# chpio/crdt-enc

Hardware: AMD Instinct MI355X
Metric: op files compacted/sec + AEAD-open GB/s, 1M×4KiB ops/4096 actors, 1–8 GPUs (higher is better)
Workload: dtype u32; 1 GPU; C2: 1,048,576 x 4 KiB encrypted GCounter op files per GPU (4096 actors x 256 versions at N=1), decrypt + max-join + compact; plaintext_bytes=4085, actors=4096, parallelism=single GPU

## Files before the change

### crdt-enc_amd/csrc/ce_core.cpp

```cpp
#include <algorithm>
#include <atomic>
#include <cstdio>
#include <functional>
#include <set>

#include "ce_core.h"
#include "ce_shard.h"

using namespace ce;

namespace ce {


bool skip_any(Rd& r, int depth) {
  if (depth > 1024) return false;
  uint64_t at, cnt = 0;
  if (r.i >= r.n) return false;
  const uint8_t m = r.p[r.i];
  bool cont = false;
  if ((m & 0xf0) == 0x80) { r.i++; cnt = 2ull * (m & 15); cont = true; }
  else if ((m & 0xf0) == 0x90) { r.i++; cnt = m & 15; cont = true; }
  else if (m == 0xdc || m == 0xdd || m == 0xde || m == 0xdf) {
    r.i++;
    if (!rd_be(r, (m == 0xdc || m == 0xde) ? 2 : 4, &cnt)) return false;
// ... 660 lines not shown
  if (is_dotset_kind(c->kind))
    return ds_ingest_ops(c, d_blob, d_offs, n, blob_len, actors, m, d_fa, d_fv, status_out);
  if (c->kind == CE_STATE_GSET)
    return gs_ingest_ops(c, d_blob, d_offs, n, blob_len, actors, m, d_fa, d_fv, status_out);
  if (c->kind == CE_STATE_LWWREG)
    return lw_ingest_ops(c, d_blob, d_offs, n, blob_len, actors, m, d_fa, d_fv, status_out);
  hipError_t e;
  const KeyRef key = key_of(c);
  const bool pnc = c->kind == CE_STATE_PNCOUNTER;
  auto words = [&] { return (uint64_t)state_planes(c->kind) * c->cap; };
  std::vector<uint32_t> wslot;
  if (c->last_writers_gen == c->table_gen && c->last_writers.size() == 16ull * m &&
      std::memcmp(c->last_writers.data(), actors, 16ull * m) == 0) {
    wslot = c->last_wslot;
  } else {
    wslot.resize(m);
    const uint64_t gen0 = c->table_gen;
    for (uint32_t a = 0; a < m; a++) {
      Uuid u;
      std::memcpy(u.data(), actors + 16ull * a, 16);
      int rc = insert_actor(c, u, &wslot[a]);
      if (rc) return rc;
    }
    if (c->table_gen != gen0) refresh_slots(c, actors, m, &wslot);
    c->last_writers.assign(actors, actors + 16ull * m);
    c->last_wslot = wslot;
    c->last_writers_gen = c->table_gen;
  }
  int rc = table_upload(c);
  if (rc) return rc;
  if ((rc = ensure_supported(c))) return rc;
  if ((e = ctx->out.reserve(blob_len + 16ull * n + 128)) || (e = ctx->status.reserve(n * 4ull + 64)) ||
      (e = ctx->apply.reserve(n + 64)) || (e = ctx->refold.reserve(n + 64)) ||
      (e = c->d_refold2.reserve(n + 64)) || (e = ctx->miss.reserve(65536 * 16)) ||
      (e = c->d_gate.reserve(m * 32ull + 8ull * c->cap + 64)) ||
      (e = ctx->h_stage2.reserve(m * 32ull + 8ull * c->cap + 64)) ||
      (e = ctx->redo.reserve(n + 64)))
    return ctx->hip_fail(e, "ingest reserve");

  uint64_t* he0 = ctx->h_stage2.as<uint64_t>();
  for (uint32_t a = 0; a < m; a++) he0[a] = c->nov[wslot[a]];
  std::memcpy(he0 + m, wslot.data(), m * 4ull);
  if (after_commit) std::memcpy(reinterpret_cast<uint8_t*>(he0) + 32ull * m, c->nov.data(), 8ull * c->cap);
  GateArgs ga{};
  ga.fa = d_fa;
  ga.fv = d_fv;
  ga.n = n;
  ga.m = m;
  uint8_t* gbase = c->d_gate.as<uint8_t>();
  ga.e0 = reinterpret_cast<const uint64_t*>(gbase);
  ga.newnov = reinterpret_cast<unsigned long long*>(gbase + 16ull * m);
  ga.run_count = reinterpret_cast<uint32_t*>(gbase + 24ull * m);
  ga.run_first = reinterpret_cast<uint32_t*>(gbase + 28ull * m);
  ga.flags = ctx->counters.as<uint32_t>() + 12;
  ga.apply = ctx->apply.as<uint8_t>();

  static const bool gate_dma = getenv("CE_GATE_DMA") != nullptr;
  const uint8_t* he0_dev = nullptr;
  if (!gate_dma) {
    void* dp = nullptr;
    if (hipHostGetDevicePointer(&dp, he0, 0) == hipSuccess) he0_dev = static_cast<const uint8_t*>(dp);
    else (void)hipGetLastError();
  }
  if (!he0_dev &&
      ((!ctx->side && (e = hipStreamCreateWithFlags(&ctx->side, hipStreamNonBlocking))) ||
       (!ctx->up_ev && (e = hipEventCreateWithFlags(&ctx->up_ev, hipEventDisableTiming))) ||
       (e = hipMemcpyAsync(gbase, he0, 12ull * m, hipMemcpyHostToDevice, ctx->side)) ||
       (after_commit && (e = hipMemcpyAsync(gbase + 32ull * m, reinterpret_cast<uint8_t*>(he0) + 32ull * m,
                                            8ull * c->cap, hipMemcpyHostToDevice, ctx->side))) ||
       (e = hipEventRecord(ctx->up_ev, ctx->side))))
    return ctx->hip_fail(e, "gate upload");

  static const bool gate_after_setup = getenv("CE_GATE_AFTER_SETUP") != nullptr;
  auto launch_gate_now = [&]() -> int {
    if (!he0_dev && (e = hipStreamWaitEvent(ctx->stream, ctx->up_ev, 0))) return ctx->hip_fail(e, "gate upload");
    const int t = ctx->tbegin("gate");
    if ((e = sharded ? launch_gate_window(ctx->stream, ga, shard_hi, ctx->counters.as<uint32_t>())
                     : launch_gate(ctx->stream, ga)))
      return ctx->hip_fail(e, "gate");
    ctx->tend(t);
    return CE_OK;
  };
  uint32_t ec;
  {
    FillArgs fl{};
    fl.r[0] = {reinterpret_cast<uint32_t*>(gbase + 16ull * m), 4ull * m, 0u};
    fl.r[1] = {c->d_batch.as<uint32_t>(), 2ull * words(), 0u};
    fl.r[2] = {ctx->refold.as<uint32_t>(), (n + 3ull) / 4, 0u};
    fl.r[3] = {ctx->redo.as<uint32_t>(), (n + 3ull) / 4, 0u};
    fl.n = 4;
    if (he0_dev) {
      fl.r[fl.n++] = {reinterpret_cast<uint32_t*>(gbase), 3ull * m, 0u, reinterpret_cast<const uint32_t*>(he0_dev)};
      if (after_commit)
        fl.r[fl.n++] = {reinterpret_cast<uint32_t*>(gbase + 32ull * m), 2ull * c->cap, 0u,
                        reinterpret_cast<const uint32_t*>(he0_dev + 32ull * m)};
    }
    if (!gate_after_setup) {
      const std::function<int()> gate = launch_gate_now;
      int rr = device_open_setup(ctx, d_blob, d_offs, n, blob_len, true, key, ctx->status.as<int32_t>(),
                                 &ec, &fl, &gate);
      if (rr) return rr;
    } else {
      int rr = device_open_setup(ctx, d_blob, d_offs, n, blob_len, true, key, ctx->status.as<int32_t>(),
                                 &ec, &fl);
      if (rr) return rr;
    }
  }
  uint32_t* hsetup = ctx->h_counters.as<uint32_t>() + 32;
  static const bool setup_event = getenv("CE_SETUP_EVENT") != nullptr;
  uint32_t* hsetup_dev = nullptr;
  if (!setup_event) {
    void* dp = nullptr;
    if (hipHostGetDevicePointer(&dp, hsetup, 0) == hipSuccess) hsetup_dev = static_cast<uint32_t*>(dp);
    else (void)hipGetLastError();
  }
  const uint32_t gen = ++ctx->publish_gen ? ctx->publish_gen : ++ctx->publish_gen;
  if (hsetup_dev) {
    if ((e = launch_publish_words(ctx->stream, ctx->counters.as<uint32_t>(), 16, hsetup_dev, gen)))
      return ctx->hip_fail(e, "setup counters");
  } else {
    if ((!ctx->setup_ev && (e = hipEventCreateWithFlags(&ctx->setup_ev, hipEventDisableTiming))) ||
        (!ctx->side_ev && (e = hipEventCreateWithFlags(&ctx->side_ev, hipEventDisableTiming))) ||
        (!ctx->side && (e = hipStreamCreateWithFlags(&ctx->side, hipStreamNonBlocking))))
      return ctx->hip_fail(e, "event");
    if ((e = hipEventRecord(ctx->side_ev, ctx->stream)) || (e = hipStreamWaitEvent(ctx->side, ctx->side_ev, 0)) ||
        (e = hipMemcpyAsync(hsetup, ctx->counters.p, 64, hipMemcpyDeviceToHost, ctx->side)) ||
        (e = hipEventRecord(ctx->setup_ev, ctx->side)))
      return ctx->hip_fail(e, "setup counters");
  }
  bool setup_known = false;
  uint32_t n_large = 0;
  if (gate_after_setup) {
    const int rg = launch_gate_now();
    if (rg) return rg;
  }
  DecodeArgs da{};
  da.pt = ctx->out.as<uint8_t>();
  da.blob = d_blob;
  da.params = ctx->params.as<FileParams>();
  da.aux = ctx->poly_aux.as<PolyAux>();
  da.status = ctx->status.as<int32_t>();
  da.n = n;
  da.supported = c->d_supported.as<uint8_t>();
  da.n_supported = (uint32_t)c->supported.size();
  da.apply = ctx->apply.as<uint8_t>();
  da.counters = ctx->counters.as<uint32_t>();
  da.miss_list = ctx->miss.as<uint4>();
  da.miss_cap = 65536;
  da.refold = ctx->refold.as<uint8_t>();
  da.table = c->d_table.as<ActorSlot>();
  da.mask = c->cap - 1;
  da.nil_actor = table_has_nil(c);
  da.batch = c->d_batch.as<unsigned long long>();
  da.large_list = ctx->large.as<uint32_t>();

  ctx->open_log.grid_cap = test_grid_cap();
  ctx->open_log.stamps = test_wave_stamps(ctx);
  ctx->open_log.stamp_waves = 0;
  auto run_fold = [&](const uint8_t* only) -> int {
    da.only = only;
    da.large_only = 1;
    if (only && (e = hipMemsetAsync(ctx->counters.as<uint32_t>() + kTicketWord, 0, 4, ctx->stream)))
      return ctx->hip_fail(e, "ticket");
    if (pnc) {
      hipEvent_t t0, t1;
      (void)ctx->tlaunch("open_fold_small", &t0, &t1);
      if ((e = launch_open_fold_pn(ctx->stream, da, ctx->open_log, t0, t1))) return ctx->hip_fail(e, "fused");
    } else if (c->fused == 2 && c->files_per_wave != 1) {
      hipEvent_t t0, t1;
      (void)ctx->tlaunch("open_fold_small", &t0, &t1);
      if ((e = launch_open_fold_v2(ctx->stream, da, c->files_per_wave, ctx->open_log, t0, t1))) return ctx->hip_fail(e, "fused");
    } else {
      const int t = ctx->tbegin("open_fold_small");
      if ((e = launch_open_fold_small(ctx->stream, da, c->files_per_wave, ctx->open_log))) return ctx->hip_fail(e, "fused");
      ctx->tend(t);
    }
    count_open_launches(c, ctx);
    if (!setup_known) {
      if (hsetup_dev) {
        volatile const uint32_t* hp = hsetup;
        for (uint64_t i = 0; hp[16] != gen; i++) {
          if (i >= 64) sched_yield();
          if (i == (1ull << 22)) {
            if ((e = hipStreamSynchronize(ctx->stream))) return ctx->hip_fail(e, "setup counters");
          } else if (i > (1ull << 22) && hp[16] != gen) {
            return ctx->fail(CE_ERR_DEVICE, "setup counters never published");
          }
        }
        std::atomic_thread_fence(std::memory_order_acquire);
      } else if ((e = hipEventSynchronize(ctx->setup_ev))) {
        return ctx->hip_fail(e, "setup counters");
      }
      n_large = hsetup[9];
      setup_known = true;
    }
    if (n_large == 0) return CE_OK;
    const char* sdv = getenv("CE_SEGDEC");
    const bool segdec = !pnc && !(sdv && sdv[0] == '0') && !getenv("CE_SPLIT");
    if (!only) {
      SegScratch sc = segscratch(ctx, ec);
      if (segdec && (e = ctx->segrec.reserve((size_t)ec * 2 * 32))) return ctx->hip_fail(e, "segment records");
      int t = ctx->tbegin("segments_open");
      if ((e = segdec ? launch_segments_decode(ctx->stream, d_blob, ctx->out.as<uint8_t>(), da, sc,
                                               grid_waves_for(n + ec), ctx->segrec.as<uint4>())
                      : launch_segments(ctx->stream, false, d_blob, ctx->out.as<uint8_t>(), da.params, n,
                                        da.status, sc, grid_waves_for(n + ec), true)))
        return ctx->hip_fail(e, "segments");
      ctx->tend(t);
      t = ctx->tbegin("finalize_open");
      if ((e = launch_finalize_multi(ctx->stream, false, ctx->out.as<uint8_t>(), da.params, da.status, sc, n)))
        return ctx->hip_fail(e, "finalize");
      ctx->tend(t);
      if (segdec) {
        t = ctx->tbegin("decode");
        DecodeArgs rd = da;
        rd.redo = ctx->redo.as<uint8_t>();
        if ((e = launch_segdec_apply(ctx->stream, rd, sc, ctx->segrec.as<uint4>(), n_large)))
          return ctx->hip_fail(e, "decode");
        rd.only = rd.redo;
        if ((e = launch_decode_dots(ctx->stream, rd, grid_waves_for(n)))) return ctx->hip_fail(e, "decode");
        ctx->tend(t);
        return CE_OK;
      }
// ... 1636 lines not shown
```

### crdt-enc_amd/csrc/ce_ctx.cpp

```cpp
#include <sys/random.h>

#include <algorithm>
#include <cstdio>

#include "ce_dotset.h"
#include "ce_dotset_io.h"
#include "ce_internal.h"
#include "ce_lww.h"

namespace ce {

hipError_t DevBuf::reserve(size_t bytes) {
  if (bytes <= cap) return hipSuccess;
  if (p) (void)hipFree(p);
  p = nullptr;
  cap = 0;
  size_t want = std::max<size_t>(bytes, 256);
  want = (want + 4095) & ~size_t(4095);
  hipError_t e = hipMalloc(&p, want);
  if (e == hipSuccess) cap = want;
  return e;
}
DevBuf::~DevBuf() {
  if (p) (void)hipFree(p);
// ... 15 lines not shown

void os_random(uint8_t* out, size_t n) {
  size_t got = 0;
  while (got < n) {
    ssize_t r = getrandom(out + got, n - got, 0);
    if (r > 0) got += (size_t)r;
  }
}

int32_t key_status(const KeyRef& k) {
  if (std::memcmp(k.version, kKeyVersion, 16) != 0) return CE_ERR_KEY_VERSION;
  if (k.len != 32) return CE_ERR_KEY_LEN;
  return CE_OK;
}

DevKey dev_key(const KeyRef& k) {
  DevKey d{};
  if (k.len == 32) std::memcpy(d.k, k.key, 32);
  return d;
}

uint32_t test_grid_cap() {
  const char* e = getenv("CE_TEST_GRID_CAP");
  const long v = e ? atol(e) : 0;
  return v < 1 ? 0u : (uint32_t)std::min<long>(v, 1l << 30);
}

unsigned long long* test_wave_stamps(ce_ctx* ctx) {
  const char* e = getenv("CE_TEST_WAVE_STAMPS");
  if (!e || atoi(e) < 1) return nullptr;
  const size_t bytes = (size_t)kStampWaves * kStampWords * 8;
  if (ctx->stamps.reserve(bytes) != hipSuccess || hipMemsetAsync(ctx->stamps.p, 0, bytes, ctx->stream) != hipSuccess) {
    (void)hipGetLastError();
    return nullptr;
  }
  return ctx->stamps.as<unsigned long long>();
}

uint32_t grid_waves_for(uint32_t work) {
  uint32_t full = 256u * 32u;
  if (const uint32_t cap = test_grid_cap()) full = std::min(full, cap);
  return std::max<uint32_t>(1, std::min<uint32_t>(work, full));
}

static int reserve_batch(ce_ctx* ctx, uint32_t n, uint64_t blob_len, uint32_t* extra_cap,
                         uint32_t seg_blocks = kSegBlocks) {
  const uint64_t ec = blob_len / (seg_blocks * 16) + 16;
  if (ec > 0xffffffffull) return ctx->fail(CE_ERR_INVALID_ARG, "batch too large");
  *extra_cap = (uint32_t)ec;
  hipError_t e;
  if ((e = ctx->params.reserve((size_t)n * sizeof(FileParams))) != hipSuccess ||
      (e = ctx->status.reserve((size_t)n * 4 + 64)) != hipSuccess ||
      (e = ctx->counters.reserve(256)) != hipSuccess ||
      (e = ctx->extra.reserve(ec * 8)) != hipSuccess ||
      (e = ctx->multi.reserve(ec * 4)) != hipSuccess ||
      (e = ctx->partials.reserve(ec * 2 * 5 * 4)) != hipSuccess ||
      (e = ctx->large.reserve((size_t)n * 4 + 64)) != hipSuccess ||
      (e = ctx->h_counters.reserve(256)) != hipSuccess)
    return ctx->hip_fail(e, "reserve batch scratch");
  return CE_OK;
}

SegScratch segscratch(ce_ctx* ctx, uint32_t extra_cap) {
  SegScratch sc;
  sc.counters = ctx->counters.as<uint32_t>();
  sc.extra_list = ctx->extra.as<uint2>();
  sc.extra_cap = extra_cap;
  sc.multi_files = ctx->multi.as<uint32_t>();
  sc.partials = ctx->partials.as<uint32_t>();
  sc.large_list = ctx->large.as<uint32_t>();
  sc.seg_blocks = kSegBlocks;
  return sc;
}

static hipError_t reset_counters(ce_ctx* ctx) {
  FillArgs fl{};
  fl.n = 0;
  fl.counters = ctx->counters.as<uint32_t>();
  return launch_fill(ctx->stream, fl);
}

int device_open_setup(ce_ctx* ctx, const uint8_t* d_blob, const uint64_t* d_offs, uint32_t n,
                      uint64_t blob_len, bool outer, const KeyRef& key, int32_t* d_status,
                      uint32_t* extra_cap, FillArgs* fills, const std::function<int()>* after_fill) {
  int rc = reserve_batch(ctx, n, blob_len, extra_cap);
  if (rc) return rc;
  hipError_t e;
  if (fills) {
    fills->counters = ctx->counters.as<uint32_t>();
    if ((e = launch_fill(ctx->stream, *fills)) != hipSuccess) return ctx->hip_fail(e, "fill");
  } else if ((e = reset_counters(ctx)) != hipSuccess) {
    return ctx->hip_fail(e, "memset counters");
  }
  if (after_fill && (rc = (*after_fill)())) return rc;
  SegScratch sc = segscratch(ctx, *extra_cap);
  if ((e = ctx->poly_aux.reserve((size_t)n * sizeof(PolyAux))) != hipSuccess)
    return ctx->hip_fail(e, "reserve poly aux");
  const int t = ctx->tbegin("open_setup");
  if ((e = launch_open_setup(ctx->stream, d_blob, d_offs, n, outer, dev_key(key), key_status(key),
                             ctx->params.as<FileParams>(), d_status, sc,
                             ctx->poly_aux.as<PolyAux>())) != hipSuccess)
    return ctx->hip_fail(e, "open setup");
  ctx->tend(t);
  return CE_OK;
}

int device_open(ce_ctx* ctx, const uint8_t* d_blob, const uint64_t* d_offs, uint32_t n,
                uint64_t blob_len, bool outer, const KeyRef& key, uint8_t* d_out,
                int32_t* d_status, bool sync_counters, bool small_lanes, const DecodeArgs* ds) {
  uint32_t ec;
  int rc = reserve_batch(ctx, n, blob_len, &ec);
  if (rc) return rc;
  hipError_t e;
  if ((e = reset_counters(ctx)) != hipSuccess) return ctx->hip_fail(e, "memset counters");
  SegScratch sc = segscratch(ctx, ec);
  FileParams* P = ctx->params.as<FileParams>();
  static const bool ds8_on = !(getenv("CE_DS8") && atoi(getenv("CE_DS8")) == 0);
  const bool want_aux = small_lanes && ds && ds->ds.on && ds->ds.big && ds8_on;
  if (want_aux && (e = ctx->poly_aux.reserve((size_t)n * sizeof(PolyAux))) != hipSuccess)
    return ctx->hip_fail(e, "reserve poly aux");
  int t = ctx->tbegin("open_setup");
  if ((e = launch_open_setup(ctx->stream, d_blob, d_offs, n, outer, dev_key(key), key_status(key),
                             P, d_status, sc, want_aux ? ctx->poly_aux.as<PolyAux>() : nullptr)) != hipSuccess)
    return ctx->hip_fail(e, "open setup");
  ctx->tend(t);
  if (small_lanes) {
    ctx->open_log.grid_cap = test_grid_cap();
    ctx->open_log.stamps = nullptr;
    ctx->open_log.stamp_waves = 0;
    DecodeArgs da{};
    da.pt = d_out;
    da.blob = d_blob;
    da.params = P;
    da.status = d_status;
    da.n = n;
    da.counters = ctx->counters.as<uint32_t>();
    if (ds) {
      da.ds = ds->ds;
      da.aux = want_aux ? ctx->poly_aux.as<PolyAux>() : nullptr;
      da.supported = ds->supported;
      da.n_supported = ds->n_supported;
      da.table = ds->table;
      da.mask = ds->mask;
    }
    t = ctx->tbegin("open_small");
    if ((e = launch_open_small_v2(ctx->stream, da, ctx->open_log)) != hipSuccess) return ctx->hip_fail(e, "open small");
    ctx->tend(t);
  }
  t = ctx->tbegin("segments_open");
  if ((e = launch_segments(ctx->stream, false, d_blob, d_out, P, n, d_status, sc,
                           grid_waves_for(n + ec), small_lanes)) != hipSuccess)
    return ctx->hip_fail(e, "open segments");
  ctx->tend(t);
  t = ctx->tbegin("finalize_open");
  if ((e = launch_finalize_multi(ctx->stream, false, d_out, P, d_status, sc, n)) != hipSuccess)
    return ctx->hip_fail(e, "open finalize");
  ctx->tend(t);
  if (sync_counters) {
    if ((e = hipMemcpyAsync(ctx->h_counters.p, ctx->counters.p, 64, hipMemcpyDeviceToHost,
                            ctx->stream)) != hipSuccess ||
        (e = stream_wait(ctx->stream)) != hipSuccess)
      return ctx->hip_fail(e, "open sync");
  }
  return CE_OK;
}

uint32_t* ctx_counters(ce_ctx* ctx) {
  return ctx->counters.reserve(256) == hipSuccess ? ctx->counters.as<uint32_t>() : nullptr;
}

int device_seal(ce_ctx* ctx, const uint8_t* d_clear, const uint64_t* d_offs, uint32_t n,
                uint64_t clear_len_total, const uint8_t* d_outer_version, const uint8_t* d_nonces,
                uint8_t* d_out, const uint64_t* d_out_offs, const KeyRef& key, bool counters_ready) {
  if (int32_t ks = key_status(key)) return ctx->fail(ks, "key rejected");
  const uint32_t seg_blocks = n <= 4 && clear_len_total <= (1u << 20) ? kPageBytes / 16 : kSegBlocks;
  uint32_t ec;
  int rc = reserve_batch(ctx, n, clear_len_total + 16ull * n, &ec, seg_blocks);
  if (rc) return rc;
  hipError_t e;
  if (!counters_ready && (e = reset_counters(ctx)) != hipSuccess) return ctx->hip_fail(e, "memset counters");
  SegScratch sc = segscratch(ctx, ec);
  sc.seg_blocks = seg_blocks;
  FileParams* P = ctx->params.as<FileParams>();
  int t = ctx->tbegin("seal_setup");
  if ((e = launch_seal_setup(ctx->stream, d_clear, d_offs, n, d_outer_version, d_nonces, d_out,
                             d_out_offs, dev_key(key), P, sc)) != hipSuccess)
    return ctx->hip_fail(e, "seal setup");
  ctx->tend(t);
  t = ctx->tbegin("segments_seal");
  if ((e = launch_segments(ctx->stream, true, d_clear, d_out, P, n, ctx->status.as<int32_t>(), sc,
                           grid_waves_for(n + ec))) != hipSuccess)
    return ctx->hip_fail(e, "seal segments");
  ctx->tend(t);
  t = ctx->tbegin("finalize_seal");
  if ((e = launch_finalize_multi(ctx->stream, true, d_out, P, ctx->status.as<int32_t>(), sc, n)) !=
      hipSuccess)
    return ctx->hip_fail(e, "seal finalize");
  ctx->tend(t);
  return CE_OK;
}

int seal_one(ce_ctx* ctx, const KeyRef& key, const uint8_t* outer_version, const uint8_t* nonce,
             const uint8_t* clear_in, size_t clear_in_len, std::vector<uint8_t>* file,
             const uint8_t* prefix16) {
  if (int32_t ks = key_status(key)) return ctx->fail(ks, "key rejected");
  const size_t pl = prefix16 ? 16 : 0;
  const size_t clear_len = pl + clear_in_len;
  const uint64_t pre = outer_version ? 16 : 0;
  const uint64_t total = pre + sealed_len(clear_len);
  uint8_t nb[24];
  if (nonce) std::memcpy(nb, nonce, 24);
  else os_random(nb, 24);
  hipError_t e;
  const uint64_t A = (clear_len + 255) & ~255ull;
  if ((e = ctx->blob.reserve(A + 128)) != hipSuccess ||
      (e = ctx->out.reserve(total + 64)) != hipSuccess ||
      (e = ctx->h_stage.reserve(std::max<uint64_t>(A + 128, total) + 256)) != hipSuccess)
    return ctx->hip_fail(e, "seal_one reserve");
  uint8_t* hs = ctx->h_stage.as<uint8_t>();
  const uint64_t args[3] = {0, clear_len, 0};
  if (pl) std::memcpy(hs, prefix16, 16);
  std::memcpy(hs + pl, clear_in, clear_in_len);
  std::memcpy(hs + A, args, 24);
  std::memcpy(hs + A + 24, nb, 24);
  if (outer_version) std::memcpy(hs + A + 48, outer_version, 16);
  if ((e = hipMemcpyAsync(ctx->blob.p, hs, A + 64, hipMemcpyHostToDevice, ctx->stream)))
    return ctx->hip_fail(e, "seal_one upload");
  uint8_t* db = ctx->blob.as<uint8_t>();
  int rc = device_seal(ctx, db, reinterpret_cast<const uint64_t*>(db + A), 1, clear_len,
                       outer_version ? db + A + 48 : nullptr, db + A + 24, ctx->out.as<uint8_t>(),
                       reinterpret_cast<const uint64_t*>(db + A + 16), key);
  if (rc) return rc;
  if ((e = hipMemcpyAsync(hs, ctx->out.p, total, hipMemcpyDeviceToHost, ctx->stream)) ||
      (e = stream_wait(ctx->stream)))
    return ctx->hip_fail(e, "seal_one download");
  file->resize(total);
  std::memcpy(file->data(), hs, total);
  return CE_OK;
}

}

using namespace ce;

template <typename F>
static int prim_run(ce_ctx* c, const char* what, bool null_arg, F&& call) {
  if (!c) return CE_ERR_INVALID_ARG;
  std::lock_guard<std::recursive_mutex> g(c->mu);
  (void)hipSetDevice(c->device);
  size_t tb = 0;
  hipError_t e = call(nullptr, tb);
  if (e == hipErrorInvalidValue) return c->fail(CE_ERR_INVALID_ARG, std::string(what) + ": more items than the primitive takes");
  if (e != hipSuccess) return c->hip_fail(e, what);
  if (null_arg) return c->fail(CE_ERR_INVALID_ARG, std::string(what) + ": null pointer");
  void* tmp = nullptr;
  if ((e = hipMalloc(&tmp, tb)) != hipSuccess) return c->hip_fail(e, what);
  if ((e = hipMemsetAsync(tmp, 0xFF, tb, c->stream)) == hipSuccess) e = call(tmp, tb);
  const hipError_t w = hipStreamSynchronize(c->stream);
  if (e == hipSuccess) e = w;
// ... 401 lines not shown
```

### crdt-enc_amd/csrc/ce_device.h

```cpp
#pragma once
#include "ce_kernels.h"

#ifndef CE_ROT16_SDWA
#define CE_ROT16_SDWA 1
#endif

namespace ce {

__device__ __forceinline__ uint32_t rotl32(uint32_t x, int c) {
  return __builtin_amdgcn_alignbit(x, x, 32 - c);
}

template <bool SD>
__device__ __forceinline__ uint32_t xor_rotl16_t(uint32_t d, uint32_t a) {
  if (!SD) return rotl32(d ^ a, 16);
  uint32_t r;
  asm("v_xor_b32_sdwa %0, %1, %2 dst_sel:WORD_0 dst_unused:UNUSED_PRESERVE src0_sel:WORD_1 src1_sel:WORD_1\n\t"
      "v_xor_b32_sdwa %0, %1, %2 dst_sel:WORD_1 dst_unused:UNUSED_PRESERVE src0_sel:WORD_0 src1_sel:WORD_0"
      : "=&v"(r) : "v"(d), "v"(a));
  return r;
}
__device__ __forceinline__ uint32_t xor_rotl16(uint32_t d, uint32_t a) {
  return xor_rotl16_t<CE_ROT16_SDWA != 0>(d, a);
}
// ... 221 lines not shown
  c = h.v[0] >> 26; h.v[0] &= M26; h.v[1] += c;
  return h;
}

__device__ __forceinline__ L5 block_limbs(uint32_t w0, uint32_t w1, uint32_t w2, uint32_t w3) {
  L5 m;
  m.v[0] = w0 & M26;
  m.v[1] = __builtin_amdgcn_alignbit(w1, w0, 26) & M26;
  m.v[2] = __builtin_amdgcn_alignbit(w2, w1, 20) & M26;
  m.v[3] = __builtin_amdgcn_alignbit(w3, w2, 14) & M26;
  m.v[4] = __builtin_amdgcn_alignbit(1u, w3, 8);
  return m;
}

__device__ __forceinline__ void poly_tag(L5 h, const uint32_t (&s)[4], uint32_t (&tag)[4]) {
  h = carry5(h);
  uint32_t c;
  c = h.v[1] >> 26; h.v[1] &= M26; h.v[2] += c;
  c = h.v[2] >> 26; h.v[2] &= M26; h.v[3] += c;
  c = h.v[3] >> 26; h.v[3] &= M26; h.v[4] += c;
  uint32_t g[5];
  g[0] = h.v[0] + 5; c = g[0] >> 26; g[0] &= M26;
  g[1] = h.v[1] + c; c = g[1] >> 26; g[1] &= M26;
  g[2] = h.v[2] + c; c = g[2] >> 26; g[2] &= M26;
  g[3] = h.v[3] + c; c = g[3] >> 26; g[3] &= M26;
  g[4] = h.v[4] + c - (1u << 26);
  const uint32_t mask = (g[4] >> 31) - 1;
#pragma unroll
  for (int i = 0; i < 5; i++) h.v[i] = (h.v[i] & ~mask) | (g[i] & mask);
  const uint32_t w0 = h.v[0] | (h.v[1] << 26);
  const uint32_t w1 = (h.v[1] >> 6) | (h.v[2] << 20);
  const uint32_t w2 = (h.v[2] >> 12) | (h.v[3] << 14);
  const uint32_t w3 = (h.v[3] >> 18) | (h.v[4] << 8);
  uint64_t f = (uint64_t)w0 + s[0]; tag[0] = (uint32_t)f;
  f = (uint64_t)w1 + s[1] + (f >> 32); tag[1] = (uint32_t)f;
  f = (uint64_t)w2 + s[2] + (f >> 32); tag[2] = (uint32_t)f;
  f = (uint64_t)w3 + s[3] + (f >> 32); tag[3] = (uint32_t)f;
}

__device__ __forceinline__ L5 load_l5(const uint32_t* p) {
  L5 o;
#pragma unroll
  for (int i = 0; i < 5; i++) o.v[i] = p[i];
  return o;
}

__device__ __forceinline__ uint32_t ld_le32(const uint8_t* p) {
  return (uint32_t)p[0] | ((uint32_t)p[1] << 8) | ((uint32_t)p[2] << 16) | ((uint32_t)p[3] << 24);
}

__device__ __forceinline__ void key_schedule_w(const DevKey& key, const uint32_t (&nw)[6], FileParams& P) {
  uint32_t k[8], n16[4], sub[8];
#pragma unroll
  for (int i = 0; i < 8; i++) k[i] = key.k[i];
#pragma unroll
  for (int i = 0; i < 4; i++) n16[i] = nw[i];
  hchacha20(k, n16, sub);
  const uint32_t n2a = nw[4], n2b = nw[5];
  uint32_t b0[16];
  chacha_block(sub, 0, 0, n2a, n2b, b0);
#pragma unroll
  for (int i = 0; i < 8; i++) P.subkey[i] = sub[i];
  P.n2[0] = n2a; P.n2[1] = n2b;
  const uint32_t r0 = b0[0] & 0x0fffffffu, r1 = b0[1] & 0x0ffffffcu, r2 = b0[2] & 0x0ffffffcu,
                 r3 = b0[3] & 0x0ffffffcu;
  L5 r;
  r.v[0] = r0 & M26;
  r.v[1] = __builtin_amdgcn_alignbit(r1, r0, 26) & M26;
  r.v[2] = __builtin_amdgcn_alignbit(r2, r1, 20) & M26;
  r.v[3] = __builtin_amdgcn_alignbit(r3, r2, 14) & M26;
  r.v[4] = r3 >> 8;
  P.s[0] = b0[4]; P.s[1] = b0[5]; P.s[2] = b0[6]; P.s[3] = b0[7];
#pragma unroll
  for (int i = 0; i < 5; i++) P.rpow[0][i] = r.v[i];
  L5 p = r;
#pragma unroll
  for (int kk = 1; kk < 7; kk++) {
    p = mulmod(p, p);
#pragma unroll
    for (int i = 0; i < 5; i++) P.rpow[kk][i] = p.v[i];
  }
}

__device__ __forceinline__ void poly_aux(const FileParams& P, PolyAux& X) {
  const L5 r = load_l5(P.rpow[0]), r2 = load_l5(P.rpow[1]), r4 = load_l5(P.rpow[2]);
  const L5 r3 = mulmod(r2, r);
  const L5 r12 = mulmod(load_l5(P.rpow[3]), r4);
  const L5 r48 = mulmod(load_l5(P.rpow[5]), load_l5(P.rpow[4]));
  const uint32_t npc = (P.len + 15) >> 4, nblk = (P.len + 63) >> 6;
  const uint32_t delta = 4 * nblk - npc;
  const L5 r5 = mulmod(r4, r), r6 = mulmod(r4, r2);
  const L5 e6 = delta == 0 ? r6 : delta == 1 ? r5 : delta == 2 ? r4 : r3;
  const L5 lr = mulmod(block_limbs(0u, 0u, P.len, 0u), r);
#pragma unroll
  for (int i = 0; i < 5; i++) {
    X.r3[i] = r3.v[i]; X.r12[i] = r12.v[i]; X.r48[i] = r48.v[i];
    X.e6[i] = e6.v[i]; X.lr[i] = lr.v[i];
  }
  uint64_t b = 0;
#pragma unroll
  for (int i = 0; i < 4; i++) {
    const uint64_t d = (uint64_t)P.tag[i] - P.s[i] - b;
    X.ts[i] = (uint32_t)d;
    b = (d >> 32) & 1;
  }
  X.pad[0] = X.pad[1] = X.pad[2] = 0;
}

__device__ __forceinline__ bool poly_check(L5 h, const uint32_t (&ts)[4]) {
  uint32_t c;
  c = h.v[0] >> 26; h.v[0] &= M26; h.v[1] += c;
  c = h.v[1] >> 26; h.v[1] &= M26; h.v[2] += c;
  c = h.v[2] >> 26; h.v[2] &= M26; h.v[3] += c;
  c = h.v[3] >> 26; h.v[3] &= M26; h.v[4] += c;
  c = h.v[4] >> 26; h.v[4] &= M26; h.v[0] += c * 5;
  c = h.v[0] >> 26; h.v[0] &= M26; h.v[1] += c;
  c = h.v[1] >> 26; h.v[1] &= M26; h.v[2] += c;
  c = h.v[2] >> 26; h.v[2] &= M26; h.v[3] += c;
  c = h.v[3] >> 26; h.v[3] &= M26; h.v[4] += c;
  uint32_t g[5];
  g[0] = h.v[0] + 5; c = g[0] >> 26; g[0] &= M26;
  g[1] = h.v[1] + c; c = g[1] >> 26; g[1] &= M26;
  g[2] = h.v[2] + c; c = g[2] >> 26; g[2] &= M26;
  g[3] = h.v[3] + c; c = g[3] >> 26; g[3] &= M26;
  g[4] = h.v[4] + c - (1u << 26);
  const uint32_t mask = (g[4] >> 31) - 1;
#pragma unroll
  for (int i = 0; i < 5; i++) h.v[i] = (h.v[i] & ~mask) | (g[i] & mask);
  const uint32_t w0 = h.v[0] | (h.v[1] << 26);
  const uint32_t w1 = (h.v[1] >> 6) | (h.v[2] << 20);
  const uint32_t w2 = (h.v[2] >> 12) | (h.v[3] << 14);
  const uint32_t w3 = (h.v[3] >> 18) | (h.v[4] << 8);
  return ((w0 ^ ts[0]) | (w1 ^ ts[1]) | (w2 ^ ts[2]) | (w3 ^ ts[3])) == 0;
}

__device__ __forceinline__ void key_schedule(const DevKey& key, const uint8_t* nonce, FileParams& P) {
  uint32_t nw[6];
#pragma unroll
  for (int i = 0; i < 6; i++) nw[i] = ld_le32(nonce + 4 * i);
  key_schedule_w(key, nw, P);
}

__device__ __forceinline__ void reserve_segments(FileParams& P, uint32_t f, SegScratch sc, bool mine = true) {
  const uint64_t nblk = ((uint64_t)P.len + 15) / 16 + 1;
  const uint32_t nseg = mine ? (uint32_t)((nblk + sc.seg_blocks - 1) / sc.seg_blocks) : 0u;
  if (mine) {
    P.nseg = nseg;
    P.extra_base = 0;
  }
  uint32_t e = 0;
  if (nseg > 1) {
    e = atomicAdd(&sc.counters[0], nseg - 1);
    const uint32_t pb = atomicAdd(&sc.counters[6], nseg);
    const uint32_t mf = atomicAdd(&sc.counters[1], 1u);
    P.extra_base = pb;
    sc.multi_files[mf] = f;
    if (nseg <= 33)
      for (uint32_t j = 1; j < nseg; j++) sc.extra_list[e + j - 1] = make_uint2(f, j);
  }
  const unsigned long long act = __ballot(true);
  const uint32_t lane = threadIdx.x & 63;
  const uint32_t rank = (uint32_t)__builtin_popcountll(act & ((1ull << lane) - 1ull));
  const uint32_t nact = (uint32_t)__builtin_popcountll(act);
  for (unsigned long long big = __ballot(nseg > 33); big; big &= big - 1) {
    const int src = (int)__builtin_ctzll(big);
    const uint32_t fe = (uint32_t)__shfl((int)e, src), ff = (uint32_t)__shfl((int)f, src);
    const uint32_t fn = (uint32_t)__shfl((int)nseg, src);
    for (uint32_t j = 1 + rank; j < fn; j += nact) sc.extra_list[fe + j - 1] = make_uint2(ff, j);
  }
}


static constexpr int kKsStride = 80;

__device__ __forceinline__ uint32_t bcast(uint32_t v) { return __builtin_amdgcn_readfirstlane(v); }

__device__ __forceinline__ void batch_max(unsigned long long* p, unsigned long long v) {
  if (v > *p) atomicMax(p, v);
}

__device__ __forceinline__ uint32_t lookup_slot(const ActorSlot* __restrict__ tab, uint32_t mask,
// ... 87 lines not shown
```

### crdt-enc_amd/csrc/ce_fused.hip

```cpp
#include <algorithm>

#include <hip/hip_ext.h>

#include "ce_device.h"
#include "ce_gset_device.h"
#include "ce_lww.h"

namespace ce {

static constexpr uint32_t kRegion = 64 * kKsStride - 16;

#ifndef CE_NCH
#define CE_NCH 2
#endif
template <int LPF>
struct FusedCfg {
  static constexpr int F = 64 / LPF;
  static constexpr int WPB = LPF == 16 ? 2 : 4;
  static constexpr int LOG = LPF == 16 ? 4 : LPF == 32 ? 5 : 6;
  static constexpr int WAVES_PER_SIMD = LPF == 16 ? 2 : LPF == 32 ? 3 : 4;
  static constexpr int NCH = LPF * CE_NCH <= 64 ? CE_NCH : 64 / LPF;
  static constexpr int LOGCH = NCH == 4 ? 2 : NCH == 2 ? 1 : 0;
};

// ... 586 lines not shown
        uint4 x = ct[j];
        const uint32_t boff = q * 16;
        if (boff + 16 > len) {
          const uint32_t rem = len - boff;
          uint32_t xw[4] = {x.x, x.y, x.z, x.w};
#pragma unroll
          for (int i = 0; i < 4; i++) {
            const uint32_t lo = 4 * i;
            const uint32_t keep = rem >= lo + 4 ? 0xffffffffu
                                  : (rem <= lo ? 0u : ((1u << (8 * (rem - lo))) - 1));
            xw[i] &= keep;
            kw_mask[i] = keep;
          }
          x = make_uint4(xw[0], xw[1], xw[2], xw[3]);
        }
        uint4 y = make_uint4(x.x ^ (k4.x & kw_mask[0]), x.y ^ (k4.y & kw_mask[1]),
                             x.z ^ (k4.z & kw_mask[2]), x.w ^ (k4.w & kw_mask[3]));
        *reinterpret_cast<uint4*>(fl + boff) = y;
        acc[c] = add5(mulmod(acc[c], RS), block_limbs(x.x, x.y, x.z, x.w));
      }
    }
    L5 lv = acc[0];
    {
      L5 p1, p2;
#pragma unroll
      for (int i = 0; i < 5; i++) {
        p1.v[i] = rp[5 * C::LOG + i];
        p2.v[i] = C::NCH > 2 ? rp[5 * (C::LOG + 1) + i] : 0u;
      }
      if (C::NCH > 1) lv = add5(lv, mulmod(acc[C::NCH > 1 ? 1 : 0], p1));
      if (C::NCH > 2) lv = add5(lv, mulmod(acc[C::NCH > 2 ? 2 : 0], p2));
      if (C::NCH > 3) lv = add5(lv, mulmod(acc[C::NCH > 3 ? 3 : 0], mulmod(p1, p2)));
      lv = carry5(lv);
    }
    __builtin_amdgcn_wave_barrier();

    L5 v = lv;
#pragma unroll
    for (int k = 0; k < C::LOG; k++) {
      L5 rk;
#pragma unroll
      for (int i = 0; i < 5; i++) rk.v[i] = rp[5 * k + i];
      L5 o;
#pragma unroll
      for (int i = 0; i < 5; i++)
        o.v[i] = k < 4 ? row_down(v.v[i], 1 << k) : (uint32_t)__shfl_down((int)v.v[i], 1u << k);
      v = carry5(add5(v, mulmod(o, rk)));
    }
    L5 r1;
#pragma unroll
    for (int i = 0; i < 5; i++) r1.v[i] = rp[i];
    const L5 tot = mulmod(v, r1);
    bool tag_ok = false;
    if (act && sub == 0) {
      const uint32_t sv[4] = {sv4.x, sv4.y, sv4.z, sv4.w};
      uint32_t tag[4];
      poly_tag(tot, sv, tag);
      tag_ok = ((tag[0] ^ tg4.x) | (tag[1] ^ tg4.y) | (tag[2] ^ tg4.z) | (tag[3] ^ tg4.w)) == 0;
      if (!tag_ok) a.status[f] = CE_ERR_AUTH;
    }
    fails.add(act && sub == 0 && !tag_ok, f);
    const bool ok = grp_bits<LPF>(tag_ok, grp) != 0;

    decode_fold<LPF>(a, sup, fl, len, act && ok, cur.apply != 0, f, grp, sub, S,
                     [&] { nx = load_pre<C::LOG + C::LOGCH>(a, (g + stride) * F + grp); });
    __builtin_amdgcn_wave_barrier();
  }
  fails.flush(a);
}

template <typename K>
static uint32_t resident_blocks(K kernel, int threads) {
  int dev = 0, per_cu = 0, cus = 0;
  if (hipGetDevice(&dev) != hipSuccess) return 256;
  if (hipDeviceGetAttribute(&cus, hipDeviceAttributeMultiprocessorCount, dev) != hipSuccess) cus = 256;
  if (hipOccupancyMaxActiveBlocksPerMultiprocessor(&per_cu, kernel, threads, 0) != hipSuccess ||
      per_cu < 1)
    per_cu = 1;
  return (uint32_t)(per_cu * cus);
}

hipError_t launch_open_fold_small(hipStream_t s, const DecodeArgs& a, int files_per_wave, OpenLaunchLog& log) {
  if (a.n == 0) return hipSuccess;
  static const uint32_t res16 = resident_blocks(k_open_fold_small<16>, 128);
  static const uint32_t res32 = resident_blocks(k_open_fold_small<32>, 256);
  static const uint32_t res64 = resident_blocks(k_open_fold_small<64>, 256);
  const uint32_t groups = (a.n + files_per_wave - 1) / files_per_wave;
  if (files_per_wave == 4) {
    const uint32_t blocks = log.grid(std::min<uint32_t>((groups + 1) / 2, res16), "open_small_lpf16");
    hipLaunchKernelGGL(k_open_fold_small<16>, dim3(blocks), dim3(128), 0, s, a);
  } else if (files_per_wave == 2) {
    const uint32_t blocks = log.grid(std::min<uint32_t>((groups + 3) / 4, res32), "open_small_lpf32");
    hipLaunchKernelGGL(k_open_fold_small<32>, dim3(blocks), dim3(256), 0, s, a);
  } else {
    const uint32_t blocks = log.grid(std::min<uint32_t>((groups + 3) / 4, res64), "open_small_lpf64");
    hipLaunchKernelGGL(k_open_fold_small<64>, dim3(blocks), dim3(256), 0, s, a);
  }
  return hipGetLastError();
}

static constexpr uint32_t kRegion2 = 4096;
static constexpr uint32_t kRegionStride2 = 4128;

template <int LPF>
struct V2Cfg {
  static constexpr int F = 64 / LPF;
  static constexpr int BPL = 64 / LPF;
  static constexpr int LOG = LPF == 16 ? 4 : 5;
  static constexpr int NRP = LPF == 16 ? 8 : 9;
};

struct FilePre2 {
  uint32_t ok, apply, len, in_off, in_hi;
  uint32_t key[8];
  uint32_t n2a, n2b;
  uint32_t R1[5];
  uint32_t R64[5];
  uint32_t R2[5];
};

__device__ __forceinline__ FilePre2 load_pre2(const DecodeArgs& a, uint32_t f) {
  FilePre2 p;
  const bool in = f < a.n;
  const uint32_t fi = in ? f : 0u;
  const FileParams* Pp = a.params + fi;
  const int32_t stv = a.status[fi];
  const uint32_t ov = a.only ? (uint32_t)a.only[fi] : 1u;
  const uint32_t av = a.apply ? (uint32_t)a.apply[fi] : 1u;
  p.ok = (uint32_t)in & (uint32_t)(stv == CE_OK) & (uint32_t)(ov != 0);
  p.apply = av != 0;
  p.len = Pp->len;
  p.in_off = (uint32_t)Pp->in_off;
  p.in_hi = (uint32_t)(Pp->in_off >> 32);
#pragma unroll
  for (int i = 0; i < 8; i++) p.key[i] = Pp->subkey[i];
  p.n2a = Pp->n2[0];
  p.n2b = Pp->n2[1];
#pragma unroll
  for (int i = 0; i < 5; i++) {
    p.R1[i] = Pp->rpow[0][i];
    p.R64[i] = Pp->rpow[6][i];
    p.R2[i] = Pp->rpow[1][i];
  }
  return p;
}

static constexpr uint32_t kDsStride = kDsFuseRegion + 96;
static constexpr uint32_t kDsCandCap = 96;
static constexpr uint32_t kDsVCap = 64;
static constexpr uint32_t kDsAuxHalves = kDsCandCap + 2 * kDsVCap;
static constexpr uint32_t kAddMagic = 0x6441a381u;
static constexpr uint32_t kRmMagic = 0x6d52a281u;

template <int N>
struct LdsWin {
  uint32_t w[N];
  __device__ __forceinline__ LdsWin(const uint32_t* L, uint32_t x) {
    const uint32_t* b = L + (x >> 2);
    const uint32_t sh = x & 3u;
    uint32_t d[N + 1];
#pragma unroll
    for (int k = 0; k <= N; k++) d[k] = b[k];
#pragma unroll
    for (int k = 0; k < N; k++) w[k] = __builtin_amdgcn_alignbyte(d[k + 1], d[k], sh);
  }
  __device__ __forceinline__ uint32_t word(int b) const {
    return (b & 3) ? __builtin_amdgcn_alignbyte(w[(b >> 2) + 1], w[b >> 2], b & 3) : w[b >> 2];
  }
  __device__ __forceinline__ uint32_t byte(int b) const { return (w[b >> 2] >> (8 * (b & 3))) & 0xffu; }
  __device__ __forceinline__ unsigned long long uint_at(int b, uint32_t* len) const {
    const uint32_t m = byte(b);
    const uint32_t x0 = __builtin_bswap32(word(b + 1)), x1 = __builtin_bswap32(word(b + 5));
    *len = m < 0x80u ? 1u : m == 0xccu ? 2u : m == 0xcdu ? 3u : m == 0xceu ? 5u : m == 0xcfu ? 9u : 0u;
    return m < 0x80u ? m : m == 0xccu ? x0 >> 24 : m == 0xcdu ? x0 >> 16 : m == 0xceu ? x0
                                                       : ((unsigned long long)x0 << 32) | x1;
  }
};

struct DsOp {
  uint32_t kind;
  uint32_t len, u0, u1, u2, u3;
  unsigned long long ctr, mem;
};

__device__ __forceinline__ DsOp ds_parse_fast(const uint32_t* L, uint32_t x, uint32_t len) {
  DsOp o{};
  const LdsWin<13> v(L, x);
  uint32_t l = 0, y = 0;
  if (v.w[0] == kAddMagic && v.w[1] == 0x64a38264u && v.w[2] == 0xa582746fu && v.w[3] == 0x6f746361u &&
      (v.w[4] & 0xffffffu) == 0x10c472u && v.word(35) == 0x756f63a7u && v.word(39) == 0x7265746eu) {
    o.ctr = v.uint_at(43, &l);
    o.u0 = v.word(19); o.u1 = v.word(23); o.u2 = v.word(27); o.u3 = v.word(31);
    y = 43 + l;
    o.kind = l ? 1u : 0u;
  } else if (v.w[0] == kRmMagic && v.w[1] == 0x6c63a582u && v.w[2] == 0x816b636fu && v.w[3] == 0x746f64a4u &&
             v.w[4] == 0x10c48173u) {
    o.ctr = v.uint_at(36, &l);
    o.u0 = v.w[5]; o.u1 = v.w[6]; o.u2 = v.w[7]; o.u3 = v.w[8];
    y = 36 + l;
    o.kind = l ? 2u : 0u;
  }
  if (o.kind) {
    const LdsWin<5> m(L, x + y);
    uint32_t lm = 0;
    if (m.word(0) == 0x6d656da7u && m.word(4) == 0x73726562u && m.byte(8) == 0x91u) o.mem = m.uint_at(9, &lm);
    o.len = y + 9 + lm;
    if (!lm || x + o.len > len) o.kind = 0;
  }
  return o;
}

struct DsActorCache {
  uint32_t k0 = 0, k1 = 0, k2 = 0, k3 = 0, id = 0xffffffffu;
  uint4 pk = make_uint4(0, 0, 0, 0);
  uint32_t pused = 0, pid = 0xffffffffu;
  __device__ __forceinline__ void prime(const DecodeArgs& a, const uint32_t* L, uint32_t p0, uint32_t len) {
    if (p0 + 40 > len) return;
    const LdsWin<6> w(L, p0);
    const uint32_t u = w.byte(1) == 0xa3u ? 19u : 20u;
    const LdsWin<4> v(L, p0 + u);
    k0 = v.w[0]; k1 = v.w[1]; k2 = v.w[2]; k3 = v.w[3];
    const ActorSlot& sl = a.table[actor_hash(k0, k1, k2, k3) & a.mask];
    pk = *reinterpret_cast<const uint4*>(sl.k);
    pused = sl.used;
    pid = sl.pad[0];
// ... 577 lines not shown
  uint32_t wv = 0, wm = 0, stride = 0;
  if (dec && cnt > 0 && blen - h >= 14) {
    wv = lww_uint_width((uint8_t)body[h + 5]);
    if (wv && h + 12 + wv < blen) wm = lww_uint_width((uint8_t)body[h + 12 + wv]);
    if (wv && wm) stride = 12 + wv + wm;
    if (stride && (unsigned long long)cnt * stride > blen - h) stride = 0;
  }
  bool bad = dec && cnt > 0 && stride == 0;
  unsigned long long bm = 0, bv = 0;
  uint32_t bi = 0xffffffffu;
  if (stride)
    for (uint32_t e = sub; e < cnt && !bad; e += LPF) {
      const uint32_t x = h + e * stride;
      const LdsWin<4> V(L, x);
      uint32_t lv = 0, lm = 0;
      const unsigned long long v = V.uint_at(5, &lv);
      const LdsWin<4> M(L, x + 5 + wv);
      const unsigned long long m = M.uint_at(7, &lm);
      bad = V.w[0] != 0x6176a382u || V.byte(4) != 0x6cu || lv != wv || M.w[0] != 0x72616da6u ||
            (M.w[1] & 0xffffffu) != 0x72656bu || lm != wm;
      if (!bad && m > bm) { bm = m; bv = v; bi = e; }
    }
  const bool general = dec && grp_bits<LPF>(bad, grp) != 0;
  if (dec && sub == 0) {
    C.uni += general ? 0u : 1u;
    C.gen += general ? 1u : 0u;
  }
#pragma unroll
  for (int d = LPF / 2; d >= 1; d >>= 1) {
    const unsigned long long om = lw_shfl_xor64(bm, d), ov = lw_shfl_xor64(bv, d);
    const uint32_t oi = (uint32_t)__shfl_xor((int)bi, d);
    const bool take = om > bm || (om == bm && oi < bi);
    bm = take ? om : bm;
    bv = take ? ov : bv;
    bi = take ? oi : bi;
  }
  if (general && sub == 0) {
    bm = 0;
    bv = 0;
    Rd q{body, blen, h};
    for (uint32_t e = 0; e < cnt; e++) {
      uint64_t v = 0, m = 0;
      if (parse_lww_op(q, &v, &m) != 1) { st = CE_ERR_DECODE; break; }
      if (m > bm) { bm = m; bv = v; }
    }
  }
  if (dec && st == CE_OK && apply && sub == 0 && bm != 0) a.lw->rec[f] = LwwRec{bm, bv};
  if (live && st != CE_OK && sub == 0) {
    a.status[f] = st;
    atomicAdd(&a.counters[3], 1u);
    atomicMin(&a.counters[5], f);
  }
}

__device__ const uint32_t kPolyOne[8] = {1u, 0u, 0u, 0u, 0u, 0u, 0u, 0u};

template <bool PAIR, bool EARLY, bool PN = false, bool GS = false, bool LW = false>
__global__ __launch_bounds__(64, 2)
void k_open_fold_v3(DecodeArgs a) {
  constexpr int LPF = 16, F = 4, BPL = 4;
  __shared__ __attribute__((aligned(16))) uint8_t lds[(F - 1) * kRegionStride2 + kRegion2 + 64];
  const uint32_t lane = threadIdx.x & 63;
  const uint32_t grp = lane / LPF, sub = lane % LPF;
  uint8_t* fl = lds + grp * kRegionStride2;
  const uint32_t ngroups = (a.n + F - 1) / F;
  const uint32_t fixed = (uint32_t)((uint64_t)(ngroups / gridDim.x) * CE_DYN_STATIC_PCT / 100u);
  const uint32_t dyn0 = fixed * gridDim.x;
  uint32_t tk = 0;
  auto draw = [&] {
    uint32_t tw = kTicketWord;
    asm volatile("" : "+v"(tw));
    if (lane == 0) tk = atomicAdd(a.counters + tw, 1u);
  };
  auto chunk = [&](uint32_t& lo, uint32_t& hi) {
    const uint64_t s = dyn0 + (uint64_t)bcast(tk) * CE_DYN_CHUNK;
    lo = s < ngroups ? (uint32_t)s : ngroups;
    hi = ngroups - lo < CE_DYN_CHUNK ? ngroups : lo + CE_DYN_CHUNK;
    draw();
  };
  draw();
  uint32_t gn = bcast(blockIdx.x * fixed), c_end = gn + fixed;
  if (fixed == 0) chunk(gn, c_end);
  if (a.stamps && lane == 0) a.stamps[(uint64_t)kStampWords * blockIdx.x] = __builtin_amdgcn_s_memrealtime();
  FilePre2 nx = load_pre2(a, gn * F + grp);
  const SupVers sup(a);
  DecState S{PN ? 51u : 38u, 0, 0, 0, 0, 0xffffffffu};
  GsCounts gsc;
  LwCounts lwc;
  AuthFails fails;
  const uint32_t qpos = (sub + 15u) & 15u;
  const uint32_t qx = qpos & 3u, qy = qpos >> 2;
  static_assert(offsetof(FileParams, rpow) == 80, "rpow offset");
  auto wsrc = [&](uint32_t q, uint32_t aux_off, uint32_t rp_idx, const uint8_t*& base, uint32_t& stride) {
    base = q == 0 ? reinterpret_cast<const uint8_t*>(kPolyOne)
         : q == 3 ? reinterpret_cast<const uint8_t*>(a.aux) + aux_off
                  : reinterpret_cast<const uint8_t*>(a.params) + 80u + 20u * rp_idx;
    stride = q == 0 ? 0u : q == 3 ? (uint32_t)sizeof(PolyAux) : (uint32_t)sizeof(FileParams);
  };
  const uint8_t* x_base;
  const uint8_t* y_base;
  uint32_t x_stride, y_stride;
  wsrc(qx, (uint32_t)offsetof(PolyAux, r12), qx + 1u, x_base, x_stride);
  wsrc(qy, (uint32_t)offsetof(PolyAux, r48), qy + 3u, y_base, y_stride);

  uint4 ct[BPL][4];
  while (gn < ngroups) {
    const uint32_t f = gn * F + grp;
    const FilePre2 cur = nx;
    if (++gn == c_end) chunk(gn, c_end);
    if (EARLY) nx = load_pre2(a, gn * F + grp);
    const bool act = cur.ok && cur.len <= kSmallMax;
    const uint32_t len = act ? cur.len : 0u;
    const uint32_t npc = (len + 15) >> 4;
    const int32_t nblk = (int32_t)((len + 63) >> 6);
    const FileParams* Pp = a.params + (act ? f : 0);
    const PolyAux* Xp = a.aux + (act ? f : 0);
    const uint8_t* src = act ? a.blob + (((uint64_t)cur.in_hi << 32) | cur.in_off)
                             : reinterpret_cast<const uint8_t*>(a.params);
#pragma unroll
    for (int k = BPL - 1; k >= 0; k--) {
      const int32_t b = nblk - 1 - (int32_t)sub - LPF * k;
      if (k > 0) {
        const uint8_t* bp = b >= 0 ? src + 64u * (uint32_t)b : reinterpret_cast<const uint8_t*>(a.params);
#pragma unroll
        for (int j = 0; j < 4; j++) ct[k][j] = *reinterpret_cast<const uint4*>(bp + 16 * j);
      } else {
#pragma unroll
        for (int j = 0; j < 4; j++) {
          const uint32_t q = (uint32_t)(4 * b + j);
          const uint32_t off = b >= 0 ? 16u * (q < npc ? q : npc - 1u) : 0u;
          ct[0][j] = *reinterpret_cast<const uint4*>(src + off);
        }
      }
    }
    L5 R1, RC, R2, R3;
#pragma unroll
    for (int i = 0; i < 5; i++) {
      R1.v[i] = cur.R1[i];
      RC.v[i] = cur.R64[i];
      R2.v[i] = Pp->rpow[1][i];
      R3.v[i] = Xp->r3[i];
    }
    const ChachaPre cpre = chacha_pre(cur.key, 0u, cur.n2a, cur.n2b);
    L5 acc{{0, 0, 0, 0, 0}}, glast{{0, 0, 0, 0, 0}};
    L5 X, Y, E6, LR;
    uint32_t ts[4];
    uint4 pc[4];
    const uint32_t dl = sub == 0 ? (uint32_t)(4 * nblk) - npc : 0u;
    const uint32_t rb = sub == 0 && npc ? len - 16u * (npc - 1u) : 16u;
    uint32_t kbn[16];

#pragma unroll
    for (int k = BPL - 1; k >= 0; k--) {
      const int32_t b = nblk - 1 - (int32_t)sub - LPF * k;
      const bool has = b >= 0;
      if (k == (PAIR ? 1 : 0)) {
        const int32_t b0 = nblk - 1 - (int32_t)sub;
        const uint8_t* pb = b0 >= 0 ? src + 16 * (int64_t)(4 * b0 - (int32_t)dl) : src;
#pragma unroll
        for (int j = 0; j < 4; j++) pc[j] = *reinterpret_cast<const uint4*>(pb + 16 * j);
        const uint32_t fi = act ? f : 0u;
        const uint32_t* xs = reinterpret_cast<const uint32_t*>(x_base + (uint64_t)fi * x_stride);
        const uint32_t* ys = reinterpret_cast<const uint32_t*>(y_base + (uint64_t)fi * y_stride);
#pragma unroll
        for (int i = 0; i < 5; i++) {
          X.v[i] = xs[i];
          Y.v[i] = ys[i];
          E6.v[i] = Xp->e6[i];
          LR.v[i] = Xp->lr[i];
        }
#pragma unroll
        for (int i = 0; i < 4; i++) ts[i] = Xp->ts[i];
      }
      uint32_t kb[16];
      if (!PAIR) {
        chacha_block_pre<true, CE_V3_UNR>(cpre, cur.key, 1u + (uint32_t)b, 0u, cur.n2a, cur.n2b, kb);
      } else {
        if (k & 1) chacha_block_pre2<CE_V3_UNR>(cpre, cur.key, 1u + (uint32_t)b, 1u + (uint32_t)(b + LPF), 0u,
                                     cur.n2a, cur.n2b, kb, kbn);
        else {
#pragma unroll
          for (int i = 0; i < 16; i++) kb[i] = kbn[i];
        }
      }
      L5 m[4];
#pragma unroll
      for (int j = 0; j < 4; j++) {
        const uint32_t q = (uint32_t)(4 * b + j);
        const uint4 c = ct[k][j];
        const uint4 pv = make_uint4(c.x ^ kb[4 * j], c.y ^ kb[4 * j + 1], c.z ^ kb[4 * j + 2], c.w ^ kb[4 * j + 3]);
        *reinterpret_cast<uint4*>(fl + (has ? q * 16u : kRegion2 - 16u)) = pv;
        if (k > 0) {
          m[j] = block_limbs(c.x, c.y, c.z, c.w);
        } else {
          uint32_t w[4] = {pc[j].x, pc[j].y, pc[j].z, pc[j].w};
          const bool pres = (uint32_t)j >= dl;
#pragma unroll
          for (int i = 0; i < 4; i++) {
            if (j == 3) {
              const int32_t cb = (int32_t)rb - 4 * i;
              const uint32_t keep = cb >= 4 ? ~0u : cb <= 0 ? 0u : ((1u << (8 * cb)) - 1u);
              w[i] &= keep;
            } else {
              w[i] = pres ? w[i] : 0u;
            }
          }
          m[j] = block_limbs(w[0], w[1], w[2], w[3]);
          if (j < 3) m[j].v[4] = pres ? m[j].v[4] : 0u;
        }
      }
      uint64_t d[5] = {m[3].v[0], m[3].v[1], m[3].v[2], m[3].v[3], m[3].v[4]};
      if (k < BPL - 1) {
        L5 ain = acc;
        if (k == 0) {
#pragma unroll
          for (int i = 0; i < 5; i++) ain.v[i] = sub == 0 ? 0u : acc.v[i];
        }
        mac5(d, ain, mul_r(RC));
      }
      mac5(d, m[0], mul_r(R3));
      mac5(d, m[1], mul_r(R2));
      mac5(d, m[2], mul_r(R1));
      const L5 an = reduce5(d);
      const bool to_acc = has && !(k == 0 && sub == 0);
#pragma unroll
      for (int i = 0; i < 5; i++) acc.v[i] = to_acc ? an.v[i] : acc.v[i];
      if (k == 0) {
#pragma unroll
        for (int i = 0; i < 5; i++) glast.v[i] = has && sub == 0 ? an.v[i] : 0u;
      }
    }

    L5 v = mulmod(mulmod(acc, X), Y);
#pragma unroll
    for (int k = 0; k < 4; k++) {
#pragma unroll
      for (int i = 0; i < 5; i++) v.v[i] += row_down(v.v[i], 1 << k);
    }
    uint64_t d[5] = {LR.v[0], LR.v[1], LR.v[2], LR.v[3], LR.v[4]};
    mac5(d, v, mul_r(E6));
    mac5(d, glast, mul_r(R2));
    const L5 tot = reduce5(d);
    bool tag_ok = false;
    if (act && sub == 0) {
      tag_ok = poly_check(tot, ts);
      if (!tag_ok) a.status[f] = CE_ERR_AUTH;
    }
    fails.add(act && sub == 0 && !tag_ok, f);
    const bool ok = grp_bits<LPF>(tag_ok, grp) != 0;

    if (CE_V3_PRIO) __builtin_amdgcn_s_setprio(CE_V3_PRIO);
    if constexpr (LW) {
      decode_lww_lds<LPF>(a, sup, fl, len, act && ok, cur.apply != 0, f, grp, sub, lwc, [&] {
        if (!EARLY) nx = load_pre2(a, gn * F + grp);
      });
    } else if constexpr (GS) {
      decode_gset_lds<LPF>(a, sup, fl, len, act && ok, cur.apply != 0, f, grp, sub, gsc, [&] {
        if (!EARLY) nx = load_pre2(a, gn * F + grp);
      });
    } else {
      decode_fold<LPF, true, PN>(a, sup, fl, len, act && ok, cur.apply != 0, f, grp, sub, S, [&] {
        if (!EARLY) nx = load_pre2(a, gn * F + grp);
      });
    }
    if (CE_V3_PRIO) __builtin_amdgcn_s_setprio(0);
    __builtin_amdgcn_wave_barrier();
  }
  if constexpr (LW) lwc.flush(a);
  else if constexpr (GS) gsc.flush(a);
  else flush_pending<LPF>(a, sub, S.pslot, S.pbest);
  fails.flush(a);
  if (a.stamps) {
    const unsigned long long t_out = __builtin_amdgcn_s_memrealtime();
    const unsigned long long hw = (uint32_t)__builtin_amdgcn_s_getreg((31 << 11) | 4) |
                                  ((unsigned long long)(uint32_t)__builtin_amdgcn_s_getreg((3 << 11) | 20) << 32);
    if (lane == 0) {
      unsigned long long* o = a.stamps + (uint64_t)kStampWords * blockIdx.x;
      o[1] = t_out;
      o[2] = hw;
    }
  }
}

template <bool PF>
__global__ __launch_bounds__(64, 2)
void k_open_ds8(DecodeArgs a) {
  constexpr int LPF = 8, F = 8, BPL = 4;
  constexpr uint32_t kStride = kDsFuseRegion + 64;
  __shared__ __attribute__((aligned(16))) uint8_t lds[F * kStride + F * kDsAuxHalves * 2];
  const uint32_t lane = threadIdx.x & 63;
  const uint32_t grp = lane / LPF, sub = lane % LPF;
  uint8_t* fl = lds + grp * kStride;
  uint16_t* aux = reinterpret_cast<uint16_t*>(lds + F * kStride) + grp * kDsAuxHalves;
  const uint32_t ngroups = (a.n + F - 1) / F;
  const uint32_t g_end = (uint32_t)(((uint64_t)(blockIdx.x + 1) * ngroups) / gridDim.x);
  uint32_t g = bcast((uint32_t)(((uint64_t)blockIdx.x * ngroups) / gridDim.x));
  FilePre2 nx = load_pre2(a, g * F + grp);
  const SupVers sup(a);
  AuthFails fails;
  const uint32_t qpos = (sub + 7u) & 7u;
  const uint32_t qx = qpos & 3u;
  const bool x_one = qx == 0, y_one = (qpos >> 2) == 0, x_aux = qx == 3;
  const uint32_t x_off = x_aux ? (uint32_t)offsetof(PolyAux, r12) : 80u + 20u * (qx + 1u);
  uint4 ct[BPL][4];
  auto load_ct = [&](const FilePre2& p) {
    const bool ac = p.ok && p.len <= kDsFuseRegion;
    const uint32_t ln = ac ? p.len : 0u;
    const uint32_t np = (ln + 15) >> 4;
    const int32_t nb = (int32_t)((ln + 63) >> 6);
    const uint8_t* sr = ac ? a.blob + (((uint64_t)p.in_hi << 32) | p.in_off) : reinterpret_cast<const uint8_t*>(a.params);
#pragma unroll
    for (int k = BPL - 1; k >= 0; k--) {
      const int32_t b = nb - 1 - (int32_t)sub - LPF * k;
      if (k > 0) {
        const uint8_t* bp = b >= 0 ? sr + 64u * (uint32_t)b : reinterpret_cast<const uint8_t*>(a.params);
#pragma unroll
        for (int j = 0; j < 4; j++) ct[k][j] = *reinterpret_cast<const uint4*>(bp + 16 * j);
      } else {
#pragma unroll
        for (int j = 0; j < 4; j++) {
          const uint32_t q = (uint32_t)(4 * b + j);
          const uint32_t off = b >= 0 ? 16u * (q < np ? q : np - 1u) : 0u;
          ct[0][j] = *reinterpret_cast<const uint4*>(sr + off);
        }
      }
    }
  };
  if (PF) load_ct(nx);
  for (; g < g_end; g++) {
    const uint32_t f = g * F + grp;
    const FilePre2 cur = nx;
    nx = load_pre2(a, (g + 1) * F + grp);
    const bool act0 = cur.ok && cur.len <= kSmallMax;
    const bool big = act0 && cur.len > kDsFuseRegion;
    const bool act = act0 && !big;
    const uint32_t len = act ? cur.len : 0u;
    const uint32_t npc = (len + 15) >> 4;
    const int32_t nblk = (int32_t)((len + 63) >> 6);
    const FileParams* Pp = a.params + (act ? f : 0);
    const PolyAux* Xp = a.aux + (act ? f : 0);
    const uint8_t* src = act ? a.blob + (((uint64_t)cur.in_hi << 32) | cur.in_off)
                             : reinterpret_cast<const uint8_t*>(a.params);
    uint8_t* gout = const_cast<uint8_t*>(a.pt) + Pp->out_off;
    if (!PF) load_ct(cur);
    L5 R1, RC, R2, R3;
// ... 84 lines not shown
      X.v[i] = x_one ? (i == 0 ? 1u : 0u) : X.v[i];
      Y.v[i] = y_one ? (i == 0 ? 1u : 0u) : Y.v[i];
    }
    L5 v = mulmod(mulmod(acc, X), Y);
#pragma unroll
    for (int k = 0; k < 3; k++) {
#pragma unroll
      for (int i = 0; i < 5; i++) v.v[i] += row_down(v.v[i], 1 << k);
    }
    uint64_t d[5] = {LR.v[0], LR.v[1], LR.v[2], LR.v[3], LR.v[4]};
    mac5(d, v, mul_r(E6));
    mac5(d, glast, mul_r(R2));
    const L5 tot = reduce5(d);
    bool tag_ok = false;
    if (act && sub == 0) {
      tag_ok = poly_check(tot, ts);
      if (!tag_ok) a.status[f] = CE_ERR_AUTH;
    }
    fails.add(act && sub == 0 && !tag_ok, f);
    const bool ok = grp_bits<LPF>(tag_ok, grp) != 0;
    if (PF) load_ct(nx);
    bool done = false;
    if (__any(act && ok)) {
      if (CE_DS_PRIO) __builtin_amdgcn_s_setprio(CE_DS_PRIO);
      done = ds_fused_decode<LPF>(a, sup, fl, aux, len, act && ok, f, grp, sub);
      if (CE_DS_PRIO) __builtin_amdgcn_s_setprio(0);
    }
    if (act && ok && !done) {
      for (uint32_t q = sub; q * 16u < len; q += LPF)
        *reinterpret_cast<uint4*>(gout + q * 16u) = *reinterpret_cast<const uint4*>(fl + q * 16u);
    }
    if (sub == 0 && f < a.n) {
      a.ds.done[f] = done ? 1 : 0;
      a.ds.big[f] = big ? 1 : 0;
    }
    const unsigned long long bb = __ballot(big && sub == 0);
    if (bb && lane == (uint32_t)__builtin_ctzll(bb)) atomicAdd(&a.counters[10], (uint32_t)__builtin_popcountll(bb));
    __syncthreads();
  }
  fails.flush(a);
}

template <int LPF, int W, bool PF, bool DEC = true, bool DS = false>
static void launch_v2(hipStream_t s, const DecodeArgs& a, OpenLaunchLog& log, const char* key,
                      hipEvent_t t0 = nullptr, hipEvent_t t1 = nullptr) {
  static const uint32_t res = resident_blocks(k_open_fold_v2<LPF, W, PF, DEC, DS>, 64);
  const uint32_t groups = (a.n + 64 / LPF - 1) / (64 / LPF);
  const dim3 grid(log.grid(std::min<uint32_t>(groups, res), key));
  if (t0) {
    hipExtLaunchKernelGGL((k_open_fold_v2<LPF, W, PF, DEC, DS>), grid, dim3(64), 0, s, t0, t1, 0u, a);
  } else {
    hipLaunchKernelGGL((k_open_fold_v2<LPF, W, PF, DEC, DS>), grid, dim3(64), 0, s, a);
  }
}

hipError_t launch_open_small_v2(hipStream_t s, const DecodeArgs& a, OpenLaunchLog& log) {
  if (a.n == 0) return hipSuccess;
  static const bool ds8_on = !(getenv("CE_DS8") && atoi(getenv("CE_DS8")) == 0);
  if (a.ds.on && a.aux && a.ds.big && ds8_on) {
    static const bool pf = !(getenv("CE_DS8_PF") && atoi(getenv("CE_DS8_PF")) == 0);
    if (pf) {
      static const uint32_t res = resident_blocks(k_open_ds8<true>, 64);
      const dim3 grid(log.grid(std::min<uint32_t>((a.n + 7) / 8, res), "open_ds8_pf"));
      hipLaunchKernelGGL(k_open_ds8<true>, grid, dim3(64), 0, s, a);
    } else {
      static const uint32_t res = resident_blocks(k_open_ds8<false>, 64);
      const dim3 grid(log.grid(std::min<uint32_t>((a.n + 7) / 8, res), "open_ds8_nopf"));
      hipLaunchKernelGGL(k_open_ds8<false>, grid, dim3(64), 0, s, a);
    }
    DecodeArgs b = a;
    b.only = a.ds.big;
    launch_v2<16, 3, false, false, true>(s, b, log, "open_ds16");
  } else if (a.ds.on) {
    launch_v2<16, 3, false, false, true>(s, a, log, "open_ds16");
  } else {
    launch_v2<16, 3, false, false>(s, a, log, "open_only_lpf16");
  }
  return hipGetLastError();
}

hipError_t launch_open_fold_pn(hipStream_t s, const DecodeArgs& a, OpenLaunchLog& log, hipEvent_t t0,
                               hipEvent_t t1) {
  if (a.n == 0) return hipSuccess;
  if (!a.aux) return hipErrorInvalidValue;
  static const uint32_t res = resident_blocks(k_open_fold_v3<false, true, true>, 64);
  const dim3 grid(log.grid(std::min<uint32_t>((a.n + 3) / 4, res), "open_v3_pn"));
  const DecodeArgs b = log.stamped(a, grid.x);
  if (t0) hipExtLaunchKernelGGL((k_open_fold_v3<false, true, true>), grid, dim3(64), 0, s, t0, t1, 0u, b);
  else hipLaunchKernelGGL((k_open_fold_v3<false, true, true>), grid, dim3(64), 0, s, b);
  return hipGetLastError();
}

hipError_t launch_open_fold_gset(hipStream_t s, const DecodeArgs& a, OpenLaunchLog& log, hipEvent_t t0,
                                 hipEvent_t t1) {
  if (a.n == 0) return hipSuccess;
  if (!a.aux || !a.gs) return hipErrorInvalidValue;
  static const uint32_t res = resident_blocks(k_open_fold_v3<false, true, false, true>, 64);
  const dim3 grid(log.grid(std::min<uint32_t>((a.n + 3) / 4, res), "open_v3_gset"));
  const DecodeArgs b = log.stamped(a, grid.x);
  if (t0) hipExtLaunchKernelGGL((k_open_fold_v3<false, true, false, true>), grid, dim3(64), 0, s, t0, t1, 0u, b);
  else hipLaunchKernelGGL((k_open_fold_v3<false, true, false, true>), grid, dim3(64), 0, s, b);
  return hipGetLastError();
}

hipError_t launch_open_fold_lww(hipStream_t s, const DecodeArgs& a, OpenLaunchLog& log, hipEvent_t t0,
                                hipEvent_t t1) {
  if (a.n == 0) return hipSuccess;
  if (!a.aux || !a.lw) return hipErrorInvalidValue;
  static const uint32_t res = resident_blocks(k_open_fold_v3<false, true, false, false, true>, 64);
  const dim3 grid(log.grid(std::min<uint32_t>((a.n + 3) / 4, res), "open_v3_lww"));
  const DecodeArgs b = log.stamped(a, grid.x);
  if (t0) hipExtLaunchKernelGGL((k_open_fold_v3<false, true, false, false, true>), grid, dim3(64), 0, s, t0, t1, 0u, b);
  else hipLaunchKernelGGL((k_open_fold_v3<false, true, false, false, true>), grid, dim3(64), 0, s, b);
  return hipGetLastError();
}

hipError_t launch_open_fold_v2(hipStream_t s, const DecodeArgs& a, int files_per_wave, OpenLaunchLog& log,
                               hipEvent_t t0, hipEvent_t t1) {
  if (a.n == 0) return hipSuccess;
  static const bool force_v2 = getenv("CE_FUSED_V2") != nullptr;
  if (files_per_wave == 4 && a.aux && !force_v2) {
    static const int v3 = [] {
      const char* e = getenv("CE_V3");
      return e ? atoi(e) : 2;
    }();
    auto go = [&](auto kern, const char* key) {
      const uint32_t res = resident_blocks(kern, 64);
      const dim3 grid(log.grid(std::min<uint32_t>((a.n + 3) / 4, res), key));
      const DecodeArgs b = log.stamped(a, grid.x);
      if (t0) hipExtLaunchKernelGGL(kern, grid, dim3(64), 0, s, t0, t1, 0u, b);
      else hipLaunchKernelGGL(kern, grid, dim3(64), 0, s, b);
    };
    switch (v3 & 3) {
      case 1: go(k_open_fold_v3<true, false>, "open_v3_p1e0"); break;
      case 2: go(k_open_fold_v3<false, true>, "open_v3_p0e1"); break;
      case 3: go(k_open_fold_v3<true, true>, "open_v3_p1e1"); break;
      default: go(k_open_fold_v3<false, false>, "open_v3_p0e0"); break;
    }
    return hipGetLastError();
  }
  if (files_per_wave == 2) launch_v2<32, 3, true>(s, a, log, "open_v2_lpf32", t0, t1);
  else launch_v2<16, 2, false>(s, a, log, "open_v2_lpf16", t0, t1);
  return hipGetLastError();
}

__global__ void k_gate_runs(GateArgs g) {
  const uint32_t i = blockIdx.x * blockDim.x + threadIdx.x;
  if (i >= g.n) return;
  const uint32_t a = g.fa[i];
  if (a >= g.m) { atomicOr(&g.flags[0], 1u); return; }
  if (i == 0 || g.fa[i - 1] != a) {
    if (atomicAdd(&g.run_count[a], 1u) != 0) atomicOr(&g.flags[0], 1u);
    g.run_first[a] = i;
    if (g.fv[i] > g.e0[a]) atomicMin(&g.flags[1], i);
  } else if (g.fv[i] != g.fv[i - 1] + 1) {
    atomicOr(&g.flags[0], 1u);
  }
}

__global__ void k_gate_apply(GateArgs g) {
  const uint32_t i = blockIdx.x * blockDim.x + threadIdx.x;
  if (i >= g.n) return;
  const uint32_t a = g.fa[i];
  bool ap = false;
  if (a < g.m) {
    const uint64_t e0 = g.e0[a];
    const uint64_t vf = g.fv[g.run_first[a]];
    const uint32_t gap = g.flags[1];
    ap = g.fv[i] >= e0 && vf <= e0 && i < gap;
    const bool last = i + 1 == g.n || g.fa[i + 1] != a || i + 1 >= gap;
    if (ap && last) {
      atomicMax(&g.newnov[a], (unsigned long long)(g.fv[i] + 1));
      if (g.newnov_host) g.newnov_host[a] = g.fv[i] + 1;
    }
  }
  g.apply[i] = ap ? 1 : 0;
}

hipError_t launch_gate(hipStream_t s, const GateArgs& g) {
  if (g.n == 0) return hipSuccess;
  const uint32_t blocks = (g.n + 255) / 256;
  hipLaunchKernelGGL(k_gate_runs, dim3(blocks), dim3(256), 0, s, g);
  hipLaunchKernelGGL(k_gate_apply, dim3(blocks), dim3(256), 0, s, g);
  return hipGetLastError();
}

}
```

### crdt-enc_amd/csrc/ce_gset.h

```cpp
#pragma once
#include <hip/hip_runtime.h>
#include <stdint.h>

#include "ce_kernels.h"

namespace ce {

static constexpr int kGsCount = 0;
static constexpr int kGsZero = 1;
static constexpr int kGsOverflow = 2;
static constexpr int kGsMetaWords = 4;

struct GsTable {
  unsigned long long* slots;
  uint32_t mask;
  uint32_t limit;
  uint32_t* meta;
};

struct GsDecodeArgs {
  const uint8_t* pt;
  const FileParams* params;
  int32_t* status;
  uint32_t n;
  const uint8_t* supported;
  uint32_t n_supported;
  const uint8_t* apply;
  const uint8_t* only;
  int large_only;
  GsTable committed;
  GsTable batch;
  uint32_t* paths;
};

struct GsFused {
  GsTable committed, batch;
  uint32_t* paths;
};

hipError_t launch_decode_gset(hipStream_t s, const GsDecodeArgs& a, uint32_t grid_waves);
hipError_t launch_gs_insert(hipStream_t s, GsTable t, const unsigned long long* keys, uint32_t n);
static constexpr uint32_t kGsMaxParts = 64;
struct GsParts {
  const unsigned long long* part[kGsMaxParts];
  uint32_t pre[kGsMaxParts + 1];
  uint32_t k;
};
hipError_t launch_gs_insert_parts(hipStream_t s, GsTable t, const GsParts& ps);
struct GsStateFile {
  unsigned long long body;
  uint32_t blen;
  uint32_t count;
  uint32_t pre;
  uint32_t pad;
};
static constexpr uint32_t kGsStateRunWords = 8;
static constexpr uint32_t kGsStateMaxFiles = 128;
hipError_t launch_gs_state_runs(hipStream_t s, const uint8_t* base, const GsStateFile* files, uint32_t n,
                                uint32_t max_count, uint32_t* runs);
hipError_t launch_gs_state_insert(hipStream_t s, GsTable t, const uint8_t* base, const GsStateFile* files, uint32_t k,
                                  uint32_t total, const uint32_t* runs);
hipError_t launch_gs_move(hipStream_t s, GsTable src, GsTable dst);
hipError_t launch_gs_contains(hipStream_t s, GsTable t, const unsigned long long* q, uint64_t n, uint8_t* out,
                              uint32_t grid_cap);
hipError_t launch_gs_collect(hipStream_t s, GsTable t, unsigned long long* out, uint32_t* n_out);
hipError_t launch_gs_widths(hipStream_t s, const unsigned long long* v, uint32_t n, uint32_t* w);
hipError_t launch_gs_write(hipStream_t s, const unsigned long long* v, const uint32_t* off, uint32_t n, uint8_t* out,
                           unsigned long long* clear_len_at, uint64_t head_len);

static constexpr uint32_t kGsFileMembers = 453;
struct GsFilesArgs {
  const unsigned long long* members;
  unsigned long long n;
  uint32_t per_file;
  uint32_t n_files;
  uint32_t* clen;
  uint32_t* xlen;
  const uint32_t* coff;
  const uint32_t* xoff;
  uint8_t dv[16];
  uint8_t* clear;
  unsigned long long* offs;
  unsigned long long* file_offs;
};
static constexpr uint64_t kGsSealBase = 16 + sealed_len(0);
hipError_t launch_gs_file_sizes(hipStream_t s, const GsFilesArgs& a);
hipError_t launch_gs_files_encode(hipStream_t s, const GsFilesArgs& a, uint32_t grid_cap);
hipError_t launch_gs_new_mark(hipStream_t s, GsTable t, const unsigned long long* sorted, uint32_t n, uint32_t* keep);
hipError_t launch_gs_new_compact(hipStream_t s, const unsigned long long* sorted, const uint32_t* keep,
                                 const uint32_t* pos, uint32_t n, unsigned long long* out);

}
```

### crdt-enc_amd/csrc/ce_gset.hip

```cpp
#include <hip/hip_runtime.h>
#include <stdint.h>

#include "ce_gset.h"
#include "ce_gset_device.h"

namespace ce {
namespace {

constexpr int kWaves = 4;

__device__ uint32_t gs_elem(const uint8_t* body, uint32_t blen, uint32_t p, unsigned long long* out) {
  if (p >= blen) return 0;
  const uint32_t m = body[p];
  if (m <= 0x7f) {
    *out = m;
    return 1;
  }
  if (m < 0xcc || m > 0xd3) return 0;
  const bool sgn = m >= 0xd0;
  const uint32_t w = 1u << ((m - 0xcc) & 3);
  if (blen - p - 1 < w) return 0;
  unsigned long long x = 0;
  for (uint32_t k = 0; k < w; k++) x = (x << 8) | body[p + 1 + k];
  if (sgn && ((x >> (8 * w - 1)) & 1)) return 0;
// ... 10 lines not shown
  else {
    const uint4 dv = *reinterpret_cast<const uint4*>(pt);
    bool found = false;
    for (uint32_t s = 0; s < a.n_supported; s++) {
      const uint4 sv = *reinterpret_cast<const uint4*>(a.supported + 16 * s);
      found |= dv.x == sv.x && dv.y == sv.y && dv.z == sv.z && dv.w == sv.w;
    }
    if (!found) st = CE_ERR_PT_VERSION;
  }
  const bool ins = st == CE_OK && a.apply[f];
  auto put = [&](unsigned long long v) { gs_put(a.committed, a.batch, v); };
  if (st == CE_OK) {
    const uint8_t* body = pt + 16;
    const uint32_t blen = len - 16;
    uint32_t cnt = 0, h = 0;
    if (blen == 0) st = CE_ERR_DECODE;
    else {
      const uint32_t m = body[0];
      if ((m & 0xf0) == 0x90) { cnt = m & 15; h = 1; }
      else if (m == 0xdc && blen >= 3) { cnt = (uint32_t)body[1] << 8 | body[2]; h = 3; }
      else if (m == 0xdd && blen >= 5) {
        cnt = (uint32_t)body[1] << 24 | (uint32_t)body[2] << 16 | (uint32_t)body[3] << 8 | body[4];
        h = 5;
      } else st = CE_ERR_DECODE;
      if (st == CE_OK && cnt > blen - h) st = CE_ERR_DECODE;
    }
    if (st == CE_OK) {
      uint32_t w0 = 0, mk = 0;
      if (cnt > 0) {
        mk = body[h];
        w0 = mk <= 0x7f ? 1u : (mk >= 0xcc && mk <= 0xcf) ? 1u + (1u << (mk - 0xcc)) : 0u;
        if (w0 && (unsigned long long)cnt * w0 > blen - h) w0 = 0;
      }
      bool ok = w0 != 0;
      if (w0)
        for (uint32_t e = lane; e < cnt && ok; e += 64) {
          const uint32_t m = body[h + e * w0];
          ok = w0 == 1 ? m <= 0x7f : m == mk;
        }
      const bool uniform = cnt == 0 || __ballot(ok) == ~0ull;
      if (uniform) {
        if (lane == 0) atomicAdd(&a.paths[0], 1u);
        if (ins) {
          for (uint32_t e = lane; e < cnt; e += 64) {
            unsigned long long v = 0;
            (void)gs_elem(body, blen, h + e * w0, &v);
            put(v);
          }
        }
      } else {
        if (lane == 0) atomicAdd(&a.paths[1], 1u);
        uint32_t pos = h, remaining = cnt;
        while (remaining > 0 && st == CE_OK) {
          const uint32_t todo = remaining < 64 ? remaining : 64;
          uint32_t mine = 0xffffffffu;
          for (uint32_t k = 0; k < todo; k++) {
            uint32_t w = 0;
            unsigned long long v;
            if (lane == 0) w = gs_elem(body, blen, pos, &v);
            w = (uint32_t)__shfl((int)w, 0);
            if (w == 0) { st = CE_ERR_DECODE; break; }
            if (lane == k) mine = pos;
            pos += w;
          }
          if (st != CE_OK) break;
          if (ins && mine != 0xffffffffu) {
            unsigned long long v = 0;
            (void)gs_elem(body, blen, mine, &v);
            put(v);
          }
          remaining -= todo;
        }
      }
    }
  }
  if (st != CE_OK && lane == 0) a.status[f] = st;
}

__global__ __launch_bounds__(256) void k_decode_gset(GsDecodeArgs a) {
  const uint32_t lane = threadIdx.x & 63;
  const uint32_t stride = gridDim.x * kWaves;
  for (uint32_t f = __builtin_amdgcn_readfirstlane(blockIdx.x * kWaves + (threadIdx.x >> 6)); f < a.n; f += stride) {
    if (a.only && !a.only[f]) continue;
    if (a.large_only && a.params[f].len <= kSmallMax) continue;
    if (a.status[f] != CE_OK) continue;
    decode_gset_file(a, f, lane);
  }
}

__global__ __launch_bounds__(256) void k_gs_insert(GsTable t, const unsigned long long* keys, uint32_t n) {
  for (uint32_t i = blockIdx.x * 256 + threadIdx.x; i < n; i += gridDim.x * 256) gs_insert(t, keys[i]);
}

__global__ __launch_bounds__(256) void k_gs_insert_parts(GsTable t, GsParts ps) {
  __shared__ uint32_t s_pre[kGsMaxParts + 1];
  __shared__ const unsigned long long* s_ptr[kGsMaxParts];
  if (threadIdx.x <= ps.k) s_pre[threadIdx.x] = ps.pre[threadIdx.x];
  if (threadIdx.x < ps.k) s_ptr[threadIdx.x] = ps.part[threadIdx.x];
  __syncthreads();
  const uint32_t total = ps.pre[ps.k];
  const uint32_t stride = gridDim.x * 256;
  for (uint32_t base = blockIdx.x * 256 + threadIdx.x; base < total; base += 4 * stride) {
    unsigned long long v[4], s[4];
#pragma unroll
    for (int j = 0; j < 4; j++) {
      const uint32_t i = base + (uint32_t)j * stride;
      v[j] = 0;
      if (i < total) {
        uint32_t lo = 0, hi = ps.k;
        while (hi - lo > 1) {
          const uint32_t mid = (lo + hi) >> 1;
          if (s_pre[mid] <= i) lo = mid;
          else hi = mid;
        }
        v[j] = s_ptr[lo][i - s_pre[lo]];
      }
    }
#pragma unroll
    for (int j = 0; j < 4; j++) s[j] = ld_slot(&t.slots[gs_hash(v[j]) & t.mask]);
#pragma unroll
    for (int j = 0; j < 4; j++) {
      if (base + (uint32_t)j * stride >= total) continue;
      if (v[j] != 0 && s[j] == v[j]) continue;
      gs_insert(t, v[j]);
    }
  }
}

__device__ __forceinline__ uint32_t gs_run_width(uint32_t r) { return r == 0 ? 1u : r == 1 ? 2u : r == 2 ? 3u : r == 3 ? 5u : 9u; }

__global__ __launch_bounds__(256) void k_gs_state_runs(const uint8_t* base, const GsStateFile* files, uint32_t n,
                                                       uint32_t* runs, uint32_t phase) {
  const uint32_t w = gs_run_width(phase);
  const uint32_t stride = gridDim.x * 256;
  for (uint32_t f = blockIdx.y; f < n; f += gridDim.y) {
    const GsStateFile F = files[f];
    uint32_t* R = runs + kGsStateRunWords * f;
    uint32_t s = 0;
    unsigned long long o = 0;
    for (uint32_t k = 0; k < phase; k++) {
      const uint32_t L = R[k];
      s += L;
      o += (unsigned long long)L * gs_run_width(k);
    }
    const uint32_t rem = F.count - s;
    const uint8_t* body = base + F.body;
    for (uint32_t t = blockIdx.x * 256 + threadIdx.x; t <= rem; t += stride) {
      if (t >= ld_word(&R[phase])) break;
      bool bad = t == rem;
      if (!bad) {
        const unsigned long long pos = o + (unsigned long long)w * t;
        if (pos + w > F.blen) bad = true;
        else {
          const uint32_t m = body[pos];
          bad = phase == 0 ? m > 0x7f : m != 0xcbu + phase;
        }
      }
      if (bad) {
        if (t < ld_word(&R[phase])) atomicMin(&R[phase], t);
        break;
      }
    }
  }
}

__global__ __launch_bounds__(256) void k_gs_state_insert(GsTable t, const uint8_t* base, const GsStateFile* files,
                                                         uint32_t k, const uint32_t* runs) {
// ... 215 lines not shown
```

### crdt-enc_amd/csrc/ce_gset_host.cpp

```cpp
#include <algorithm>
#include <cstring>

#include "ce_core.h"
#include "ce_dotset.h"
#include "ce_dotset_io.h"
#include "ce_gset.h"

namespace ce {

struct GsState {
  DevBuf slots, bslots;
  DevBuf meta;
  uint32_t cap = 0, bcap = 0;
  bool batch_dirty = false;
  DevBuf col, sorted, vals, sort_tmp, scan_tmp, only;
  DevBuf gate;
  DevBuf fused;
  GsFused h_fused;
  DevBuf rd;
  HostBuf h_rd;
  uint64_t head_hint = 1u << 14;
  DevBuf wr, filt, up_col, up_files, up_offs;
};

// ... 2 lines not shown
namespace {

constexpr uint32_t kMetaWords = 16;
constexpr uint32_t kMinCap = 16;

uint32_t pow2_at_least(uint64_t v) {
  uint32_t p = kMinCap;
  while (p < v && p < (1u << 31)) p <<= 1;
  return p;
}

GsTable committed(const GsState* g) {
  return GsTable{g->slots.as<unsigned long long>(), g->cap - 1, g->cap / 2, g->meta.as<uint32_t>()};
}
GsTable batch(const GsState* g) {
  return GsTable{g->bslots.as<unsigned long long>(), g->bcap - 1, g->bcap / 2, g->meta.as<uint32_t>() + 4};
}

int read_meta(ce_core* c, uint32_t* hm) {
  hipError_t e;
  if ((e = hipMemcpyAsync(hm, c->gs->meta.p, kMetaWords * 4, hipMemcpyDeviceToHost, c->ctx->stream)) ||
      (e = stream_wait(c->ctx->stream)))
    return c->ctx->hip_fail(e, "gset meta");
  return CE_OK;
}

int rehash(ce_core* c, bool is_batch, uint32_t new_cap) {
  GsState* g = c->gs;
  hipStream_t s = c->ctx->stream;
  DevBuf nb;
  hipError_t e;
  uint32_t* meta = g->meta.as<uint32_t>();
  if ((e = nb.reserve((size_t)new_cap * 8)) || (e = hipMemsetAsync(nb.p, 0, (size_t)new_cap * 8, s)) ||
      (e = hipMemsetAsync(meta + 8, 0, 16, s)))
    return c->ctx->hip_fail(e, "gset grow");
  const GsTable src = is_batch ? batch(g) : committed(g);
  const GsTable dst{nb.as<unsigned long long>(), new_cap - 1, new_cap / 2, meta + 8};
  if ((e = launch_gs_move(s, src, dst)) ||
      (e = hipMemcpyAsync(src.meta, meta + 8, 16, hipMemcpyDeviceToDevice, s)) || (e = stream_wait(s)))
    return c->ctx->hip_fail(e, "gset grow");
  if (is_batch) {
    g->bslots = std::move(nb);
    g->bcap = new_cap;
  } else {
    g->slots = std::move(nb);
    g->cap = new_cap;
  }
  c->path_counts[is_batch ? "gset_batch_grows" : "gset_grows"]++;
  return CE_OK;
}

int ensure_committed(ce_core* c, uint64_t count, uint64_t extra) {
  GsState* g = c->gs;
  if (count + extra <= g->cap / 2) return CE_OK;
  if (count + extra > (1ull << 30)) return c->ctx->fail(CE_ERR_INVALID_ARG, "set too large for the table");
  return rehash(c, false, pow2_at_least(2 * (count + extra)));
}

int clear_batch(ce_core* c) {
  GsState* g = c->gs;
  hipError_t e;
  if ((e = hipMemsetAsync(g->bslots.p, 0, (size_t)g->bcap * 8, c->ctx->stream)) ||
      (e = hipMemsetAsync(g->meta.as<uint32_t>() + 4, 0, 16, c->ctx->stream)))
    return c->ctx->hip_fail(e, "gset batch clear");
  g->batch_dirty = false;
  return CE_OK;
}

int decode_pass(ce_core* c, uint32_t n, const uint8_t* only, bool large_only = false) {
  ce_ctx* ctx = c->ctx;
  GsState* g = c->gs;
  hipError_t e;
  for (int round = 0;; round++) {
    GsDecodeArgs a{};
    a.pt = ctx->out.as<uint8_t>();
    a.params = ctx->params.as<FileParams>();
    a.status = ctx->status.as<int32_t>();
    a.n = n;
    a.supported = c->d_supported.as<uint8_t>();
    a.n_supported = (uint32_t)c->supported.size();
    a.apply = ctx->apply.as<uint8_t>();
    a.only = only;
    a.large_only = large_only ? 1 : 0;
    a.committed = committed(g);
    a.batch = batch(g);
    a.paths = g->meta.as<uint32_t>() + 12;
    if ((e = hipMemsetAsync(a.paths, 0, 12, ctx->stream))) return ctx->hip_fail(e, "gset decode");
    const int t = ctx->tbegin("decode_gset");
    if ((e = launch_decode_gset(ctx->stream, a, grid_waves_for(n)))) return ctx->hip_fail(e, "gset decode");
    ctx->tend(t);
    g->batch_dirty = true;
    uint32_t hm[kMetaWords];
    int rc = read_meta(c, hm);
    if (rc) return rc;
    if (!hm[4 + kGsOverflow]) {
      c->path_counts["gset_uniform_files"] += hm[12];
      c->path_counts["gset_general_files"] += hm[13];
      return CE_OK;
    }
    if (round > 32 || g->bcap >= (1u << 31)) return ctx->fail(CE_ERR_DEVICE, "batch table did not converge");
    if ((e = hipMemsetAsync(g->meta.as<uint32_t>() + 4 + kGsOverflow, 0, 4, ctx->stream)))
      return ctx->hip_fail(e, "gset decode");
    if ((rc = rehash(c, true, g->bcap * 2))) return rc;
  }
}

int download_status(ce_core* c, uint32_t n, std::vector<int32_t>* st) {
  st->resize(n);
  hipError_t e;
  if ((e = hipMemcpyAsync(st->data(), c->ctx->status.p, n * 4ull, hipMemcpyDeviceToHost, c->ctx->stream)) ||
      (e = stream_wait(c->ctx->stream)))
    return c->ctx->hip_fail(e, "status");
  return CE_OK;
}

int commit_batch(ce_core* c) {
  GsState* g = c->gs;
  uint32_t hm[kMetaWords];
  int rc = read_meta(c, hm);
  if (rc) return rc;
  if (hm[4 + kGsCount] == 0 && hm[4 + kGsZero] == 0) return clear_batch(c);
  if ((rc = ensure_committed(c, hm[kGsCount], hm[4 + kGsCount]))) return rc;
  hipError_t e;
  const int t = c->ctx->tbegin("gset_commit");
  if ((e = launch_gs_move(c->ctx->stream, batch(g), committed(g)))) return c->ctx->hip_fail(e, "gset commit");
  c->ctx->tend(t);
  return clear_batch(c);
}

bool read_members(Rd& r, std::vector<uint64_t>* out) {
  uint64_t cnt;
  if (!rd_array_hdr(r, &cnt) || cnt > r.n - r.i) return false;
  out->reserve(out->size() + cnt);
  for (uint64_t k = 0; k < cnt; k++) {
    uint64_t v;
    if (!rd_u64(r, &v)) return false;
    out->push_back(v);
  }
  return true;
}

}

bool parse_gset_ops(const uint8_t* p, size_t n, std::vector<uint64_t>* out) {
  Rd r{p, n, 0};
  return read_members(r, out);
}

bool read_gset_state(Rd& r, std::vector<uint64_t>* out) {
  return read_struct(r, {"value"}, [&](int, Rd& q) { return read_members(q, out); });
}

void write_gset_state(Wr* w, const std::vector<uint64_t>& sorted_members) {
  w->map(1);
  w->str("value");
  w->arr(sorted_members.size());
  for (uint64_t v : sorted_members) w->uint(v);
}

int gs_init(ce_core* c) {
  GsState* g = c->gs = new GsState();
  uint32_t cap = 1u << 16;
  if (const char* e = getenv("CE_GSET_CAP")) cap = pow2_at_least((uint64_t)std::max(1l, atol(e)));
  g->cap = g->bcap = cap;
  hipError_t e;
  hipStream_t s = c->ctx->stream;
// ... 555 lines not shown
  const uint64_t v0 = c->nov[slot];
  if (c->storage) {
    std::vector<uint8_t> out(total);
    std::vector<uint64_t> fo(F + 1);
    if ((e = hipMemcpyAsync(out.data(), d_files, total, hipMemcpyDeviceToHost, s)) ||
        (e = hipMemcpyAsync(fo.data(), d_file_offs, 8ull * (F + 1), hipMemcpyDeviceToHost, s)) || (e = stream_wait(s)))
      return ctx->hip_fail(e, "gset apply download");
    for (uint32_t i = 0; i < F; i++)
      if ((rc = storage_store_op(c->storage, c->local_actor, v0 + i, out.data() + fo[i], fo[i + 1] - fo[i])))
        return ctx->fail(rc, "failed writing ops file");
  }
  t = ctx->tbegin("gset_apply_insert");
  if ((e = launch_gs_insert(s, committed(g), col, n))) return ctx->hip_fail(e, "gset apply insert");
  ctx->tend(t);
  if ((e = stream_wait(s))) return ctx->hip_fail(e, "gset apply insert");
  slot = c->slot_of.at(c->local_actor);
  c->nov[slot] = v0 + F;
  c->path_counts["gset_apply_device_files"] += F;
  c->path_counts["gset_apply_device_members"] += n;
  *n_files = F;
  *bytes = total;
  return table_upload(c);
}

namespace {

struct GsGate {
  std::vector<uint32_t> wslot;
  uint64_t gen0 = 0;
  std::vector<uint64_t> expect;
  uint32_t first_gap = 0xffffffffu;
  bool gap = false;
};

int prepare_ingest(ce_core* c, uint32_t n, uint64_t blob_len, const uint8_t* actors, uint32_t m, GsGate* gt) {
  ce_ctx* ctx = c->ctx;
  GsState* g = c->gs;
  hipError_t e;
  int rc;
  gt->wslot.resize(m);
  gt->gen0 = c->table_gen;
  for (uint32_t a = 0; a < m; a++) {
    Uuid u;
    std::memcpy(u.data(), actors + 16ull * a, 16);
    if ((rc = insert_actor(c, u, &gt->wslot[a]))) return rc;
  }
  if (c->table_gen != gt->gen0) refresh_slots(c, actors, m, &gt->wslot);
  if ((rc = table_upload(c)) || (rc = ensure_supported(c))) return rc;
  if ((e = ctx->out.reserve(blob_len + 16ull * n + 128)) || (e = ctx->status.reserve(n * 4ull + 64)) ||
      (e = ctx->apply.reserve(n + 64)) || (e = g->only.reserve(n + 64)))
    return ctx->hip_fail(e, "ingest reserve");
  if (g->batch_dirty && (rc = clear_batch(c))) return rc;
  gt->expect.resize(m);
  for (uint32_t a = 0; a < m; a++) gt->expect[a] = c->nov[gt->wslot[a]];
  return CE_OK;
}

int gate_host(ce_core* c, uint32_t n, uint32_t m, const uint32_t* d_fa, const uint64_t* d_fv, GsGate* gt) {
  ce_ctx* ctx = c->ctx;
  hipError_t e;
  std::vector<uint32_t> fa(n);
  std::vector<uint64_t> fv(n);
  std::vector<uint8_t> ap(n);
  if ((e = hipMemcpyAsync(fa.data(), d_fa, n * 4ull, hipMemcpyDeviceToHost, ctx->stream)) ||
      (e = hipMemcpyAsync(fv.data(), d_fv, n * 8ull, hipMemcpyDeviceToHost, ctx->stream)) ||
      (e = stream_wait(ctx->stream)))
    return ctx->hip_fail(e, "gate");
  for (uint32_t i = 0; i < n; i++)
    if (fa[i] >= m) return ctx->fail(CE_ERR_INVALID_ARG, "file_actor out of range");
  gt->first_gap = host_gate(fa.data(), fv.data(), n, &gt->expect, ap.data());
  if ((e = hipMemcpyAsync(ctx->apply.p, ap.data(), n, hipMemcpyHostToDevice, ctx->stream)) ||
      (e = stream_wait(ctx->stream)))
    return ctx->hip_fail(e, "gate");
  return CE_OK;
}

int fold_batch(ce_core* c, const uint8_t* d_blob, const uint64_t* d_offs, uint32_t n, uint64_t blob_len,
               int32_t* status_out) {
  ce_ctx* ctx = c->ctx;
  GsState* g = c->gs;
  hipError_t e;
  int rc;
  uint32_t ec = 0;
  if ((rc = device_open_setup(ctx, d_blob, d_offs, n, blob_len, true, key_of(c), ctx->status.as<int32_t>(), &ec)))
    return rc;
  uint32_t* paths = g->meta.as<uint32_t>() + 12;
  g->h_fused = GsFused{committed(g), batch(g), paths};
  if ((e = g->fused.reserve(sizeof(GsFused))) || (e = hipMemsetAsync(paths, 0, 12, ctx->stream)) ||
      (e = hipMemcpyAsync(g->fused.p, &g->h_fused, sizeof(GsFused), hipMemcpyHostToDevice, ctx->stream)))
    return ctx->hip_fail(e, "gset fused args");
  DecodeArgs da{};
  da.pt = ctx->out.as<uint8_t>();
  da.blob = d_blob;
  da.params = ctx->params.as<FileParams>();
  da.status = ctx->status.as<int32_t>();
  da.n = n;
  da.supported = c->d_supported.as<uint8_t>();
  da.n_supported = (uint32_t)c->supported.size();
  da.apply = ctx->apply.as<uint8_t>();
  da.counters = ctx->counters.as<uint32_t>();
  da.aux = ctx->poly_aux.as<PolyAux>();
  da.gs = g->fused.as<GsFused>();
  ctx->open_log.grid_cap = test_grid_cap();
  ctx->open_log.stamps = test_wave_stamps(ctx);
  ctx->open_log.stamp_waves = 0;
  {
    hipEvent_t t0, t1;
    (void)ctx->tlaunch("open_fold_small", &t0, &t1);
    if ((e = launch_open_fold_gset(ctx->stream, da, ctx->open_log, t0, t1))) return ctx->hip_fail(e, "fused");
  }
  g->batch_dirty = true;
  const SegScratch sc = segscratch(ctx, ec);
  int t = ctx->tbegin("segments_open");
  if ((e = launch_segments(ctx->stream, false, d_blob, ctx->out.as<uint8_t>(), ctx->params.as<FileParams>(), n,
                           ctx->status.as<int32_t>(), sc, grid_waves_for(n + ec), true)))
    return ctx->hip_fail(e, "open segments");
  ctx->tend(t);
  t = ctx->tbegin("finalize_open");
  if ((e = launch_finalize_multi(ctx->stream, false, ctx->out.as<uint8_t>(), ctx->params.as<FileParams>(),
                                 ctx->status.as<int32_t>(), sc, n)))
    return ctx->hip_fail(e, "open finalize");
  ctx->tend(t);
  count_open_launches(c, ctx);
  uint32_t hm[kMetaWords], hc[16];
  if ((e = hipMemcpyAsync(hc, ctx->counters.p, 64, hipMemcpyDeviceToHost, ctx->stream))) return ctx->hip_fail(e, "counters");
  if ((rc = read_meta(c, hm))) return rc;
  std::vector<int32_t> st;
  if (hm[4 + kGsOverflow]) {
    if ((e = hipMemsetAsync(g->meta.as<uint32_t>() + 4 + kGsOverflow, 0, 4, ctx->stream))) return ctx->hip_fail(e, "gset grow");
    if ((rc = rehash(c, true, g->bcap * 2)) ||
        (rc = device_open(ctx, d_blob, d_offs, n, blob_len, true, key_of(c), ctx->out.as<uint8_t>(),
                          ctx->status.as<int32_t>(), false, true)))
      return rc;
    count_open_launches(c, ctx);
    c->path_counts["gset_refolds"]++;
    if ((rc = download_status(c, n, &st))) return rc;
    if (std::find(st.begin(), st.end(), kStatusHostParse) != st.end()) {
      if ((rc = resolve_host_parse(c, d_blob, d_offs, n, true))) return rc;
    }
    if ((rc = decode_pass(c, n, nullptr)) || (rc = download_status(c, n, &st))) return rc;
  } else {
    c->path_counts["gset_fused_files"] += hm[14];
    c->path_counts["gset_uniform_files"] += hm[12];
    c->path_counts["gset_general_files"] += hm[13];
    if (hc[9] && (rc = decode_pass(c, n, nullptr, true))) return rc;
    if ((rc = download_status(c, n, &st))) return rc;
    if (std::find(st.begin(), st.end(), kStatusHostParse) != st.end()) {
      std::vector<uint8_t> sel(n);
      for (uint32_t i = 0; i < n; i++) sel[i] = st[i] == kStatusHostParse;
      if ((rc = resolve_host_parse(c, d_blob, d_offs, n, true))) return rc;
      if ((e = hipMemcpyAsync(g->only.p, sel.data(), n, hipMemcpyHostToDevice, ctx->stream)) ||
          (e = stream_wait(ctx->stream)))
        return ctx->hip_fail(e, "host parse mask");
      if ((rc = decode_pass(c, n, g->only.as<uint8_t>())) || (rc = download_status(c, n, &st))) return rc;
    }
  }
  if ((c->flags & CE_OPEN_MULTI_KEY) && !c->alt_keys.empty()) {
    bool any_auth = false, only_auth = true;
    for (int32_t s : st) {
      any_auth |= s == CE_ERR_AUTH;
      only_auth &= s == CE_OK || s == CE_ERR_AUTH;
    }
    if (any_auth && only_auth) {
      std::vector<int32_t> sk;
      std::vector<uint8_t> sel(n);
      for (const AltKey& ak : c->alt_keys) {
        if (std::find(st.begin(), st.end(), (int32_t)CE_ERR_AUTH) == st.end()) break;
        const KeyRef kr{ak.version, ak.key.data(), ak.key.size()};
        if ((rc = device_open(ctx, d_blob, d_offs, n, blob_len, true, kr, ctx->out.as<uint8_t>(),
                              ctx->status.as<int32_t>(), false)) ||
            (rc = download_status(c, n, &sk)))
          return rc;
        bool opened = false;
        for (uint32_t i = 0; i < n; i++) opened |= (sel[i] = st[i] == CE_ERR_AUTH && sk[i] == CE_OK) != 0;
        if (!opened) continue;
        if ((e = hipMemcpyAsync(g->only.p, sel.data(), n, hipMemcpyHostToDevice, ctx->stream)) ||
            (e = stream_wait(ctx->stream)))
          return ctx->hip_fail(e, "multi-key mask");
        if ((rc = decode_pass(c, n, g->only.as<uint8_t>())) || (rc = download_status(c, n, &sk))) return rc;
        for (uint32_t i = 0; i < n; i++)
          if (sel[i]) st[i] = sk[i];
      }
    }
  }
// ... 217 lines not shown
```

### crdt-enc_amd/csrc/ce_internal.h

```cpp
#pragma once
#include <utility>
#include <hip/hip_runtime.h>
#include <hsa/hsa.h>
#include <sched.h>

#include <array>
#include <cstring>
#include <mutex>
#include <string>
#include <unordered_map>
#include <functional>
#include <vector>

#include "ce_common.h"
#include "ce_kernels.h"
#include "crdtenc.h"

namespace ce {

using Uuid = std::array<uint8_t, 16>;

struct UuidHash {
  size_t operator()(const Uuid& u) const {
    uint32_t w[4];
// ... 32 lines not shown
  size_t cap = 0;
  HostBuf() = default;
  HostBuf(const HostBuf&) = delete;
  HostBuf& operator=(const HostBuf&) = delete;
  HostBuf(HostBuf&& o) noexcept : p(o.p), cap(o.cap) { o.p = nullptr; o.cap = 0; }
  HostBuf& operator=(HostBuf&& o) noexcept {
    std::swap(p, o.p);
    std::swap(cap, o.cap);
    return *this;
  }
  hipError_t reserve(size_t bytes);
  ~HostBuf();
  template <typename T>
  T* as() const { return reinterpret_cast<T*>(p); }
};

inline hipError_t stream_wait(hipStream_t s) {
  static const bool yield = getenv("CE_SYNC_YIELD") != nullptr;
  if (yield) return hipStreamSynchronize(s);
  thread_local hipEvent_t evs[64] = {};
  int dev = 0;
  hipError_t e;
  if ((e = hipGetDevice(&dev))) return e;
  if (dev < 0 || dev >= 64) return hipStreamSynchronize(s);
  hipEvent_t& ev = evs[dev];
  if (!ev && (e = hipEventCreateWithFlags(&ev, hipEventDisableTiming))) return e;
  if ((e = hipEventRecord(ev, s))) return e;
  for (unsigned i = 0; (e = hipEventQuery(ev)) == hipErrorNotReady; i++)
    if (i >= 32) sched_yield();
  return e;
}

inline hipError_t stream_mark(hipStream_t s, hipEvent_t* out) {
  thread_local hipEvent_t evs[64] = {};
  int dev = 0;
  hipError_t e;
  if ((e = hipGetDevice(&dev))) return e;
  if (dev < 0 || dev >= 64) return hipErrorInvalidDevice;
  hipEvent_t& ev = evs[dev];
  if (!ev && (e = hipEventCreateWithFlags(&ev, hipEventDisableTiming))) return e;
  *out = ev;
  return hipEventRecord(ev, s);
}

inline hipError_t mark_wait(hipEvent_t ev) {
  hipError_t e;
  for (unsigned i = 0; (e = hipEventQuery(ev)) == hipErrorNotReady; i++)
    if (i >= 32) sched_yield();
  return e;
}

struct KeyRef {
  const uint8_t* version;
  const uint8_t* key;
  size_t len;
};

struct OpenResult {
  uint32_t auth_failed = 0;
  uint32_t first_fail = 0xffffffffu;
};

}

namespace ce {
struct Uploader;
struct HostPool;
}

struct ce_storage {
  std::string local, remote;
};

struct ce_ctx {
  int device = 0;
  hipStream_t stream = nullptr;
  bool own_stream = false;
  std::recursive_mutex mu;
  std::string last_error;
  ce::DevBuf params, status, counters, extra, multi, partials, large, out, apply, refold, miss,
      supported, blob, offs, nonces, out_offs, outer_ver, batch_counters, split, segrec, redo, heads,
      poly_aux,
      stamps;
  ce::OpenLaunchLog open_log;
  ce::HostBuf h_counters, h_apply, h_stage, h_stage2, h_heads;
  uint32_t publish_gen = 0;
  hipEvent_t setup_ev = nullptr;
  hipStream_t side = nullptr;
  hipEvent_t side_ev = nullptr;
  hipEvent_t up_ev = nullptr;
  ce::Uploader* up = nullptr;
  ce::HostPool* pool = nullptr;
  bool timing = false;
  struct TimedLaunch {
    const char* name;
    hipEvent_t a, b;
  };
  std::vector<TimedLaunch> timed;
  std::vector<hipEvent_t> event_pool;
  hipEvent_t take_event() {
    if (!event_pool.empty()) {
      hipEvent_t e = event_pool.back();
      event_pool.pop_back();
      return e;
    }
    hipEvent_t e = nullptr;
    (void)hipEventCreate(&e);
    return e;
  }
  std::string timing_only;
  int tbegin(const char* name) {
    if (!timing || (!timing_only.empty() && timing_only != name)) return -1;
    TimedLaunch t{name, take_event(), take_event()};
    (void)hipEventRecord(t.a, stream);
    timed.push_back(t);
    return (int)timed.size() - 1;
  }
  void tend(int idx) {
    if (idx >= 0) (void)hipEventRecord(timed[idx].b, stream);
  }
  int tlaunch(const char* name, hipEvent_t* a, hipEvent_t* b) {
    *a = *b = nullptr;
    if (!timing || (!timing_only.empty() && timing_only != name)) return -1;
    TimedLaunch t{name, take_event(), take_event()};
    *a = t.a;
    *b = t.b;
    timed.push_back(t);
    return (int)timed.size() - 1;
  }

  hipEvent_t spin_ev = nullptr;
  hipError_t sync_spin() {
    static const bool yield = getenv("CE_SYNC_YIELD") != nullptr;
    if (yield) return hipStreamSynchronize(stream);
    hipError_t e;
    if (!spin_ev && (e = hipEventCreateWithFlags(&spin_ev, hipEventDisableTiming))) return e;
    if ((e = hipEventRecord(spin_ev, stream))) return e;
    for (unsigned i = 0; (e = hipEventQuery(spin_ev)) == hipErrorNotReady; i++)
      if (i >= 32) sched_yield();
    return e;
  }

  int fail(int code, const std::string& msg) {
    last_error = msg;
    return code;
  }
  int hip_fail(hipError_t e, const char* where) {
    last_error = std::string(where) + ": " + hipGetErrorString(e);
    return CE_ERR_DEVICE;
  }
};

namespace ce {

int32_t key_status(const KeyRef& k);
DevKey dev_key(const KeyRef& k);

int device_open_setup(ce_ctx* ctx, const uint8_t* d_blob, const uint64_t* d_offs, uint32_t n,
                      uint64_t blob_len, bool outer, const KeyRef& key, int32_t* d_status,
                      uint32_t* extra_cap, FillArgs* fills = nullptr,
                      const std::function<int()>* after_fill = nullptr);
SegScratch segscratch(ce_ctx* ctx, uint32_t extra_cap);
int device_open(ce_ctx* ctx, const uint8_t* d_blob, const uint64_t* d_offs, uint32_t n,
                uint64_t blob_len, bool outer, const KeyRef& key, uint8_t* d_out,
                int32_t* d_status, bool sync_counters, bool small_lanes = false,
                const DecodeArgs* ds = nullptr);

int device_seal(ce_ctx* ctx, const uint8_t* d_clear, const uint64_t* d_offs, uint32_t n,
                uint64_t clear_len_total, const uint8_t* d_outer_version, const uint8_t* d_nonces,
                uint8_t* d_out, const uint64_t* d_out_offs, const KeyRef& key, bool counters_ready = false);
uint32_t* ctx_counters(ce_ctx* ctx);

int seal_one(ce_ctx* ctx, const KeyRef& key, const uint8_t* outer_version, const uint8_t* nonce,
             const uint8_t* clear, size_t clear_len, std::vector<uint8_t>* file,
             const uint8_t* prefix16 = nullptr);

uint32_t grid_waves_for(uint32_t work);
uint32_t test_grid_cap();
unsigned long long* test_wave_stamps(ce_ctx* ctx);

struct DmaD2H {
  bool ok = false;
  hsa_agent_t gpu{0}, cpu{0};
  uint32_t engine = 0;
};
bool dma_init(int device, DmaD2H* out);
bool dma_d2h(const DmaD2H& d, void* dst, const void* src, size_t n, hsa_signal_t sig);
void dma_wait(hsa_signal_t sig);
bool dma_signal(hsa_signal_t* sig);
void dma_signal_destroy(hsa_signal_t sig);

int stage_host_batch(ce_ctx* ctx, const uint8_t* const* files, const uint64_t* offs, uint32_t n);
void destroy_uploader(ce_ctx* ctx);
void host_parallel_for(ce_ctx* ctx, uint32_t n, const std::function<void(uint32_t)>& fn);

}
```

### crdt-enc_amd/csrc/ce_kernels.h

```cpp
#pragma once
#include <hip/hip_runtime.h>
#include <stdint.h>

#include "ce_common.h"

namespace ce {

static constexpr uint32_t kPageBytes = 4096;
static constexpr uint32_t kSegPages = 4;
static constexpr uint32_t kSegBlocks = kSegPages * kPageBytes / 16;
static constexpr uint32_t kSmallMax = kPageBytes;

struct alignas(16) FileParams {
  uint32_t subkey[8];
  uint32_t n2[2];
  uint32_t pad0[2];
  uint32_t s[4];
  uint32_t tag[4];
  uint32_t rpow[7][5];
  uint32_t pad1;
  uint64_t in_off;
  uint64_t out_off;
  uint32_t len;
  int32_t status;
  uint32_t nseg;
  uint32_t extra_base;
};
static_assert(sizeof(FileParams) == 256, "FileParams layout");

struct alignas(16) PolyAux {
  uint32_t r3[5];
  uint32_t r12[5];
  uint32_t r48[5];
  uint32_t e6[5];
  uint32_t lr[5];
  uint32_t ts[4];
  uint32_t pad[3];
};
static_assert(sizeof(PolyAux) == 128, "PolyAux layout");

struct DevKey {
  uint32_t k[8];
};

struct SegScratch {
  uint32_t* counters;
  uint2* extra_list;
  uint32_t extra_cap;
  uint32_t* multi_files;
  uint32_t* partials;
  uint32_t* large_list;
  uint32_t seg_blocks;
};

static constexpr int kMaxFill = 10;
struct FillRange {
  uint32_t* p;
  uint64_t words;
  uint32_t value;
  const uint32_t* src = nullptr;
};
struct FillArgs {
  FillRange r[kMaxFill];
  int n;
  uint32_t* counters;
};
hipError_t launch_fill(hipStream_t s, const FillArgs& a);
hipError_t launch_publish_words(hipStream_t s, const uint32_t* src, uint32_t n, uint32_t* dst, uint32_t gen);
hipError_t launch_publish_sealed_len(hipStream_t s, const uint64_t* clear_len_at, uint64_t bound, uint64_t cap,
                                     uint64_t* len_out);

hipError_t launch_open_setup(hipStream_t s, const uint8_t* blob, const uint64_t* offs,
                             uint32_t n, bool outer, DevKey key, int32_t key_status,
                             FileParams* params, int32_t* status, SegScratch sc,
                             PolyAux* aux = nullptr);
hipError_t launch_seal_setup(hipStream_t s, const uint8_t* clear, const uint64_t* offs,
                             uint32_t n, const uint8_t* outer_version ,
                             const uint8_t* nonces, uint8_t* out, const uint64_t* out_offs,
                             DevKey key, FileParams* params, SegScratch sc);
hipError_t launch_segments(hipStream_t s, bool seal, const uint8_t* in, uint8_t* out,
                           const FileParams* params, uint32_t n, int32_t* status, SegScratch sc,
                           uint32_t grid_waves, bool skip_small = false);
hipError_t launch_finalize_multi(hipStream_t s, bool seal, uint8_t* out, const FileParams* params,
                                 int32_t* status, SegScratch sc, uint32_t n);

static constexpr uint32_t kDsFuseRegion = 2048;
struct DsFuse {
  int on;
  uint32_t rows;
  uint32_t* rawcnt;
  uint8_t* done;
  uint32_t* add_actor;
  unsigned long long* add_ctr;
  unsigned long long* add_mem;
  uint32_t* rm_actor;
  unsigned long long* rm_ctr;
  unsigned long long* rm_mem;
  uint32_t* why;
  uint8_t* big;
};

struct DecodeArgs {
  const uint8_t* pt;
  const FileParams* params;
  int32_t* status;
  uint32_t n;
  const uint8_t* supported;
  uint32_t n_supported;
  const uint8_t* apply;
  const ActorSlot* table;
  uint32_t mask;
  unsigned long long* batch;
  uint32_t* counters;
  union {
    uint4* miss_list;
    const struct GsFused* gs;
    const struct LwwFused* lw;
  };
  uint32_t miss_cap;
  uint8_t* refold;
  const uint8_t* only;
  int large_only;
  const uint32_t* large_list;
  const uint8_t* blob;
  uint8_t* redo;
  int nil_actor;
  DsFuse ds;
  const PolyAux* aux;
  unsigned long long* stamps;
};
static constexpr uint32_t kTicketWord = 32;
#ifndef CE_DYN_CHUNK
#define CE_DYN_CHUNK 4u
#endif
#ifndef CE_DYN_STATIC_PCT
#define CE_DYN_STATIC_PCT 50u
#endif
static_assert(CE_DYN_CHUNK >= 1 && CE_DYN_CHUNK <= 64 && CE_DYN_STATIC_PCT <= 100, "k_open_fold_v3 schedule");
static constexpr uint32_t kStampWords = 4;
static constexpr uint32_t kStampWaves = 16384;
hipError_t launch_decode_dots(hipStream_t s, const DecodeArgs& a, uint32_t grid_waves);
hipError_t launch_decode_pn_ops(hipStream_t s, const DecodeArgs& a, uint32_t grid_waves);
hipError_t launch_clock_probe(hipStream_t s, unsigned long long* out, uint32_t blocks,
                              uint32_t samples, uint32_t ticks);

static constexpr uint32_t kSplitParts = 16;
static constexpr uint32_t kSplitMinDots = 2048;
static constexpr uint32_t kSplitDone = 0xfffffffeu;
struct SplitScratch {
  uint4* part;
};
hipError_t launch_decode_split(hipStream_t s, const DecodeArgs& a, SplitScratch sp, uint32_t n_large);
hipError_t launch_segments_decode(hipStream_t s, const uint8_t* in, uint8_t* out, const DecodeArgs& da,
                                  SegScratch sc, uint32_t grid_waves, uint4* rec);
hipError_t launch_segdec_apply(hipStream_t s, const DecodeArgs& a, SegScratch sc, const uint4* rec,
                               uint32_t n_large);

struct OpenLaunchLog {
  uint32_t grid_cap = 0;
  uint32_t n = 0;
  const char* took[8];
  void note(const char* key) {
    if (n < 8) took[n++] = key;
  }
  uint32_t grid(uint32_t blocks, const char* key) {
    note(key);
    if (grid_cap == 0 || blocks <= grid_cap) return blocks;
    note("open_grid_capped");
    return grid_cap;
  }
  unsigned long long* stamps = nullptr;
  uint32_t stamp_waves = 0;
  DecodeArgs stamped(const DecodeArgs& a, uint32_t blocks) {
    DecodeArgs b = a;
    b.stamps = blocks <= kStampWaves ? stamps : nullptr;
    stamp_waves = b.stamps ? blocks : 0;
    return b;
  }
};

hipError_t launch_open_fold_small(hipStream_t s, const DecodeArgs& a, int files_per_wave, OpenLaunchLog& log);
hipError_t launch_open_fold_v2(hipStream_t s, const DecodeArgs& a, int files_per_wave, OpenLaunchLog& log,
                               hipEvent_t t0 = nullptr, hipEvent_t t1 = nullptr);
hipError_t launch_open_fold_pn(hipStream_t s, const DecodeArgs& a, OpenLaunchLog& log,
                               hipEvent_t t0 = nullptr, hipEvent_t t1 = nullptr);
hipError_t launch_open_fold_gset(hipStream_t s, const DecodeArgs& a, OpenLaunchLog& log,
                                 hipEvent_t t0 = nullptr, hipEvent_t t1 = nullptr);
hipError_t launch_open_fold_lww(hipStream_t s, const DecodeArgs& a, OpenLaunchLog& log,
                                hipEvent_t t0 = nullptr, hipEvent_t t1 = nullptr);
hipError_t launch_open_small_v2(hipStream_t s, const DecodeArgs& a, OpenLaunchLog& log);

struct GateArgs {
  const uint32_t* fa;
  const uint64_t* fv;
  uint32_t n, m;
  const uint64_t* e0;
  uint32_t* run_count;
  uint32_t* run_first;
  uint32_t* flags;
  unsigned long long* newnov;
  uint8_t* apply;
  unsigned long long* newnov_host;
};
hipError_t launch_gate(hipStream_t s, const GateArgs& g);

hipError_t launch_merge_max(hipStream_t s, unsigned long long* dst,
                            const unsigned long long* src, uint32_t n);
hipError_t launch_sum_u64_128(hipStream_t s, const unsigned long long* planes, uint32_t cap, uint32_t n_planes,
                              unsigned long long* out);
hipError_t launch_gather_u64(hipStream_t s, const unsigned long long* src, const uint32_t* idx, uint32_t m,
                             unsigned long long* dst);
hipError_t launch_merge_max_if(hipStream_t s, unsigned long long* dst, const unsigned long long* src,
                               uint32_t n, const uint32_t* counters);
hipError_t launch_nov_apply(hipStream_t s, unsigned long long* nov, const uint32_t* wslot,
                            const unsigned long long* newnov, uint32_t m, const uint32_t* counters);
hipError_t launch_serialize_vclock(hipStream_t s, const unsigned long long* nov,
                                  const unsigned long long* st, const uint32_t* sorted, uint32_t k,
                                  const ActorSlot* table, bool gcounter, const uint8_t* prefix16,
                                  uint8_t* out, unsigned long long* offs, uint32_t pn_cap = 0);
inline uint64_t vclock_ser_bound(uint64_t k, bool pn = false) {
  const uint64_t two = 16 + 24 + 5 + 27 * k + 19 + 5 + 27 * k;
  return pn ? two + 3 + 15 + 5 + 27 * k : two;
}

struct CompactArgs {
  uint8_t nonce[24];
  uint8_t outer[16];
  uint8_t prefix[16];
};
hipError_t launch_compact_prologue(hipStream_t s, uint8_t* args, const CompactArgs& ca, uint32_t* seal_counters,
                                   unsigned long long* nov, const uint32_t* wslot,
                                   const unsigned long long* newnov, uint32_t m, const uint32_t* counters,
                                   unsigned long long* merge_dst = nullptr,
                                   const unsigned long long* merge_src = nullptr, uint32_t merge_n = 0);
hipError_t launch_tail_pack(hipStream_t s, uint8_t* dst, const unsigned long long* src_len,
                            const uint32_t* counters, const unsigned long long* newnov, uint32_t m);

struct GatherRange {
  const uint8_t* src;
  uint64_t dst_off, len;
};
hipError_t launch_gather_ranges(hipStream_t s, uint8_t* dst, const GatherRange* r, uint32_t n);

hipError_t launch_state_heads(hipStream_t s, const FileParams* params, const int32_t* status,
                              const uint8_t* out, uint32_t n, uint8_t* dst);

}
```

### crdt-enc_amd/csrc/ce_kernels.hip

```cpp
#include "ce_device.h"

namespace ce {

__global__ __launch_bounds__(256) void k_open_setup(const uint8_t* __restrict__ blob,
                                                    const uint64_t* __restrict__ offs, uint32_t n,
                                                    int outer, DevKey key, int32_t key_status,
                                                    FileParams* __restrict__ params,
                                                    int32_t* __restrict__ status, SegScratch sc,
                                                    PolyAux* __restrict__ aux) {
  __shared__ uint4 stage[256 * 8];
  const uint32_t f = blockIdx.x * blockDim.x + threadIdx.x;
  const bool active = f < n;
  const uint64_t off = active ? offs[f] : 0;
  const uint64_t flen = active ? offs[f + 1] - off : 0;
  const uint8_t* enc = blob + off;
  uint64_t enc_len = flen;
  int32_t st = active ? CE_OK : CE_ERR_OUTER_LEN;
  if (active && outer) {
    if (flen < 16) st = CE_ERR_OUTER_LEN;
    else {
      const uint4 v = *reinterpret_cast<const uint4*>(enc);
      auto le = [](int i) {
        return (uint32_t)kCoreVersion[4 * i] | ((uint32_t)kCoreVersion[4 * i + 1] << 8) |
               ((uint32_t)kCoreVersion[4 * i + 2] << 16) | ((uint32_t)kCoreVersion[4 * i + 3] << 24);
      };
      if (v.x != le(0) || v.y != le(1) || v.z != le(2) || v.w != le(3)) st = CE_ERR_OUTER_VERSION;
      enc += 16;
      enc_len -= 16;
    }
  }
  if (st == CE_OK) st = key_status;
  Envelope e{};
  bool fast = false;
  uint32_t nw[6];
  if (st == CE_OK && enc_len >= 67 + 16) {
    uint32_t w[17];
#pragma unroll
    for (int i = 0; i < 4; i++) {
      const uint4 v = *reinterpret_cast<const uint4*>(enc + 16 * i);
      w[4 * i] = v.x; w[4 * i + 1] = v.y; w[4 * i + 2] = v.z; w[4 * i + 3] = v.w;
    }
    w[16] = ld_le32(enc + 64);
    auto byte = [&](int i) -> uint32_t { return (w[i >> 2] >> (8 * (i & 3))) & 0xffu; };
    bool ok = byte(0) == 0x92 && byte(1) == 0xc4 && byte(2) == 0x10 && byte(19) == 0xc5 &&
              byte(22) == 0x82 && byte(23) == 0xa5 && byte(24) == 'n' && byte(25) == 'o' &&
              byte(26) == 'n' && byte(27) == 'c' && byte(28) == 'e' && byte(29) == 0xc4 &&
              byte(30) == 0x18 && byte(55) == 0xa8 && byte(56) == 'e' && byte(57) == 'n' &&
              byte(58) == 'c' && byte(59) == '_' && byte(60) == 'd' && byte(61) == 'a' &&
              byte(62) == 't' && byte(63) == 'a' && byte(64) == 0xc5;
#pragma unroll
    for (int i = 0; i < 16; i++) ok = ok && byte(3 + i) == kBoxVersion[i];
    const uint32_t eb = (byte(20) << 8) | byte(21);
    const uint32_t l2 = (byte(65) << 8) | byte(66);
    if (ok && eb == 45 + l2 && 22ull + eb <= enc_len && l2 >= 16) {
      e.nonce_off = 31; e.nonce_len = 24; e.enc_off = 67; e.enc_len = l2;
      fast = true;
#pragma unroll
      for (int k = 0; k < 6; k++) nw[k] = __builtin_amdgcn_alignbyte(w[8 + k], w[7 + k], 3);
    }
  }
  if (st == CE_OK && !fast) st = parse_envelope(enc, enc_len, &e);
  FileParams P;
  P.status = st;
  P.len = 0;
  P.in_off = 0;
  P.out_off = (off + 15) & ~15ull;
  P.nseg = 0;
  P.extra_base = 0;
  if (st == CE_OK) {
    const uint64_t ct_off = (uint64_t)(enc - blob) + e.enc_off;
    P.in_off = ct_off;
    P.len = (uint32_t)(e.enc_len - 16);
    const uint4 t = *reinterpret_cast<const uint4*>(blob + ct_off + P.len);
    P.tag[0] = t.x; P.tag[1] = t.y; P.tag[2] = t.z; P.tag[3] = t.w;
    if (!fast) {
#pragma unroll
      for (int k = 0; k < 6; k++) nw[k] = ld_le32(enc + e.nonce_off + 4 * k);
    }
    key_schedule_w(key, nw, P);
    if (P.len > kSmallMax) sc.large_list[atomicAdd(&sc.counters[9], 1u)] = f;
  }
  reserve_segments(P, f, sc, st == CE_OK);
  PolyAux X;
  if (aux) {
    if (st == CE_OK) poly_aux(P, X);
    else X = PolyAux{};
  }
  {
    const uint4* pv = reinterpret_cast<const uint4*>(&P);
    const uint4* xv = reinterpret_cast<const uint4*>(&X);
    const uint32_t f0 = blockIdx.x * blockDim.x;
    const uint32_t nrow = min(n - f0, (uint32_t)blockDim.x);
    uint4* dstp = reinterpret_cast<uint4*>(params + f0);
    uint4* dsta = aux ? reinterpret_cast<uint4*>(aux + f0) : nullptr;
#pragma unroll
    for (int h = 0; h < 3; h++) {
      if (h == 2 && !aux) break;
      if (h) __syncthreads();
#pragma unroll
      for (int i = 0; i < 8; i++) stage[threadIdx.x * 8 + (i ^ (threadIdx.x & 7))] = h < 2 ? pv[8 * h + i] : xv[i];
      __syncthreads();
#pragma unroll
      for (int k = 0; k < 8; k++) {
        const uint32_t j = threadIdx.x + 256u * k;
        const uint32_t row = j >> 3, col = j & 7;
        if (row < nrow) {
          const uint4 v = stage[row * 8 + (col ^ (row & 7))];
          if (h < 2) dstp[row * 16 + 8 * h + col] = v;
          else dsta[row * 8 + col] = v;
        }
      }
    }
  }
  if (!active) return;
  status[f] = st;
  const uint32_t lane = threadIdx.x & 63;
  const unsigned long long hp = __ballot(active && st == kStatusHostParse);
  const unsigned long long bad = __ballot(active && st != CE_OK && st != kStatusHostParse);
  if (hp && lane == (uint32_t)__builtin_ctzll(hp)) atomicAdd(&sc.counters[7], (uint32_t)__builtin_popcountll(hp));
  if (bad && lane == (uint32_t)__builtin_ctzll(bad)) {
    atomicAdd(&sc.counters[8], (uint32_t)__builtin_popcountll(bad));
    atomicMin(&sc.counters[5], f);
  }
}

__global__ __launch_bounds__(256) void k_seal_setup(const uint8_t* __restrict__ clear,
                                                    const uint64_t* __restrict__ offs, uint32_t n,
                                                    const uint8_t* __restrict__ outer_version,
                                                    const uint8_t* __restrict__ nonces,
                                                    uint8_t* __restrict__ out,
                                                    const uint64_t* __restrict__ out_offs,
                                                    DevKey key, FileParams* __restrict__ params,
                                                    SegScratch sc) {
  const uint32_t f = blockIdx.x * blockDim.x + threadIdx.x;
  const bool mine = f < n;
  FileParams P;
  P.len = 0;
  if (mine) {
    const uint64_t off = offs[f];
    const uint64_t len = offs[f + 1] - off;
    uint8_t* o = out + out_offs[f];
    uint64_t k = 0;
    if (outer_version) {
#pragma unroll
      for (int i = 0; i < 16; i++) o[i] = outer_version[i];
      k = 16;
    }
    const uint8_t* nonce = nonces + 24ull * f;
    uint8_t nb[24];
#pragma unroll
    for (int i = 0; i < 24; i++) nb[i] = nonce[i];
    const uint64_t h = put_envelope_header(o + k, len, nb);
    P.status = CE_OK;
    P.in_off = off;
    P.out_off = out_offs[f] + k + h;
    P.len = (uint32_t)len;
    key_schedule(key, nb, P);
  }
  reserve_segments(P, f, sc, mine);
  if (mine) params[f] = P;
}

static constexpr int kWavesPerBlock = 4;
static constexpr uint32_t kSegBytes = kSegBlocks * 16;

template <bool PN = false>
__device__ void decode_file(const DecodeArgs& a, uint32_t f, uint32_t lane);

__device__ __forceinline__ void dot_window(const uint8_t* pt, uint32_t p, uint32_t (&w)[12]) {
  const uint4 A = *reinterpret_cast<const uint4*>(pt + p);
  const uint4 B = *reinterpret_cast<const uint4*>(pt + p + 16);
  const uint4 C = *reinterpret_cast<const uint4*>(pt + p + 32);
  w[0] = A.x; w[1] = A.y; w[2] = A.z; w[3] = A.w;
  w[4] = B.x; w[5] = B.y; w[6] = B.z; w[7] = B.w;
  w[8] = C.x; w[9] = C.y; w[10] = C.z; w[11] = C.w;
}

struct SlotCache {
  uint32_t c0 = 0, c1 = 0, c2 = 0, c3 = 0, slot = 0xffffffffu;
  __device__ __forceinline__ uint32_t get(const DecodeArgs& a, uint32_t k0, uint32_t k1, uint32_t k2, uint32_t k3) {
    if (slot != 0xffffffffu && k0 == c0 && k1 == c1 && k2 == c2 && k3 == c3) return slot;
    const uint32_t s = lookup_slot1(a.table, a.mask, a.nil_actor, k0, k1, k2, k3);
    if (s != 0xffffffffu) { c0 = k0; c1 = k1; c2 = k2; c3 = k3; slot = s; }
    return s;
  }
};

__device__ void seg_record(const DecodeArgs& a, const uint8_t* pt, uint32_t len, uint32_t S,
                           uint32_t E, uint32_t lane, uint4* rec) {
  uint32_t m = 0xffffffffu, L = 0, hcount = 0, hok = 0;
  if (S == 0) {
    uint32_t hm = 0xffffffffu, hl = 0;
    if (lane == 0 && len >= 16) {
      const uint4 dv = *reinterpret_cast<const uint4*>(pt);
      bool found = false;
// ... 461 lines not shown
          continue;
        }
        const uint32_t L2 = PN ? (pos + 39 <= blen ? pn_len_of_marker(body[pos + 38]) : 0)
                               : (pos + 34 <= blen ? dot_len_of_marker(body[pos + 33]) : 0);
        if (L2 != 0 && L2 != L) {
          L = L2;
          in = load(pos, remaining);
          continue;
        }
        int ok = 0;
        uint32_t g0 = 0, g1 = 0, g2 = 0, g3 = 0;
        unsigned long long gc = 0;
        uint32_t npos = pos;
        if (lane == 0) {
          Rd q{body, blen, pos};
          uint64_t aoff = 0, c = 0;
          if constexpr (PN) ok = parse_pn_op(q, &aoff, &c, &dir);
          else ok = parse_dot(q, &aoff, &c);
          if (ok == 1) {
            g0 = ld_le32(body + aoff); g1 = ld_le32(body + aoff + 4);
            g2 = ld_le32(body + aoff + 8); g3 = ld_le32(body + aoff + 12);
            gc = c;
            npos = (uint32_t)q.i;
          }
        }
        ok = __shfl(ok, 0);
        if (ok != 1) { st = CE_ERR_DECODE; break; }
        npos = bcast(npos);
        if (do_fold && lane == 0) fold_dot(g0, g1, g2, g3, gc, dir);
        pos = npos;
        remaining -= 1;
        L = PN ? (remaining > 0 && pos + 39 <= blen ? pn_len_of_marker(body[pos + 38]) : 0)
               : (remaining > 0 && pos + 34 <= blen ? dot_len_of_marker(body[pos + 33]) : 0);
        in = load(pos, remaining);
      }
      if (do_fold) {
        const uint32_t hi = pslot == 0xffffffffu ? 0u : pslot + 1;
        const uint32_t lo = pslot == 0xffffffffu ? 0xffffffffu : pslot + 1;
        uint32_t mx = hi, mn = lo;
        unsigned long long b = pslot == 0xffffffffu ? 0ull : pbest;
#pragma unroll
        for (int d = 32; d >= 1; d >>= 1) {
          const uint32_t omx = (uint32_t)__shfl_xor((int)mx, d), omn = (uint32_t)__shfl_xor((int)mn, d);
          const unsigned long long ob = __shfl_xor(b, d);
          mx = omx > mx ? omx : mx;
          mn = omn < mn ? omn : mn;
          b = ob > b ? ob : b;
        }
        if (mx != 0 && mn == mx) {
          if (lane == 0) batch_max(&a.batch[mx - 1], b);
        } else if (pslot != 0xffffffffu) {
          batch_max(&a.batch[pslot], pbest);
        }
      }
    }
    if (st != CE_OK && lane == 0) {
      a.status[f] = st;
      atomicAdd(&a.counters[3], 1u);
      atomicMin(&a.counters[5], f);
    }
  }
}


__global__ __launch_bounds__(256) void k_decode_pn_ops(DecodeArgs a) {
  const uint32_t lane = threadIdx.x & 63;
  const uint32_t stride = gridDim.x * kWavesPerBlock;
  const uint32_t nwork = (a.large_only && !a.only) ? *((volatile uint32_t*)&a.counters[9]) : a.n;
  if (a.large_only && !a.only) {
    for (;;) {
      uint32_t w = 0;
      if (lane == 0) w = atomicAdd(&a.counters[15], 1u);
      w = __shfl(w, 0);
      if (w >= nwork) break;
      const uint32_t f = bcast(a.large_list[w]);
      const FileParams* Pp = a.params + f;
      if (Pp->len <= kSmallMax || a.status[f] != CE_OK) continue;
      decode_file<true>(a, f, lane);
    }
    return;
  }
  for (uint32_t w = bcast(blockIdx.x * kWavesPerBlock + (threadIdx.x >> 6)); w < nwork; w += stride) {
    const uint32_t f = w;
    const FileParams* Pp = a.params + f;
    if ((a.only && !a.only[f]) || (a.large_only && Pp->len <= kSmallMax)) continue;
    if (a.status[f] != CE_OK) continue;
    decode_file<true>(a, f, lane);
  }
}

__global__ __launch_bounds__(256) void k_decode_dots(DecodeArgs a) {
  const uint32_t lane = threadIdx.x & 63;
  const uint32_t stride = gridDim.x * kWavesPerBlock;
  const uint32_t nwork = (a.large_only && !a.only) ? *((volatile uint32_t*)&a.counters[9]) : a.n;
  if (a.large_only && !a.only) {
    for (;;) {
      uint32_t w = 0;
      if (lane == 0) w = atomicAdd(&a.counters[15], 1u);
      w = __shfl(w, 0);
      if (w >= nwork) break;
      const uint32_t f = bcast(a.large_list[w]);
      const FileParams* Pp = a.params + f;
      if (Pp->len <= kSmallMax || a.status[f] != CE_OK) continue;
      decode_file(a, f, lane);
    }
    return;
  }
  for (uint32_t w = bcast(blockIdx.x * kWavesPerBlock + (threadIdx.x >> 6)); w < nwork; w += stride) {
    const uint32_t f = w;
    const FileParams* Pp = a.params + f;
    if ((a.only && !a.only[f]) || (a.large_only && Pp->len <= kSmallMax)) continue;
    if (a.status[f] != CE_OK) continue;
    decode_file(a, f, lane);
  }
}

__global__ __launch_bounds__(256) void k_decode_split(DecodeArgs a, SplitScratch sp) {
  const uint32_t lane = threadIdx.x & 63;
  const uint32_t stride = gridDim.x * kWavesPerBlock;
  const uint32_t nl = *((volatile uint32_t*)&a.counters[9]);
  for (uint32_t item = bcast(blockIdx.x * kWavesPerBlock + (threadIdx.x >> 6)); item < nl * kSplitParts;
       item += stride) {
    const uint32_t w = item / kSplitParts, part = item % kSplitParts;
    const uint32_t f = bcast(a.large_list[w]);
    const FileParams* Pp = a.params + f;
    if (Pp->len <= kSmallMax || a.status[f] != CE_OK) continue;
    const uint8_t* pt = a.pt + Pp->out_off;
    const uint32_t len = Pp->len;
    bool split = len >= 16 && (a.apply == nullptr || a.apply[f]);
    uint32_t count = 0, pos0 = 0, L = 0;
    const uint8_t* body = pt + 16;
    const uint32_t blen = split ? len - 16 : 0;
    if (split) {
      const uint4 dv = *reinterpret_cast<const uint4*>(pt);
      bool found = false;
      for (uint32_t s = 0; s < a.n_supported; s++) {
        const uint4 sv = *reinterpret_cast<const uint4*>(a.supported + 16 * s);
        found |= dv.x == sv.x && dv.y == sv.y && dv.z == sv.z && dv.w == sv.w;
      }
      Rd r{body, blen, 0};
      uint64_t c64 = 0;
      split = found && rd_array_hdr(r, &c64) && c64 <= blen && c64 >= kSplitMinDots;
      if (split) {
        count = (uint32_t)c64;
        pos0 = (uint32_t)r.i;
        L = pos0 + 34 <= blen ? dot_len_of_marker(body[pos0 + 33]) : 0;
        split = L != 0;
      }
    }
    if (!split) {
      if (part == 0) {
        decode_file(a, f, lane);
        if (lane == 0) sp.part[item] = make_uint4(kSplitDone, 0u, 0u, 0u);
      }
      continue;
    }
    const uint32_t D = ((count + kSplitParts - 1) / kSplitParts + 63) & ~63u;
    const uint32_t d0 = min(part * D, count), d1 = min(d0 + D, count);
    bool fail = false;
    uint32_t myslot = 0xffffffffu, cslot = 0xffffffffu, c0 = 0, c1 = 0, c2 = 0, c3 = 0;
    unsigned long long best = 0;
    for (uint32_t i = d0; i < d1; i += 64) {
      const uint32_t k = i + lane;
      const uint64_t cand = pos0 + (uint64_t)k * L;
      const bool in = k < d1 && cand + L <= blen;
      const uint8_t* q = body + (in ? cand : 0u);
      const uint4 A = *reinterpret_cast<const uint4*>(q);
      const uint4 B = *reinterpret_cast<const uint4*>(q + 16);
      const uint4 C = *reinterpret_cast<const uint4*>(q + 32);
      uint32_t k0 = 0, k1 = 0, k2 = 0, k3 = 0;
      unsigned long long ctr = 0;
      bool valid = false;
      if (in) {
        const uint32_t wv[12] = {A.x, A.y, A.z, A.w, B.x, B.y, B.z, B.w, C.x, C.y, C.z, C.w};
        valid = canon_dot(wv, L, k0, k1, k2, k3, ctr);
      }
      if (k < d1 && !valid) fail = true;
      if (valid) {
        uint32_t slot;
        if (cslot != 0xffffffffu && k0 == c0 && k1 == c1 && k2 == c2 && k3 == c3) slot = cslot;
        else {
          slot = lookup_slot1(a.table, a.mask, a.nil_actor, k0, k1, k2, k3);
          c0 = k0; c1 = k1; c2 = k2; c3 = k3; cslot = slot;
        }
        if (slot == 0xffffffffu || (myslot != 0xffffffffu && slot != myslot)) fail = true;
        else {
          best = (myslot == 0xffffffffu || ctr > best) ? ctr : best;
          myslot = slot;
        }
      }
    }
    uint32_t mx = myslot == 0xffffffffu ? 0u : myslot + 1;
    uint32_t mn = myslot == 0xffffffffu ? 0xffffffffu : myslot + 1;
    unsigned long long bm = best;
// ... 289 lines not shown
      o = out + q_hdr;
      o += mp_put_str(o, "n", 1);
      *o++ = 0x81;
      o += mp_put_str(o, "inner", 5);
      *o++ = 0x81;
      o += mp_put_str(o, "dots", 4);
      o += mp_put_map_hdr(o, cq);
      offs[0] = 0;
      offs[1] = q_at + tbq;
    }
  } else
  if (me == 0 && t == 0) {
    uint8_t* o = out;
    for (uint32_t i = 0; i < pl; i++) *o++ = prefix16[i];
    *o++ = 0x82;
    o += mp_put_str(o, "next_op_versions", 16);
    *o++ = 0x81;
    o += mp_put_str(o, "dots", 4);
    o += mp_put_map_hdr(o, cn);
    o = out + st_hdr;
    o += mp_put_str(o, "state", 5);
    if (gcounter) {
      *o++ = 0x81;
      o += mp_put_str(o, "inner", 5);
    }
    *o++ = 0x81;
    o += mp_put_str(o, "dots", 4);
    o += mp_put_map_hdr(o, cs);
    offs[0] = 0;
    offs[1] = st_at + tbs;
  }
  auto put = [&](uint32_t at, const ActorSlot& a, unsigned long long v) {
    const uint32_t ul = mp_uint_len(v);
    const uint32_t nb = ul - 1;
    const unsigned long long be = nb ? __builtin_bswap64(v) >> (8 * (8 - nb)) : 0ull;
    const uint32_t mk = ul == 2 ? 0xccu : ul == 3 ? 0xcdu : ul == 5 ? 0xceu : 0xcfu;
    const unsigned long long lo = ul == 1 ? v : (mk | (be << 8));
    const uint32_t hi = ul == 9 ? (uint32_t)(be >> 56) : 0u;
    const uint32_t t0 = (uint32_t)lo, t1 = (uint32_t)(lo >> 32);
    uint32_t w[7];
    w[0] = 0x10c4u | (a.k[0] << 16);
    w[1] = (a.k[0] >> 16) | (a.k[1] << 16);
    w[2] = (a.k[1] >> 16) | (a.k[2] << 16);
    w[3] = (a.k[2] >> 16) | (a.k[3] << 16);
    w[4] = (a.k[3] >> 16) | (t0 << 16);
    w[5] = (t0 >> 16) | (t1 << 16);
    w[6] = (t1 >> 16) | (hi << 16);
    const uint32_t len = 18 + ul, nd = len >> 2;
    uint8_t* o = out + at;
#pragma unroll
    for (uint32_t q = 0; q < 7; q++)
      if (q < nd) *reinterpret_cast<uint32_t*>(o + 4 * q) = w[q];
    const uint32_t tail = w[nd < 7 ? nd : 6];
    for (uint32_t b = 4 * nd; b < len; b++) o[b] = (uint8_t)(tail >> (8 * (b & 3)));
  };
  {
    const uint32_t i = me * 1024 + t;
    const uint32_t slot = i < k ? sorted[i] : 0xffffffffu;
    const unsigned long long vn = slot != 0xffffffffu ? nov[slot] : 0ull;
    const unsigned long long vs = slot != 0xffffffffu ? st[slot] : 0ull;
    const uint32_t ln = vn != 0 ? 18u + mp_uint_len(vn) : 0u;
    const uint32_t ls = vs != 0 ? 18u + mp_uint_len(vs) : 0u;
    unsigned long long vq = 0;
    uint32_t lq = 0;
    if constexpr (PN) {
      vq = slot != 0xffffffffu ? st[slot + pn_cap] : 0ull;
      lq = vq != 0 ? 18u + mp_uint_len(vq) : 0u;
    }
    ActorSlot a;
    if (ln | ls | lq) a = table[slot];
    uint32_t tot;
    const uint32_t at = block_scan_1024(ln | (ls << 16), ws, &tot);
    if (ln) put(nov_at + tpn + (at & 0xffff), a, vn);
    if (ls) put(st_at + tps + (at >> 16), a, vs);
    if constexpr (PN) {
      const uint32_t atq = block_scan_1024(lq, ws, &tot);
      if (lq) put(q_at + tpq + atq, a, vq);
    }
  }
}

hipError_t launch_open_setup(hipStream_t s, const uint8_t* blob, const uint64_t* offs, uint32_t n,
                             bool outer, DevKey key, int32_t key_status, FileParams* params,
                             int32_t* status, SegScratch sc, PolyAux* aux) {
  if (n == 0) return hipSuccess;
  hipLaunchKernelGGL(k_open_setup, dim3((n + 255) / 256), dim3(256), 0, s, blob, offs, n,
                     outer ? 1 : 0, key, key_status, params, status, sc, aux);
  return hipGetLastError();
}

__global__ void k_fill(FillArgs a) {
  const uint32_t r = blockIdx.y;
  if ((int)r == a.n) {
    if (blockIdx.x == 0 && threadIdx.x < 16)
      a.counters[threadIdx.x] = (threadIdx.x == 5 || threadIdx.x == 13) ? 0xffffffffu : 0u;
    if (blockIdx.x == 0 && threadIdx.x == kTicketWord) a.counters[kTicketWord] = 0u;
    return;
  }
  const FillRange f = a.r[r];
  const uint64_t t0 = blockIdx.x * (uint64_t)blockDim.x + threadIdx.x, ts = (uint64_t)gridDim.x * blockDim.x;
  const uint64_t head = ((16 - (reinterpret_cast<uintptr_t>(f.p) & 15)) & 15) / 4;
  const bool vec = (reinterpret_cast<uintptr_t>(f.p) & 3) == 0 &&
                   (!f.src || ((reinterpret_cast<uintptr_t>(f.src) ^ reinterpret_cast<uintptr_t>(f.p)) & 15) == 0) &&
                   f.words > head + 4;
  if (!vec) {
    for (uint64_t i = t0; i < f.words; i += ts) f.p[i] = f.src ? f.src[i] : f.value;
    return;
  }
  const uint64_t body = (f.words - head) / 4, tail0 = head + 4 * body;
  uint4* p4 = reinterpret_cast<uint4*>(f.p + head);
  if (f.src) {
    const uint4* s4 = reinterpret_cast<const uint4*>(f.src + head);
    for (uint64_t i = t0; i < body; i += ts) p4[i] = s4[i];
  } else {
    const uint4 v = make_uint4(f.value, f.value, f.value, f.value);
    for (uint64_t i = t0; i < body; i += ts) p4[i] = v;
  }
  if (t0 < head) f.p[t0] = f.src ? f.src[t0] : f.value;
  if (t0 < f.words - tail0) f.p[tail0 + t0] = f.src ? f.src[tail0 + t0] : f.value;
}

__global__ void k_publish_sealed_len(const uint64_t* clear_len_at, uint64_t bound, uint64_t cap, uint64_t* len_out) {
  const uint64_t cl = *clear_len_at;
  const uint64_t total = 16 + sealed_len(cl);
  *reinterpret_cast<volatile uint64_t*>(len_out) = cl > bound ? ~1ull : total > cap ? ~0ull : total;
}

__global__ void k_publish_words(const uint32_t* src, uint32_t n, uint32_t* dst, uint32_t gen) {
  if (threadIdx.x < n) reinterpret_cast<volatile uint32_t*>(dst)[threadIdx.x] = src[threadIdx.x];
  __threadfence_system();
  if (threadIdx.x == 0) reinterpret_cast<volatile uint32_t*>(dst)[n] = gen;
}

hipError_t launch_publish_words(hipStream_t s, const uint32_t* src, uint32_t n, uint32_t* dst, uint32_t gen) {
  if (n > 64) return hipErrorInvalidValue;
  hipLaunchKernelGGL(k_publish_words, dim3(1), dim3(64), 0, s, src, n, dst, gen);
  return hipGetLastError();
}

hipError_t launch_publish_sealed_len(hipStream_t s, const uint64_t* clear_len_at, uint64_t bound, uint64_t cap,
                                     uint64_t* len_out) {
  hipLaunchKernelGGL(k_publish_sealed_len, dim3(1), dim3(1), 0, s, clear_len_at, bound, cap, len_out);
  return hipGetLastError();
}

hipError_t launch_fill(hipStream_t s, const FillArgs& a) {
  uint64_t mx = 16;
  for (int i = 0; i < a.n; i++) mx = a.r[i].words > mx ? a.r[i].words : mx;
  const uint32_t gx = (uint32_t)std::min<uint64_t>((mx / 4 + 255) / 256, 1024);
  hipLaunchKernelGGL(k_fill, dim3(gx, a.n + (a.counters ? 1 : 0)), dim3(256), 0, s, a);
  return hipGetLastError();
}

hipError_t launch_seal_setup(hipStream_t s, const uint8_t* clear, const uint64_t* offs, uint32_t n,
                             const uint8_t* outer_version, const uint8_t* nonces, uint8_t* out,
                             const uint64_t* out_offs, DevKey key, FileParams* params,
                             SegScratch sc) {
  if (n == 0) return hipSuccess;
  hipLaunchKernelGGL(k_seal_setup, dim3((n + 255) / 256), dim3(256), 0, s, clear, offs, n,
                     outer_version, nonces, out, out_offs, key, params, sc);
  return hipGetLastError();
}

hipError_t launch_segments(hipStream_t s, bool seal, const uint8_t* in, uint8_t* out,
                           const FileParams* params, uint32_t n, int32_t* status, SegScratch sc,
                           uint32_t grid_waves, bool skip_small) {
  if (n == 0) return hipSuccess;
  const uint32_t blocks = (grid_waves + kWavesPerBlock - 1) / kWavesPerBlock;
  if (seal)
    hipLaunchKernelGGL((k_segments<true, false>), dim3(blocks), dim3(256), 0, s, in, out, params, n,
// ... 305 lines not shown
```

### crdt-enc_amd/csrc/ce_lww.h

```cpp
#pragma once
#include <hip/hip_runtime.h>
#include <stdint.h>

#include "ce_common.h"
#include "ce_kernels.h"

namespace ce {

template <typename R>
CE_HD int parse_lww_op(R& r, uint64_t* val, uint64_t* marker) {
  static constexpr const char* kF[2] = {"val", "marker"};
  if (r.i >= r.n) return 0;
  const uint8_t m = rb(r, r.i);
  uint64_t cnt;
  const bool arr = is_array_marker(m);
  if (arr) {
    if (!rd_array_hdr(r, &cnt) || cnt != 2) return 0;
  } else if (!rd_map_hdr(r, &cnt)) {
    return 0;
  }
  unsigned seen = 0;
  for (uint64_t k = 0; k < cnt; k++) {
    int f = arr ? (int)k : rd_field<2>(r, kF);
    if (f < 0) return 0;
    if (f == 2) {
      int s = rd_skip(r);
      if (s <= 0) return s;
      continue;
    }
    if (seen & (1u << f)) return 0;
    seen |= 1u << f;
    if (!rd_u64(r, f == 0 ? val : marker)) return 0;
  }
  return seen == 3u ? 1 : 0;
}

CE_HD uint32_t lww_uint_width(uint8_t m) {
  return m <= 0x7f ? 1u : (m >= 0xcc && m <= 0xcf) ? 1u + (1u << (m - 0xcc)) : 0u;
}

struct LwwRec {
  unsigned long long marker, val;
};

struct LwwFused {
  LwwRec* rec;
  uint32_t* paths;
};

struct LwwDecodeArgs {
  const uint8_t* pt;
  const FileParams* params;
  int32_t* status;
  uint32_t n;
  const uint8_t* supported;
  uint32_t n_supported;
  const uint8_t* apply;
  const uint8_t* only;
  int large_only;
  LwwRec* rec;
  uint32_t* paths;
};

hipError_t launch_decode_lww(hipStream_t s, const LwwDecodeArgs& a, uint32_t grid_waves);

static constexpr uint32_t kLwwBlock = 256;
static constexpr uint32_t kLwwTile = 256;
static constexpr uint32_t kLwwMaxBlocks = 64;
struct LwwPartial {
  unsigned long long marker, val;
  uint32_t idx, pad;
};
hipError_t launch_lww_reduce(hipStream_t s, const LwwRec* rec, uint32_t n, LwwPartial* part, LwwRec* out,
                             uint32_t grid_cap);

struct LwwKeyed {
  unsigned long long marker, val, fa, fv;
};
static constexpr LwwKeyed kLwwKeyedNone = {0ull, 0ull, ~0ull, ~0ull};
struct LwwKeyedPartial {
  unsigned long long marker, val, fv;
  uint32_t fa, idx;
};
CE_HD bool lww_keyed_better(unsigned long long ma, unsigned long long faa, unsigned long long fva, uint32_t ia,
                            unsigned long long mb, unsigned long long fab, unsigned long long fvb, uint32_t ib) {
  if (ma != mb) return ma > mb;
  if (faa != fab) return faa < fab;
  if (fva != fvb) return fva < fvb;
  return ia < ib;
}
hipError_t launch_lww_reduce_keyed(hipStream_t s, const LwwRec* rec, const uint32_t* fa, const uint64_t* fv,
                                   uint32_t n, LwwKeyedPartial* part, LwwKeyed* out, uint32_t grid_cap);

}
```

### crdt-enc_amd/csrc/ce_lww.hip

```cpp
#include <hip/hip_runtime.h>
#include <stdint.h>

#include "ce_lww.h"

namespace ce {
namespace {

constexpr int kWaves = 4;

__device__ __forceinline__ bool lww_better(unsigned long long ma, uint32_t ia, unsigned long long mb, uint32_t ib) {
  return ma > mb || (ma == mb && ia < ib);
}

__device__ __forceinline__ unsigned long long shfl_xor64(unsigned long long v, int d) {
  const uint32_t lo = (uint32_t)__shfl_xor((int)(uint32_t)v, d);
  const uint32_t hi = (uint32_t)__shfl_xor((int)(uint32_t)(v >> 32), d);
  return ((unsigned long long)hi << 32) | lo;
}

__device__ __forceinline__ void wave_best(unsigned long long& m, uint32_t& i, unsigned long long& v) {
#pragma unroll
  for (int d = 32; d >= 1; d >>= 1) {
    const unsigned long long om = shfl_xor64(m, d), ov = shfl_xor64(v, d);
    const uint32_t oi = (uint32_t)__shfl_xor((int)i, d);
// ... 20 lines not shown
  *marker = lww_uint(k + 7, wm);
  return true;
}

__device__ void decode_lww_file(const LwwDecodeArgs& a, uint32_t f, uint32_t lane) {
  const FileParams* Pp = a.params + f;
  const uint8_t* pt = a.pt + Pp->out_off;
  const uint32_t len = Pp->len;
  int32_t st = CE_OK;
  if (len < 16) st = CE_ERR_PT_LEN;
  else {
    const uint4 dv = *reinterpret_cast<const uint4*>(pt);
    bool found = false;
    for (uint32_t s = 0; s < a.n_supported; s++) {
      const uint4 sv = *reinterpret_cast<const uint4*>(a.supported + 16 * s);
      found |= dv.x == sv.x && dv.y == sv.y && dv.z == sv.z && dv.w == sv.w;
    }
    if (!found) st = CE_ERR_PT_VERSION;
  }
  unsigned long long bm = 0, bv = 0;
  uint32_t bi = 0xffffffffu;
  if (st == CE_OK) {
    const uint8_t* body = pt + 16;
    const uint32_t blen = len - 16;
    uint32_t cnt = 0, h = 0;
    if (blen == 0) st = CE_ERR_DECODE;
    else {
      const uint32_t m = body[0];
      if ((m & 0xf0) == 0x90) { cnt = m & 15; h = 1; }
      else if (m == 0xdc && blen >= 3) { cnt = (uint32_t)body[1] << 8 | body[2]; h = 3; }
      else if (m == 0xdd && blen >= 5) {
        cnt = (uint32_t)body[1] << 24 | (uint32_t)body[2] << 16 | (uint32_t)body[3] << 8 | body[4];
        h = 5;
      } else st = CE_ERR_DECODE;
      if (st == CE_OK && cnt > blen - h) st = CE_ERR_DECODE;
    }
    if (st == CE_OK) {
      uint32_t wv = 0, wm = 0, stride = 0;
      if (cnt > 0 && blen - h >= 14) {
        wv = lww_uint_width(body[h + 5]);
        if (wv && h + 12 + wv < blen) wm = lww_uint_width(body[h + 12 + wv]);
        if (wv && wm) stride = 12 + wv + wm;
        if (stride && (unsigned long long)cnt * stride > blen - h) stride = 0;
      }
      bool ok = stride != 0;
      if (stride)
        for (uint32_t e = lane; e < cnt && ok; e += 64) {
          unsigned long long v, m;
          ok = lww_elem_fixed(body + h + (unsigned long long)e * stride, wv, wm, &v, &m);
          if (ok && m > bm) { bm = m; bv = v; bi = e; }
        }
      const bool uniform = cnt == 0 || __ballot(ok) == ~0ull;
      if (uniform) {
        if (lane == 0) atomicAdd(&a.paths[0], 1u);
        wave_best(bm, bi, bv);
      } else {
        if (lane == 0) {
          atomicAdd(&a.paths[1], 1u);
          bm = 0;
          bv = 0;
          Rd q{body, blen, h};
          for (uint32_t e = 0; e < cnt; e++) {
            uint64_t v = 0, m = 0;
            if (parse_lww_op(q, &v, &m) != 1) { st = CE_ERR_DECODE; break; }
            if (m > bm) { bm = m; bv = v; }
          }
        }
      }
    }
  }
  if (lane == 0) {
    atomicAdd(&a.paths[3], 1u);
    if (st != CE_OK) a.status[f] = st;
    const bool win = st == CE_OK && a.apply[f] && bm != 0;
    a.rec[f] = LwwRec{win ? bm : 0ull, win ? bv : 0ull};
  }
}

__global__ __launch_bounds__(256) void k_decode_lww(LwwDecodeArgs a) {
  const uint32_t lane = threadIdx.x & 63;
  const uint32_t stride = gridDim.x * kWaves;
  for (uint32_t f = __builtin_amdgcn_readfirstlane(blockIdx.x * kWaves + (threadIdx.x >> 6)); f < a.n; f += stride) {
    if (a.only && !a.only[f]) continue;
    if (a.large_only && a.params[f].len <= kSmallMax) continue;
    if (a.status[f] != CE_OK) continue;
    decode_lww_file(a, f, lane);
  }
}

__device__ __forceinline__ void block_best(unsigned long long& m, uint32_t& i, unsigned long long& v) {
  __shared__ unsigned long long s_m[kLwwBlock / 64], s_v[kLwwBlock / 64];
  __shared__ uint32_t s_i[kLwwBlock / 64];
  wave_best(m, i, v);
  const uint32_t w = threadIdx.x >> 6;
  if ((threadIdx.x & 63) == 0) { s_m[w] = m; s_v[w] = v; s_i[w] = i; }
  __syncthreads();
  if (threadIdx.x == 0)
    for (uint32_t k = 1; k < kLwwBlock / 64; k++)
      if (lww_better(s_m[k], s_i[k], m, i)) { m = s_m[k]; i = s_i[k]; v = s_v[k]; }
}

__global__ __launch_bounds__(kLwwBlock) void k_lww_reduce(const LwwRec* rec, uint32_t n, LwwPartial* part) {
  static_assert(kLwwTile % kLwwBlock == 0, "a tile is whole rounds of the block");
  unsigned long long bm = 0, bv = 0;
  uint32_t bi = 0xffffffffu;
  const uint32_t tiles = (uint32_t)(((unsigned long long)n + kLwwTile - 1) / kLwwTile);
  for (uint32_t t = blockIdx.x; t < tiles; t += gridDim.x) {
    const unsigned long long base = (unsigned long long)t * kLwwTile;
#pragma unroll
    for (uint32_t r = 0; r < kLwwTile / kLwwBlock; r++) {
      const unsigned long long i = base + r * kLwwBlock + threadIdx.x;
      if (i < n) {
        const LwwRec x = rec[i];
        if (lww_better(x.marker, (uint32_t)i, bm, bi)) { bm = x.marker; bv = x.val; bi = (uint32_t)i; }
      }
    }
  }
  block_best(bm, bi, bv);
  if (threadIdx.x == 0) part[blockIdx.x] = LwwPartial{bm, bv, bi, 0};
}

__global__ __launch_bounds__(kLwwBlock) void k_lww_reduce_final(const LwwPartial* part, uint32_t k, LwwRec* out) {
  unsigned long long bm = 0, bv = 0;
  uint32_t bi = 0xffffffffu;
  for (uint32_t j = threadIdx.x; j < k; j += kLwwBlock) {
    const LwwPartial p = part[j];
    if (lww_better(p.marker, p.idx, bm, bi)) { bm = p.marker; bv = p.val; bi = p.idx; }
  }
  block_best(bm, bi, bv);
  if (threadIdx.x == 0) out[0] = LwwRec{bm, bm ? bv : 0ull};
}

struct Keyed {
  unsigned long long m, v, fv;
  uint32_t fa, i;
};

__device__ __forceinline__ bool keyed_better(const Keyed& a, const Keyed& b) {
  return lww_keyed_better(a.m, a.fa, a.fv, a.i, b.m, b.fa, b.fv, b.i);
}

__device__ __forceinline__ void wave_best_keyed(Keyed& x) {
#pragma unroll
  for (int d = 32; d >= 1; d >>= 1) {
    Keyed o;
    o.m = shfl_xor64(x.m, d);
    o.v = shfl_xor64(x.v, d);
    o.fv = shfl_xor64(x.fv, d);
    o.fa = (uint32_t)__shfl_xor((int)x.fa, d);
    o.i = (uint32_t)__shfl_xor((int)x.i, d);
    if (keyed_better(o, x)) x = o;
  }
}

__device__ __forceinline__ void block_best_keyed(Keyed& x) {
  __shared__ Keyed s_k[kLwwBlock / 64];
  wave_best_keyed(x);
  const uint32_t w = threadIdx.x >> 6;
  if ((threadIdx.x & 63) == 0) s_k[w] = x;
  __syncthreads();
  if (threadIdx.x == 0)
    for (uint32_t k = 1; k < kLwwBlock / 64; k++)
      if (keyed_better(s_k[k], x)) x = s_k[k];
}

__global__ __launch_bounds__(kLwwBlock) void k_lww_reduce_keyed(const LwwRec* rec, const uint32_t* fa,
                                                                const uint64_t* fv, uint32_t n,
// ... 65 lines not shown
```

### crdt-enc_amd/csrc/ce_lww_host.cpp

```cpp
#include <algorithm>
#include <cstring>

#include "ce_core.h"
#include "ce_lww.h"

namespace ce {

struct LwState {
  uint64_t val = 0, marker = 0;
  DevBuf rec;
  DevBuf red;
  DevBuf fused;
  LwwFused h_fused;
  DevBuf only;
  DevBuf gate;
  DevBuf kred;
  LwwKeyed pend = kLwwKeyedNone;
};

void lw_free(LwState* l) { delete l; }

namespace {

constexpr uint64_t kResultAt = sizeof(LwwPartial) * kLwwMaxBlocks;
constexpr uint64_t kPathsAt = kResultAt + sizeof(LwwRec);

LwwRec* result_of(LwState* l) { return reinterpret_cast<LwwRec*>(l->red.as<uint8_t>() + kResultAt); }
uint32_t* paths_of(LwState* l) { return reinterpret_cast<uint32_t*>(l->red.as<uint8_t>() + kPathsAt); }

void update(LwState* l, uint64_t val, uint64_t marker) {
  if (l->marker < marker) {
    l->val = val;
    l->marker = marker;
  }
}

int download_status(ce_core* c, uint32_t n, std::vector<int32_t>* st) {
  st->resize(n);
  hipError_t e;
  if ((e = hipMemcpyAsync(st->data(), c->ctx->status.p, n * 4ull, hipMemcpyDeviceToHost, c->ctx->stream)) ||
      (e = stream_wait(c->ctx->stream)))
    return c->ctx->hip_fail(e, "status");
  return CE_OK;
}

int decode_pass(ce_core* c, uint32_t n, const uint8_t* only, bool large_only = false) {
  ce_ctx* ctx = c->ctx;
  LwState* l = c->lw;
  hipError_t e;
  LwwDecodeArgs a{};
  a.pt = ctx->out.as<uint8_t>();
  a.params = ctx->params.as<FileParams>();
  a.status = ctx->status.as<int32_t>();
  a.n = n;
  a.supported = c->d_supported.as<uint8_t>();
  a.n_supported = (uint32_t)c->supported.size();
  a.apply = ctx->apply.as<uint8_t>();
  a.only = only;
  a.large_only = large_only ? 1 : 0;
  a.rec = l->rec.as<LwwRec>();
  a.paths = paths_of(l);
  uint32_t hp[4];
  if ((e = hipMemsetAsync(a.paths, 0, 16, ctx->stream))) return ctx->hip_fail(e, "lww decode");
  const int t = ctx->tbegin("decode_lww");
  if ((e = launch_decode_lww(ctx->stream, a, grid_waves_for(n)))) return ctx->hip_fail(e, "lww decode");
  ctx->tend(t);
  if ((e = hipMemcpyAsync(hp, a.paths, 16, hipMemcpyDeviceToHost, ctx->stream)) || (e = stream_wait(ctx->stream)))
    return ctx->hip_fail(e, "lww decode");
  c->path_counts["lww_uniform_files"] += hp[0];
  c->path_counts["lww_general_files"] += hp[1];
  c->path_counts["lww_page_files"] += hp[3];
  return CE_OK;
}

bool read_reg(Rd& r, uint64_t* val, uint64_t* marker) { return parse_lww_op(r, val, marker) == 1; }

struct LwGate {
  std::vector<uint32_t> wslot;
  uint64_t gen0 = 0;
  std::vector<uint64_t> expect;
  uint32_t first_gap = 0xffffffffu;
};

int prepare_ingest(ce_core* c, uint32_t n, uint64_t blob_len, const uint8_t* actors, uint32_t m, LwGate* gt) {
  ce_ctx* ctx = c->ctx;
  LwState* l = c->lw;
  hipError_t e;
  int rc;
  gt->wslot.resize(m);
  gt->gen0 = c->table_gen;
  for (uint32_t a = 0; a < m; a++) {
    Uuid u;
    std::memcpy(u.data(), actors + 16ull * a, 16);
    if ((rc = insert_actor(c, u, &gt->wslot[a]))) return rc;
  }
  if (c->table_gen != gt->gen0) refresh_slots(c, actors, m, &gt->wslot);
  if ((rc = table_upload(c)) || (rc = ensure_supported(c))) return rc;
  if ((e = ctx->out.reserve(blob_len + 16ull * n + 128)) || (e = ctx->status.reserve(n * 4ull + 64)) ||
      (e = ctx->apply.reserve(n + 64)) || (e = l->only.reserve(n + 64)) ||
      (e = l->rec.reserve(sizeof(LwwRec) * (uint64_t)n + 64)) || (e = l->red.reserve(kPathsAt + 64)) ||
      (e = l->fused.reserve(sizeof(LwwFused))))
    return ctx->hip_fail(e, "ingest reserve");
  gt->expect.resize(m);
  for (uint32_t a = 0; a < m; a++) gt->expect[a] = c->nov[gt->wslot[a]];
  return CE_OK;
}

int gate_host(ce_core* c, uint32_t n, uint32_t m, const uint32_t* d_fa, const uint64_t* d_fv, LwGate* gt) {
  ce_ctx* ctx = c->ctx;
  hipError_t e;
  std::vector<uint32_t> fa(n);
  std::vector<uint64_t> fv(n);
  std::vector<uint8_t> ap(n);
  if ((e = hipMemcpyAsync(fa.data(), d_fa, n * 4ull, hipMemcpyDeviceToHost, ctx->stream)) ||
      (e = hipMemcpyAsync(fv.data(), d_fv, n * 8ull, hipMemcpyDeviceToHost, ctx->stream)) ||
      (e = stream_wait(ctx->stream)))
    return ctx->hip_fail(e, "gate");
  for (uint32_t i = 0; i < n; i++)
    if (fa[i] >= m) return ctx->fail(CE_ERR_INVALID_ARG, "file_actor out of range");
  gt->first_gap = host_gate(fa.data(), fv.data(), n, &gt->expect, ap.data());
  if ((e = hipMemcpyAsync(ctx->apply.p, ap.data(), n, hipMemcpyHostToDevice, ctx->stream)) ||
      (e = stream_wait(ctx->stream)))
    return ctx->hip_fail(e, "gate");
  return CE_OK;
}

int open_decode(ce_core* c, const uint8_t* d_blob, const uint64_t* d_offs, uint32_t n, uint64_t blob_len,
                int32_t* status_out) {
  ce_ctx* ctx = c->ctx;
  LwState* l = c->lw;
  hipError_t e;
  int rc;
  uint32_t ec = 0;
  if ((rc = device_open_setup(ctx, d_blob, d_offs, n, blob_len, true, key_of(c), ctx->status.as<int32_t>(), &ec)))
    return rc;
  uint32_t* paths = paths_of(l);
  l->h_fused = LwwFused{l->rec.as<LwwRec>(), paths};
  if ((e = hipMemsetAsync(l->rec.p, 0, sizeof(LwwRec) * (uint64_t)n, ctx->stream)) ||
      (e = hipMemsetAsync(paths, 0, 16, ctx->stream)) ||
      (e = hipMemcpyAsync(l->fused.p, &l->h_fused, sizeof(LwwFused), hipMemcpyHostToDevice, ctx->stream)))
    return ctx->hip_fail(e, "lww fused args");
  DecodeArgs da{};
  da.pt = ctx->out.as<uint8_t>();
  da.blob = d_blob;
  da.params = ctx->params.as<FileParams>();
  da.status = ctx->status.as<int32_t>();
  da.n = n;
  da.supported = c->d_supported.as<uint8_t>();
  da.n_supported = (uint32_t)c->supported.size();
  da.apply = ctx->apply.as<uint8_t>();
  da.counters = ctx->counters.as<uint32_t>();
  da.aux = ctx->poly_aux.as<PolyAux>();
  da.lw = l->fused.as<LwwFused>();
  ctx->open_log.grid_cap = test_grid_cap();
  ctx->open_log.stamps = test_wave_stamps(ctx);
  ctx->open_log.stamp_waves = 0;
  {
    hipEvent_t t0, t1;
    (void)ctx->tlaunch("open_fold_small", &t0, &t1);
    if ((e = launch_open_fold_lww(ctx->stream, da, ctx->open_log, t0, t1))) return ctx->hip_fail(e, "fused");
  }
  const SegScratch sc = segscratch(ctx, ec);
  int t = ctx->tbegin("segments_open");
  if ((e = launch_segments(ctx->stream, false, d_blob, ctx->out.as<uint8_t>(), ctx->params.as<FileParams>(), n,
                           ctx->status.as<int32_t>(), sc, grid_waves_for(n + ec), true)))
    return ctx->hip_fail(e, "open segments");
  ctx->tend(t);
  t = ctx->tbegin("finalize_open");
  if ((e = launch_finalize_multi(ctx->stream, false, ctx->out.as<uint8_t>(), ctx->params.as<FileParams>(),
                                 ctx->status.as<int32_t>(), sc, n)))
    return ctx->hip_fail(e, "open finalize");
  ctx->tend(t);
  count_open_launches(c, ctx);
  uint32_t hp[4], hc[16];
  if ((e = hipMemcpyAsync(hc, ctx->counters.p, 64, hipMemcpyDeviceToHost, ctx->stream)) ||
      (e = hipMemcpyAsync(hp, paths, 16, hipMemcpyDeviceToHost, ctx->stream)) || (e = stream_wait(ctx->stream)))
    return ctx->hip_fail(e, "counters");
  c->path_counts["lww_uniform_files"] += hp[0];
  c->path_counts["lww_general_files"] += hp[1];
  c->path_counts["lww_fused_files"] += hp[2];
  if (hc[9] && (rc = decode_pass(c, n, nullptr, true))) return rc;
  std::vector<int32_t> st;
  if ((rc = download_status(c, n, &st))) return rc;
  if (std::find(st.begin(), st.end(), kStatusHostParse) != st.end()) {
    std::vector<uint8_t> sel(n);
    for (uint32_t i = 0; i < n; i++) sel[i] = st[i] == kStatusHostParse;
    if ((rc = resolve_host_parse(c, d_blob, d_offs, n, true))) return rc;
    if ((e = hipMemcpyAsync(l->only.p, sel.data(), n, hipMemcpyHostToDevice, ctx->stream)) ||
        (e = stream_wait(ctx->stream)))
      return ctx->hip_fail(e, "host parse mask");
    if ((rc = decode_pass(c, n, l->only.as<uint8_t>())) || (rc = download_status(c, n, &st))) return rc;
  }
  if ((c->flags & CE_OPEN_MULTI_KEY) && !c->alt_keys.empty()) {
    bool any_auth = false, only_auth = true;
    for (int32_t s : st) {
      any_auth |= s == CE_ERR_AUTH;
      only_auth &= s == CE_OK || s == CE_ERR_AUTH;
    }
    if (any_auth && only_auth) {
      std::vector<int32_t> sk;
      std::vector<uint8_t> sel(n);
      for (const AltKey& ak : c->alt_keys) {
        if (std::find(st.begin(), st.end(), (int32_t)CE_ERR_AUTH) == st.end()) break;
        const KeyRef kr{ak.version, ak.key.data(), ak.key.size()};
        if ((rc = device_open(ctx, d_blob, d_offs, n, blob_len, true, kr, ctx->out.as<uint8_t>(),
                              ctx->status.as<int32_t>(), false)) ||
            (rc = download_status(c, n, &sk)))
          return rc;
        bool opened = false;
        for (uint32_t i = 0; i < n; i++) opened |= (sel[i] = st[i] == CE_ERR_AUTH && sk[i] == CE_OK) != 0;
        if (!opened) continue;
        if ((e = hipMemcpyAsync(l->only.p, sel.data(), n, hipMemcpyHostToDevice, ctx->stream)) ||
            (e = stream_wait(ctx->stream)))
          return ctx->hip_fail(e, "multi-key mask");
        if ((rc = decode_pass(c, n, l->only.as<uint8_t>())) || (rc = download_status(c, n, &sk))) return rc;
        for (uint32_t i = 0; i < n; i++)
          if (sel[i]) st[i] = sk[i];
      }
    }
  }
  if (status_out) std::memcpy(status_out, st.data(), n * 4ull);
  for (uint32_t i = 0; i < n; i++)
    if (st[i] != CE_OK) return st[i];
  return CE_OK;
}

int fold_batch(ce_core* c, const uint8_t* d_blob, const uint64_t* d_offs, uint32_t n, uint64_t blob_len,
               int32_t* status_out, LwwRec* win) {
  ce_ctx* ctx = c->ctx;
  LwState* l = c->lw;
  hipError_t e;
  int rc;
  if ((rc = open_decode(c, d_blob, d_offs, n, blob_len, status_out))) return rc;
  const int t = ctx->tbegin("lww_reduce");
  if ((e = launch_lww_reduce(ctx->stream, l->rec.as<LwwRec>(), n, l->red.as<LwwPartial>(), result_of(l),
// ... 176 lines not shown
```

Baseline: 380.1 million op files/s.

## Pack per-file open parameters into a single row struct for fused open kernels

The setup kernel now writes a compact OpenRow per file (subkey, nonce, offset, length, s, r-powers and precomputed poly powers) through an LDS-staged, coalesced store. The fused v3 open/fold kernel reads everything from this one row instead of gathering from both FileParams and PolyAux. Full FileParams are written only for failed or large files, and the tag-minus-s value is recomputed in the kernel from the ciphertext tail instead of being stored. The aim is less scattered global traffic in setup and decode, at the cost of a more complex setup kernel and an extra 128-bit subtraction per file.

```diff
diff --git a/crdt-enc_amd/csrc/ce_core.cpp b/crdt-enc_amd/csrc/ce_core.cpp
--- a/crdt-enc_amd/csrc/ce_core.cpp
+++ b/crdt-enc_amd/csrc/ce_core.cpp
@@ -766,6 +766,7 @@
     return CE_OK;
   };
   uint32_t ec;
+  const bool want_rows = pnc || (c->fused == 2 && c->files_per_wave != 1 && open_fold_v2_takes_rows(c->files_per_wave));
   {
     FillArgs fl{};
     fl.r[0] = {reinterpret_cast<uint32_t*>(gbase + 16ull * m), 4ull * m, 0u};
@@ -782,11 +783,11 @@
     if (!gate_after_setup) {
       const std::function<int()> gate = launch_gate_now;
       int rr = device_open_setup(ctx, d_blob, d_offs, n, blob_len, true, key, ctx->status.as<int32_t>(),
-                                 &ec, &fl, &gate);
+                                 &ec, want_rows, &fl, &gate);
       if (rr) return rr;
     } else {
       int rr = device_open_setup(ctx, d_blob, d_offs, n, blob_len, true, key, ctx->status.as<int32_t>(),
-                                 &ec, &fl);
+                                 &ec, want_rows, &fl);
       if (rr) return rr;
     }
   }
@@ -822,7 +823,7 @@
   da.pt = ctx->out.as<uint8_t>();
   da.blob = d_blob;
   da.params = ctx->params.as<FileParams>();
-  da.aux = ctx->poly_aux.as<PolyAux>();
+  da.rows = ctx->open_rows;
   da.status = ctx->status.as<int32_t>();
   da.n = n;
   da.supported = c->d_supported.as<uint8_t>();
diff --git a/crdt-enc_amd/csrc/ce_ctx.cpp b/crdt-enc_amd/csrc/ce_ctx.cpp
--- a/crdt-enc_amd/csrc/ce_ctx.cpp
+++ b/crdt-enc_amd/csrc/ce_ctx.cpp
@@ -121,7 +121,8 @@
 
 int device_open_setup(ce_ctx* ctx, const uint8_t* d_blob, const uint64_t* d_offs, uint32_t n,
                       uint64_t blob_len, bool outer, const KeyRef& key, int32_t* d_status,
-                      uint32_t* extra_cap, FillArgs* fills, const std::function<int()>* after_fill) {
+                      uint32_t* extra_cap, bool rows, FillArgs* fills, const std::function<int()>* after_fill) {
+  ctx->open_rows = nullptr;
   int rc = reserve_batch(ctx, n, blob_len, extra_cap);
   if (rc) return rc;
   hipError_t e;
@@ -133,14 +134,15 @@
   }
   if (after_fill && (rc = (*after_fill)())) return rc;
   SegScratch sc = segscratch(ctx, *extra_cap);
-  if ((e = ctx->poly_aux.reserve((size_t)n * sizeof(PolyAux))) != hipSuccess)
-    return ctx->hip_fail(e, "reserve poly aux");
+  if (rows && (e = ctx->poly_aux.reserve((size_t)n * sizeof(OpenRow))) != hipSuccess)
+    return ctx->hip_fail(e, "reserve open rows");
   const int t = ctx->tbegin("open_setup");
   if ((e = launch_open_setup(ctx->stream, d_blob, d_offs, n, outer, dev_key(key), key_status(key),
-                             ctx->params.as<FileParams>(), d_status, sc,
-                             ctx->poly_aux.as<PolyAux>())) != hipSuccess)
+                             ctx->params.as<FileParams>(), d_status, sc, nullptr,
+                             rows ? ctx->poly_aux.as<OpenRow>() : nullptr)) != hipSuccess)
     return ctx->hip_fail(e, "open setup");
   ctx->tend(t);
+  if (rows) ctx->open_rows = ctx->poly_aux.as<OpenRow>();
   return CE_OK;
 }
 
@@ -148,6 +150,7 @@
                 uint64_t blob_len, bool outer, const KeyRef& key, uint8_t* d_out,
                 int32_t* d_status, bool sync_counters, bool small_lanes, const DecodeArgs* ds) {
   uint32_t ec;
+  ctx->open_rows = nullptr;
   int rc = reserve_batch(ctx, n, blob_len, &ec);
   if (rc) return rc;
   hipError_t e;
@@ -214,6 +217,7 @@
   if (int32_t ks = key_status(key)) return ctx->fail(ks, "key rejected");
   const uint32_t seg_blocks = n <= 4 && clear_len_total <= (1u << 20) ? kPageBytes / 16 : kSegBlocks;
   uint32_t ec;
+  ctx->open_rows = nullptr;
   int rc = reserve_batch(ctx, n, clear_len_total + 16ull * n, &ec, seg_blocks);
   if (rc) return rc;
   hipError_t e;
diff --git a/crdt-enc_amd/csrc/ce_device.h b/crdt-enc_amd/csrc/ce_device.h
--- a/crdt-enc_amd/csrc/ce_device.h
+++ b/crdt-enc_amd/csrc/ce_device.h
@@ -327,7 +327,8 @@
   }
 }
 
-__device__ __forceinline__ void poly_aux(const FileParams& P, PolyAux& X) {
+template <class Row>
+__device__ __forceinline__ void poly_aux_powers(const FileParams& P, Row& X) {
   const L5 r = load_l5(P.rpow[0]), r2 = load_l5(P.rpow[1]), r4 = load_l5(P.rpow[2]);
   const L5 r3 = mulmod(r2, r);
   const L5 r12 = mulmod(load_l5(P.rpow[3]), r4);
@@ -342,6 +343,37 @@
     X.r3[i] = r3.v[i]; X.r12[i] = r12.v[i]; X.r48[i] = r48.v[i];
     X.e6[i] = e6.v[i]; X.lr[i] = lr.v[i];
   }
+}
+
+__device__ __forceinline__ void tag_less_s(const uint32_t (&tag)[4], const uint32_t (&s)[4], uint32_t (&ts)[4]) {
+  typedef unsigned __int128 u128;
+  auto wide = [](const uint32_t (&w)[4]) {
+    return (u128)w[0] | ((u128)w[1] << 32) | ((u128)w[2] << 64) | ((u128)w[3] << 96);
+  };
+  const u128 d = wide(tag) - wide(s);
+#pragma unroll
+  for (int i = 0; i < 4; i++) ts[i] = (uint32_t)(d >> (32 * i));
+}
+
+__device__ __forceinline__ void open_row(const FileParams& P, OpenRow& R) {
+#pragma unroll
+  for (int i = 0; i < 8; i++) R.subkey[i] = P.subkey[i];
+  R.n2[0] = P.n2[0]; R.n2[1] = P.n2[1];
+  R.in_off = P.in_off;
+  R.len = P.len;
+  R.pad0[0] = R.pad0[1] = R.pad0[2] = 0;
+#pragma unroll
+  for (int i = 0; i < 4; i++) R.s[i] = P.s[i];
+#pragma unroll
+  for (int k = 0; k < 7; k++) {
+#pragma unroll
+    for (int i = 0; i < 5; i++) R.rpow[k][i] = P.rpow[k][i];
+  }
+  poly_aux_powers(P, R);
+}
+
+__device__ __forceinline__ void poly_aux(const FileParams& P, PolyAux& X) {
+  poly_aux_powers(P, X);
   uint64_t b = 0;
 #pragma unroll
   for (int i = 0; i < 4; i++) {
diff --git a/crdt-enc_amd/csrc/ce_fused.hip b/crdt-enc_amd/csrc/ce_fused.hip
--- a/crdt-enc_amd/csrc/ce_fused.hip
+++ b/crdt-enc_amd/csrc/ce_fused.hip
@@ -692,6 +692,7 @@
 
 hipError_t launch_open_fold_small(hipStream_t s, const DecodeArgs& a, int files_per_wave, OpenLaunchLog& log) {
   if (a.n == 0) return hipSuccess;
+  if (a.rows) return hipErrorInvalidValue;
   static const uint32_t res16 = resident_blocks(k_open_fold_small<16>, 128);
   static const uint32_t res32 = resident_blocks(k_open_fold_small<32>, 256);
   static const uint32_t res64 = resident_blocks(k_open_fold_small<64>, 256);
@@ -751,6 +752,32 @@
     p.R1[i] = Pp->rpow[0][i];
     p.R64[i] = Pp->rpow[6][i];
     p.R2[i] = Pp->rpow[1][i];
+  }
+  return p;
+}
+
+__device__ __forceinline__ FilePre2 load_pre3(const DecodeArgs& a, uint32_t f) {
+  FilePre2 p;
+  const bool in = f < a.n;
+  const uint32_t fi = in ? f : 0u;
+  const OpenRow* Rp = a.rows + fi;
+  const int32_t stv = a.status[fi];
+  const uint32_t ov = a.only ? (uint32_t)a.only[fi] : 1u;
+  const uint32_t av = a.apply ? (uint32_t)a.apply[fi] : 1u;
+  p.ok = (uint32_t)in & (uint32_t)(stv == CE_OK) & (uint32_t)(ov != 0);
+  p.apply = av != 0;
+  p.len = Rp->len;
+  p.in_off = (uint32_t)Rp->in_off;
+  p.in_hi = (uint32_t)(Rp->in_off >> 32);
+#pragma unroll
+  for (int i = 0; i < 8; i++) p.key[i] = Rp->subkey[i];
+  p.n2a = Rp->n2[0];
+  p.n2b = Rp->n2[1];
+#pragma unroll
+  for (int i = 0; i < 5; i++) {
+    p.R1[i] = Rp->rpow[0][i];
+    p.R64[i] = Rp->rpow[6][i];
+    p.R2[i] = Rp->rpow[1][i];
   }
   return p;
 }
@@ -1494,7 +1521,7 @@
   uint32_t gn = bcast(blockIdx.x * fixed), c_end = gn + fixed;
   if (fixed == 0) chunk(gn, c_end);
   if (a.stamps && lane == 0) a.stamps[(uint64_t)kStampWords * blockIdx.x] = __builtin_amdgcn_s_memrealtime();
-  FilePre2 nx = load_pre2(a, gn * F + grp);
+  FilePre2 nx = load_pre3(a, gn * F + grp);
   const SupVers sup(a);
   DecState S{PN ? 51u : 38u, 0, 0, 0, 0, 0xffffffffu};
   GsCounts gsc;
@@ -1502,38 +1529,36 @@
   AuthFails fails;
   const uint32_t qpos = (sub + 15u) & 15u;
   const uint32_t qx = qpos & 3u, qy = qpos >> 2;
-  static_assert(offsetof(FileParams, rpow) == 80, "rpow offset");
-  auto wsrc = [&](uint32_t q, uint32_t aux_off, uint32_t rp_idx, const uint8_t*& base, uint32_t& stride) {
+  auto wsrc = [&](uint32_t q, uint32_t top_off, uint32_t rp_idx, const uint8_t*& base, uint32_t& stride) {
     base = q == 0 ? reinterpret_cast<const uint8_t*>(kPolyOne)
-         : q == 3 ? reinterpret_cast<const uint8_t*>(a.aux) + aux_off
-                  : reinterpret_cast<const uint8_t*>(a.params) + 80u + 20u * rp_idx;
-    stride = q == 0 ? 0u : q == 3 ? (uint32_t)sizeof(PolyAux) : (uint32_t)sizeof(FileParams);
+                  : reinterpret_cast<const uint8_t*>(a.rows) +
+                        (q == 3 ? top_off : (uint32_t)offsetof(OpenRow, rpow) + 20u * rp_idx);
+    stride = q == 0 ? 0u : (uint32_t)sizeof(OpenRow);
   };
   const uint8_t* x_base;
   const uint8_t* y_base;
   uint32_t x_stride, y_stride;
-  wsrc(qx, (uint32_t)offsetof(PolyAux, r12), qx + 1u, x_base, x_stride);
-  wsrc(qy, (uint32_t)offsetof(PolyAux, r48), qy + 3u, y_base, y_stride);
+  wsrc(qx, (uint32_t)offsetof(OpenRow, r12), qx + 1u, x_base, x_stride);
+  wsrc(qy, (uint32_t)offsetof(OpenRow, r48), qy + 3u, y_base, y_stride);
 
   uint4 ct[BPL][4];
   while (gn < ngroups) {
     const uint32_t f = gn * F + grp;
     const FilePre2 cur = nx;
     if (++gn == c_end) chunk(gn, c_end);
-    if (EARLY) nx = load_pre2(a, gn * F + grp);
+    if (EARLY) nx = load_pre3(a, gn * F + grp);
     const bool act = cur.ok && cur.len <= kSmallMax;
     const uint32_t len = act ? cur.len : 0u;
     const uint32_t npc = (len + 15) >> 4;
     const int32_t nblk = (int32_t)((len + 63) >> 6);
-    const FileParams* Pp = a.params + (act ? f : 0);
-    const PolyAux* Xp = a.aux + (act ? f : 0);
+    const OpenRow* Rp = a.rows + (act ? f : 0);
     const uint8_t* src = act ? a.blob + (((uint64_t)cur.in_hi << 32) | cur.in_off)
-                             : reinterpret_cast<const uint8_t*>(a.params);
+                             : reinterpret_cast<const uint8_t*>(a.rows);
 #pragma unroll
     for (int k = BPL - 1; k >= 0; k--) {
       const int32_t b = nblk - 1 - (int32_t)sub - LPF * k;
       if (k > 0) {
-        const uint8_t* bp = b >= 0 ? src + 64u * (uint32_t)b : reinterpret_cast<const uint8_t*>(a.params);
+        const uint8_t* bp = b >= 0 ? src + 64u * (uint32_t)b : reinterpret_cast<const uint8_t*>(a.rows);
 #pragma unroll
         for (int j = 0; j < 4; j++) ct[k][j] = *reinterpret_cast<const uint4*>(bp + 16 * j);
       } else {
@@ -1550,8 +1575,8 @@
     for (int i = 0; i < 5; i++) {
       R1.v[i] = cur.R1[i];
       RC.v[i] = cur.R64[i];
-      R2.v[i] = Pp->rpow[1][i];
-      R3.v[i] = Xp->r3[i];
+      R2.v[i] = Rp->rpow[1][i];
+      R3.v[i] = Rp->r3[i];
     }
     const ChachaPre cpre = chacha_pre(cur.key, 0u, cur.n2a, cur.n2b);
     L5 acc{{0, 0, 0, 0, 0}}, glast{{0, 0, 0, 0, 0}};
@@ -1578,11 +1603,13 @@
         for (int i = 0; i < 5; i++) {
           X.v[i] = xs[i];
           Y.v[i] = ys[i];
-          E6.v[i] = Xp->e6[i];
-          LR.v[i] = Xp->lr[i];
+          E6.v[i] = Rp->e6[i];
+          LR.v[i] = Rp->lr[i];
         }
-#pragma unroll
-        for (int i = 0; i < 4; i++) ts[i] = Xp->ts[i];
+        const uint4 tg = *reinterpret_cast<const uint4*>(src + len);
+        const uint4 sv = *reinterpret_cast<const uint4*>(Rp->s);
+        const uint32_t tw[4] = {tg.x, tg.y, tg.z, tg.w}, sw[4] = {sv.x, sv.y, sv.z, sv.w};
+        tag_less_s(tw, sw, ts);
       }
       uint32_t kb[16];
       if (!PAIR) {
@@ -1664,15 +1691,15 @@
     if (CE_V3_PRIO) __builtin_amdgcn_s_setprio(CE_V3_PRIO);
     if constexpr (LW) {
       decode_lww_lds<LPF>(a, sup, fl, len, act && ok, cur.apply != 0, f, grp, sub, lwc, [&] {
-        if (!EARLY) nx = load_pre2(a, gn * F + grp);
+        if (!EARLY) nx = load_pre3(a, gn * F + grp);
       });
     } else if constexpr (GS) {
       decode_gset_lds<LPF>(a, sup, fl, len, act && ok, cur.apply != 0, f, grp, sub, gsc, [&] {
-        if (!EARLY) nx = load_pre2(a, gn * F + grp);
+        if (!EARLY) nx = load_pre3(a, gn * F + grp);
       });
     } else {
       decode_fold<LPF, true, PN>(a, sup, fl, len, act && ok, cur.apply != 0, f, grp, sub, S, [&] {
-        if (!EARLY) nx = load_pre2(a, gn * F + grp);
+        if (!EARLY) nx = load_pre3(a, gn * F + grp);
       });
     }
     if (CE_V3_PRIO) __builtin_amdgcn_s_setprio(0);
@@ -1923,7 +1950,7 @@
 hipError_t launch_open_fold_pn(hipStream_t s, const DecodeArgs& a, OpenLaunchLog& log, hipEvent_t t0,
                                hipEvent_t t1) {
   if (a.n == 0) return hipSuccess;
-  if (!a.aux) return hipErrorInvalidValue;
+  if (!a.rows) return hipErrorInvalidValue;
   static const uint32_t res = resident_blocks(k_open_fold_v3<false, true, true>, 64);
   const dim3 grid(log.grid(std::min<uint32_t>((a.n + 3) / 4, res), "open_v3_pn"));
   const DecodeArgs b = log.stamped(a, grid.x);
@@ -1935,7 +1962,7 @@
 hipError_t launch_open_fold_gset(hipStream_t s, const DecodeArgs& a, OpenLaunchLog& log, hipEvent_t t0,
                                  hipEvent_t t1) {
   if (a.n == 0) return hipSuccess;
-  if (!a.aux || !a.gs) return hipErrorInvalidValue;
+  if (!a.rows || !a.gs) return hipErrorInvalidValue;
   static const uint32_t res = resident_blocks(k_open_fold_v3<false, true, false, true>, 64);
   const dim3 grid(log.grid(std::min<uint32_t>((a.n + 3) / 4, res), "open_v3_gset"));
   const DecodeArgs b = log.stamped(a, grid.x);
@@ -1947,7 +1974,7 @@
 hipError_t launch_open_fold_lww(hipStream_t s, const DecodeArgs& a, OpenLaunchLog& log, hipEvent_t t0,
                                 hipEvent_t t1) {
   if (a.n == 0) return hipSuccess;
-  if (!a.aux || !a.lw) return hipErrorInvalidValue;
+  if (!a.rows || !a.lw) return hipErrorInvalidValue;
   static const uint32_t res = resident_blocks(k_open_fold_v3<false, true, false, false, true>, 64);
   const dim3 grid(log.grid(std::min<uint32_t>((a.n + 3) / 4, res), "open_v3_lww"));
   const DecodeArgs b = log.stamped(a, grid.x);
@@ -1956,11 +1983,16 @@
   return hipGetLastError();
 }
 
+bool open_fold_v2_takes_rows(int files_per_wave) {
+  static const bool force_v2 = getenv("CE_FUSED_V2") != nullptr;
+  return files_per_wave == 4 && !force_v2;
+}
+
 hipError_t launch_open_fold_v2(hipStream_t s, const DecodeArgs& a, int files_per_wave, OpenLaunchLog& log,
                                hipEvent_t t0, hipEvent_t t1) {
   if (a.n == 0) return hipSuccess;
-  static const bool force_v2 = getenv("CE_FUSED_V2") != nullptr;
-  if (files_per_wave == 4 && a.aux && !force_v2) {
+  if (a.rows && !open_fold_v2_takes_rows(files_per_wave)) return hipErrorInvalidValue;
+  if (a.rows) {
     static const int v3 = [] {
       const char* e = getenv("CE_V3");
       return e ? atoi(e) : 2;
diff --git a/crdt-enc_amd/csrc/ce_gset.h b/crdt-enc_amd/csrc/ce_gset.h
--- a/crdt-enc_amd/csrc/ce_gset.h
+++ b/crdt-enc_amd/csrc/ce_gset.h
@@ -28,6 +28,7 @@
   const uint8_t* apply;
   const uint8_t* only;
   int large_only;
+  const OpenRow* rows;
   GsTable committed;
   GsTable batch;
   uint32_t* paths;
diff --git a/crdt-enc_amd/csrc/ce_gset.hip b/crdt-enc_amd/csrc/ce_gset.hip
--- a/crdt-enc_amd/csrc/ce_gset.hip
+++ b/crdt-enc_amd/csrc/ce_gset.hip
@@ -116,7 +116,7 @@
   const uint32_t stride = gridDim.x * kWaves;
   for (uint32_t f = __builtin_amdgcn_readfirstlane(blockIdx.x * kWaves + (threadIdx.x >> 6)); f < a.n; f += stride) {
     if (a.only && !a.only[f]) continue;
-    if (a.large_only && a.params[f].len <= kSmallMax) continue;
+    if (a.large_only && setup_len(a.params, a.rows, f) <= kSmallMax) continue;
     if (a.status[f] != CE_OK) continue;
     decode_gset_file(a, f, lane);
   }
diff --git a/crdt-enc_amd/csrc/ce_gset_host.cpp b/crdt-enc_amd/csrc/ce_gset_host.cpp
--- a/crdt-enc_amd/csrc/ce_gset_host.cpp
+++ b/crdt-enc_amd/csrc/ce_gset_host.cpp
@@ -108,6 +108,7 @@
     a.apply = ctx->apply.as<uint8_t>();
     a.only = only;
     a.large_only = large_only ? 1 : 0;
+  a.rows = large_only ? ctx->open_rows : nullptr;
     a.committed = committed(g);
     a.batch = batch(g);
     a.paths = g->meta.as<uint32_t>() + 12;
@@ -829,7 +830,8 @@
   hipError_t e;
   int rc;
   uint32_t ec = 0;
-  if ((rc = device_open_setup(ctx, d_blob, d_offs, n, blob_len, true, key_of(c), ctx->status.as<int32_t>(), &ec)))
+  if ((rc = device_open_setup(ctx, d_blob, d_offs, n, blob_len, true, key_of(c), ctx->status.as<int32_t>(), &ec,
+                              true)))
     return rc;
   uint32_t* paths = g->meta.as<uint32_t>() + 12;
   g->h_fused = GsFused{committed(g), batch(g), paths};
@@ -846,7 +848,7 @@
   da.n_supported = (uint32_t)c->supported.size();
   da.apply = ctx->apply.as<uint8_t>();
   da.counters = ctx->counters.as<uint32_t>();
-  da.aux = ctx->poly_aux.as<PolyAux>();
+  da.rows = ctx->open_rows;
   da.gs = g->fused.as<GsFused>();
   ctx->open_log.grid_cap = test_grid_cap();
   ctx->open_log.stamps = test_wave_stamps(ctx);
diff --git a/crdt-enc_amd/csrc/ce_internal.h b/crdt-enc_amd/csrc/ce_internal.h
--- a/crdt-enc_amd/csrc/ce_internal.h
+++ b/crdt-enc_amd/csrc/ce_internal.h
@@ -138,6 +138,7 @@
       supported, blob, offs, nonces, out_offs, outer_ver, batch_counters, split, segrec, redo, heads,
       poly_aux,
       stamps;
+  const ce::OpenRow* open_rows = nullptr;
   ce::OpenLaunchLog open_log;
   ce::HostBuf h_counters, h_apply, h_stage, h_stage2, h_heads;
   uint32_t publish_gen = 0;
@@ -214,7 +215,7 @@
 
 int device_open_setup(ce_ctx* ctx, const uint8_t* d_blob, const uint64_t* d_offs, uint32_t n,
                       uint64_t blob_len, bool outer, const KeyRef& key, int32_t* d_status,
-                      uint32_t* extra_cap, FillArgs* fills = nullptr,
+                      uint32_t* extra_cap, bool rows, FillArgs* fills = nullptr,
                       const std::function<int()>* after_fill = nullptr);
 SegScratch segscratch(ce_ctx* ctx, uint32_t extra_cap);
 int device_open(ce_ctx* ctx, const uint8_t* d_blob, const uint64_t* d_offs, uint32_t n,
diff --git a/crdt-enc_amd/csrc/ce_kernels.h b/crdt-enc_amd/csrc/ce_kernels.h
--- a/crdt-enc_amd/csrc/ce_kernels.h
+++ b/crdt-enc_amd/csrc/ce_kernels.h
@@ -1,5 +1,6 @@
 #pragma once
 #include <hip/hip_runtime.h>
+#include <stddef.h>
 #include <stdint.h>
 
 #include "ce_common.h"
@@ -39,6 +40,26 @@
 };
 static_assert(sizeof(PolyAux) == 128, "PolyAux layout");
 
+struct alignas(64) OpenRow {
+  uint32_t subkey[8];
+  uint32_t n2[2];
+  uint64_t in_off;
+  uint32_t len;
+  uint32_t pad0[3];
+  uint32_t s[4];
+  uint32_t rpow[7][5];
+  uint32_t r3[5];
+  uint32_t r12[5];
+  uint32_t r48[5];
+  uint32_t e6[5];
+  uint32_t lr[5];
+};
+static_assert(sizeof(OpenRow) == 320 && offsetof(OpenRow, rpow) == 80 && offsetof(OpenRow, s) == 64,
+              "OpenRow layout");
+__host__ __device__ inline uint32_t setup_len(const FileParams* params, const OpenRow* rows, uint32_t f) {
+  return rows ? rows[f].len : params[f].len;
+}
+
 struct DevKey {
   uint32_t k[8];
 };
@@ -73,7 +94,7 @@
 hipError_t launch_open_setup(hipStream_t s, const uint8_t* blob, const uint64_t* offs,
                              uint32_t n, bool outer, DevKey key, int32_t key_status,
                              FileParams* params, int32_t* status, SegScratch sc,
-                             PolyAux* aux = nullptr);
+                             PolyAux* aux = nullptr, OpenRow* rows = nullptr);
 hipError_t launch_seal_setup(hipStream_t s, const uint8_t* clear, const uint64_t* offs,
                              uint32_t n, const uint8_t* outer_version ,
                              const uint8_t* nonces, uint8_t* out, const uint64_t* out_offs,
@@ -127,6 +148,7 @@
   int nil_actor;
   DsFuse ds;
   const PolyAux* aux;
+  const OpenRow* rows;
   unsigned long long* stamps;
 };
 static constexpr uint32_t kTicketWord = 32;
@@ -180,6 +202,7 @@
 };
 
 hipError_t launch_open_fold_small(hipStream_t s, const DecodeArgs& a, int files_per_wave, OpenLaunchLog& log);
+bool open_fold_v2_takes_rows(int files_per_wave);
 hipError_t launch_open_fold_v2(hipStream_t s, const DecodeArgs& a, int files_per_wave, OpenLaunchLog& log,
                                hipEvent_t t0 = nullptr, hipEvent_t t1 = nullptr);
 hipError_t launch_open_fold_pn(hipStream_t s, const DecodeArgs& a, OpenLaunchLog& log,
diff --git a/crdt-enc_amd/csrc/ce_kernels.hip b/crdt-enc_amd/csrc/ce_kernels.hip
--- a/crdt-enc_amd/csrc/ce_kernels.hip
+++ b/crdt-enc_amd/csrc/ce_kernels.hip
@@ -2,13 +2,15 @@
 
 namespace ce {
 
+constexpr uint32_t kRowVecs = sizeof(OpenRow) / 16;
+template <bool ROWS>
 __global__ __launch_bounds__(256) void k_open_setup(const uint8_t* __restrict__ blob,
                                                     const uint64_t* __restrict__ offs, uint32_t n,
                                                     int outer, DevKey key, int32_t key_status,
                                                     FileParams* __restrict__ params,
                                                     int32_t* __restrict__ status, SegScratch sc,
-                                                    PolyAux* __restrict__ aux) {
-  __shared__ uint4 stage[256 * 8];
+                                                    PolyAux* __restrict__ aux, OpenRow* __restrict__ rows) {
+  __shared__ uint4 stage[ROWS ? 128 * kRowVecs : 256 * 8];
   const uint32_t f = blockIdx.x * blockDim.x + threadIdx.x;
   const bool active = f < n;
   const uint64_t off = active ? offs[f] : 0;
@@ -61,6 +63,7 @@
   }
   if (st == CE_OK && !fast) st = parse_envelope(enc, enc_len, &e);
   FileParams P;
+  if constexpr (ROWS) P = FileParams{};
   P.status = st;
   P.len = 0;
   P.in_off = 0;
@@ -71,8 +74,10 @@
     const uint64_t ct_off = (uint64_t)(enc - blob) + e.enc_off;
     P.in_off = ct_off;
     P.len = (uint32_t)(e.enc_len - 16);
-    const uint4 t = *reinterpret_cast<const uint4*>(blob + ct_off + P.len);
-    P.tag[0] = t.x; P.tag[1] = t.y; P.tag[2] = t.z; P.tag[3] = t.w;
+    if (!ROWS || P.len > kSmallMax) {
+      const uint4 t = *reinterpret_cast<const uint4*>(blob + ct_off + P.len);
+      P.tag[0] = t.x; P.tag[1] = t.y; P.tag[2] = t.z; P.tag[3] = t.w;
+    }
     if (!fast) {
 #pragma unroll
       for (int k = 0; k < 6; k++) nw[k] = ld_le32(enc + e.nonce_off + 4 * k);
@@ -81,6 +86,31 @@
     if (P.len > kSmallMax) sc.large_list[atomicAdd(&sc.counters[9], 1u)] = f;
   }
   reserve_segments(P, f, sc, st == CE_OK);
+  if constexpr (ROWS) {
+    OpenRow R;
+    open_row(P, R);
+    if (active && (st != CE_OK || P.len > kSmallMax)) params[f] = P;
+    const uint4* rv = reinterpret_cast<const uint4*>(&R);
+    const uint32_t f0 = blockIdx.x * blockDim.x;
+    const uint32_t nrow = min(n - f0, (uint32_t)blockDim.x);
+    uint4* dst = reinterpret_cast<uint4*>(rows + f0);
+    const uint32_t t = threadIdx.x & 127;
+#pragma unroll
+    for (uint32_t h = 0; h < 2; h++) {
+      if (h) __syncthreads();
+      if ((threadIdx.x >> 7) == h) {
+#pragma unroll
+        for (uint32_t i = 0; i < kRowVecs; i++) stage[t * kRowVecs + (i ^ ((t >> 2) & 3))] = rv[i];
+      }
+      __syncthreads();
+#pragma unroll
+      for (uint32_t k = 0; k < 128 * kRowVecs / 256; k++) {
+        const uint32_t j = threadIdx.x + 256u * k;
+        const uint32_t row = j / kRowVecs, col = j % kRowVecs;
+        if (128u * h + row < nrow) dst[128u * h * kRowVecs + j] = stage[row * kRowVecs + (col ^ ((row >> 2) & 3))];
+      }
+    }
+  } else {
   PolyAux X;
   if (aux) {
     if (st == CE_OK) poly_aux(P, X);
@@ -111,6 +141,7 @@
         }
       }
     }
+  }
   }
   if (!active) return;
   status[f] = st;
@@ -738,8 +769,7 @@
   }
   for (uint32_t w = bcast(blockIdx.x * kWavesPerBlock + (threadIdx.x >> 6)); w < nwork; w += stride) {
     const uint32_t f = w;
-    const FileParams* Pp = a.params + f;
-    if ((a.only && !a.only[f]) || (a.large_only && Pp->len <= kSmallMax)) continue;
+    if ((a.only && !a.only[f]) || (a.large_only && setup_len(a.params, a.rows, f) <= kSmallMax)) continue;
     if (a.status[f] != CE_OK) continue;
     decode_file<true>(a, f, lane);
   }
@@ -764,8 +794,7 @@
   }
   for (uint32_t w = bcast(blockIdx.x * kWavesPerBlock + (threadIdx.x >> 6)); w < nwork; w += stride) {
     const uint32_t f = w;
-    const FileParams* Pp = a.params + f;
-    if ((a.only && !a.only[f]) || (a.large_only && Pp->len <= kSmallMax)) continue;
+    if ((a.only && !a.only[f]) || (a.large_only && setup_len(a.params, a.rows, f) <= kSmallMax)) continue;
     if (a.status[f] != CE_OK) continue;
     decode_file(a, f, lane);
   }
@@ -1221,10 +1250,16 @@
 
 hipError_t launch_open_setup(hipStream_t s, const uint8_t* blob, const uint64_t* offs, uint32_t n,
                              bool outer, DevKey key, int32_t key_status, FileParams* params,
-                             int32_t* status, SegScratch sc, PolyAux* aux) {
+                             int32_t* status, SegScratch sc, PolyAux* aux, OpenRow* rows) {
   if (n == 0) return hipSuccess;
-  hipLaunchKernelGGL(k_open_setup, dim3((n + 255) / 256), dim3(256), 0, s, blob, offs, n,
-                     outer ? 1 : 0, key, key_status, params, status, sc, aux);
+  if (rows && aux) return hipErrorInvalidValue;
+  if (rows) {
+    hipLaunchKernelGGL(k_open_setup<true>, dim3((n + 255) / 256), dim3(256), 0, s, blob, offs, n,
+                       outer ? 1 : 0, key, key_status, params, status, sc, aux, rows);
+  } else {
+    hipLaunchKernelGGL(k_open_setup<false>, dim3((n + 255) / 256), dim3(256), 0, s, blob, offs, n,
+                       outer ? 1 : 0, key, key_status, params, status, sc, aux, rows);
+  }
   return hipGetLastError();
 }
 
diff --git a/crdt-enc_amd/csrc/ce_lww.h b/crdt-enc_amd/csrc/ce_lww.h
--- a/crdt-enc_amd/csrc/ce_lww.h
+++ b/crdt-enc_amd/csrc/ce_lww.h
@@ -58,6 +58,7 @@
   const uint8_t* apply;
   const uint8_t* only;
   int large_only;
+  const OpenRow* rows;
   LwwRec* rec;
   uint32_t* paths;
 };
diff --git a/crdt-enc_amd/csrc/ce_lww.hip b/crdt-enc_amd/csrc/ce_lww.hip
--- a/crdt-enc_amd/csrc/ce_lww.hip
+++ b/crdt-enc_amd/csrc/ce_lww.hip
@@ -126,7 +126,7 @@
   const uint32_t stride = gridDim.x * kWaves;
   for (uint32_t f = __builtin_amdgcn_readfirstlane(blockIdx.x * kWaves + (threadIdx.x >> 6)); f < a.n; f += stride) {
     if (a.only && !a.only[f]) continue;
-    if (a.large_only && a.params[f].len <= kSmallMax) continue;
+    if (a.large_only && setup_len(a.params, a.rows, f) <= kSmallMax) continue;
     if (a.status[f] != CE_OK) continue;
     decode_lww_file(a, f, lane);
   }
diff --git a/crdt-enc_amd/csrc/ce_lww_host.cpp b/crdt-enc_amd/csrc/ce_lww_host.cpp
--- a/crdt-enc_amd/csrc/ce_lww_host.cpp
+++ b/crdt-enc_amd/csrc/ce_lww_host.cpp
@@ -58,6 +58,7 @@
   a.apply = ctx->apply.as<uint8_t>();
   a.only = only;
   a.large_only = large_only ? 1 : 0;
+  a.rows = large_only ? ctx->open_rows : nullptr;
   a.rec = l->rec.as<LwwRec>();
   a.paths = paths_of(l);
   uint32_t hp[4];
@@ -132,7 +133,8 @@
   hipError_t e;
   int rc;
   uint32_t ec = 0;
-  if ((rc = device_open_setup(ctx, d_blob, d_offs, n, blob_len, true, key_of(c), ctx->status.as<int32_t>(), &ec)))
+  if ((rc = device_open_setup(ctx, d_blob, d_offs, n, blob_len, true, key_of(c), ctx->status.as<int32_t>(), &ec,
+                              true)))
     return rc;
   uint32_t* paths = paths_of(l);
   l->h_fused = LwwFused{l->rec.as<LwwRec>(), paths};
@@ -150,7 +152,7 @@
   da.n_supported = (uint32_t)c->supported.size();
   da.apply = ctx->apply.as<uint8_t>();
   da.counters = ctx->counters.as<uint32_t>();
-  da.aux = ctx->poly_aux.as<PolyAux>();
+  da.rows = ctx->open_rows;
   da.lw = l->fused.as<LwwFused>();
   ctx->open_log.grid_cap = test_grid_cap();
   ctx->open_log.stamps = test_wave_stamps(ctx);
```

New measurement: 381.4 million op files/s (median of 5 runs). About the same (+0.3%).
